# jianhengLiu/VINS-RGBD-FAST

Hardware: AMD Instinct MI355X
Metric: VIO frames/sec (640x480, 150 feats, 10-KF window) (higher is better)
Workload: dtype f64; 1 GPU; BASELINE configs[2]: 128 independent synthetic 640x480 RGB-D + 200 Hz IMU sequences per MI355X, 150 features, 10-keyframe window; sequences_per_gpu=128, tracker_lag=1, parallelism=sequences sharded per GPU, no data-path collective

## Files before the change

### vins-rgbd-fast_amd/csrc/be_kernels.hip

```cpp
#include <hip/hip_runtime.h>
#include "kernels.h"
#include "be_factors.h"

using namespace dm;

#if VIO_TIMERS
#define PH_INIT long long ph_t0 = (s == 0 && threadIdx.x == 0) ? VIO_CLOCK() : 0
#define PH(k) do { if (s == 0 && threadIdx.x == 0) { long long n_ = VIO_CLOCK(); B.timings[k] += (float)(n_ - ph_t0); ph_t0 = n_; } } while (0)
#else
#define PH_INIT do {} while (0)
#define PH(k) do {} while (0)
#endif

namespace {

struct Ctx {
    float *timings;
    const DevCfg *C;
    int s, W, P, LW, NL, NLs, NPR;
    BeSeq *be;
    FeSeq *fe;
    const vio_calibration *K;
    PreInt *pre;
    int *lm_id, *lm_start, *lm_nobs, *lm_est, *lm_solve, *lm_dyn, *lm_order, *lm_free, *lm_tmp, *lm_pidx, *lm_aidx, *lm_relo;
// ... 1486 lines not shown
                bool hit = false;
                int r = 0;
                if (k < F) { int st_, no_, rl_, r0_; lm_fields(k, st_, no_, rl_, r0_); r = r0_ + (j - i - 1); hit = st_ == i && no_ > j - i && r < nres; }
                unsigned long long m = __ballot(hit);
                if (hit) c.pair_list[o + __popcll(m & ((1ULL << lane) - 1ULL))] = r;
                o += __popcll(m);
            }
            if (relo_on && j == i + 1)
                for (int k0 = 0; k0 < F; k0 += 64) {
                    int k = k0 + lane;
                    bool hit = false;
                    int r = 0;
                    if (k < F) { int st_, no_, rl_, r0_; lm_fields(k, st_, no_, rl_, r0_); r = r0_ + no_ - 1; hit = st_ == i && rl_ && r < nres; }
                    unsigned long long m = __ballot(hit);
                    if (hit) c.pair_list[o + __popcll(m & ((1ULL << lane) - 1ULL))] = r;
                    o += __popcll(m);
                }
        }
        __syncthreads();
    }
    PH(104);
    if (t == 0) {
        be.n_in_problem = F; be.n_var_landmarks = Fa; be.n_residuals = nres - sh_i[3];
        be.relo_factors = sh_i[3];
        be.iterations = 0; be.successful = 0;
    }
    __syncthreads();
}

__device__ __forceinline__ void solve_epilogue(Ctx &c, const Params &X, double cost, int iters_done, int succ, long long ts0, double *sdx, double *sh_d, int *sh_i) {
    const int t = threadIdx.x, nt = blockDim.x;
    const vio_config &cfg = c.C->c;
    BeSeq &be = *c.be;
    const int W = c.W, nlm = be.n_lm;
    if (!cfg.use_imu) {
        if (t == 0) {
            be.final_cost = cost; be.iterations = iters_done; be.successful = succ;
            be.iter_total += iters_done; be.solve_total++;
            be.dbg[4] = (int)(VIO_CLOCK() - ts0);
        }
        if (t <= W) {
            const int i = t;
            for (int k = 0; k < 7; k++) be.para_Pose[i][k] = X.pose[i * 7 + k];
            stm(be.Rs[i], q2R(qnormalized(mkq(X.pose[i * 7 + 6], X.pose[i * 7 + 3], X.pose[i * 7 + 4], X.pose[i * 7 + 5]))));
            be.Ps[i][0] = X.pose[i * 7]; be.Ps[i][1] = X.pose[i * 7 + 1]; be.Ps[i][2] = X.pose[i * 7 + 2];
        }
    } else {
    if (t == 0) {
        be.final_cost = cost; be.iterations = iters_done; be.successful = succ;
        be.iter_total += iters_done; be.solve_total++;
        be.dbg[4] = (int)(VIO_CLOCK() - ts0);
        v3 origin_R0 = R2ypr(ldm(be.Rs[0]));
        v3 origin_P0 = ld3(be.Ps[0]);
        quat q0 = mkq(X.pose[6], X.pose[3], X.pose[4], X.pose[5]);
        v3 origin_R00 = R2ypr(q2R(q0));
        double y_diff = origin_R0.x - origin_R00.x;
        m3 rot_diff = ypr2R(mk(y_diff, 0, 0));
        if (fabs(fabs(origin_R0.y) - 90) < 1.0 || fabs(fabs(origin_R00.y) - 90) < 1.0) rot_diff = mul(ldm(be.Rs[0]), tr(q2R(q0)));
        sh_d[0] = 0;
        for (int q = 0; q < 9; q++) sdx[q] = rot_diff.a[q];
        sdx[9] = origin_P0.x; sdx[10] = origin_P0.y; sdx[11] = origin_P0.z;
    }
    __syncthreads();
    if (t <= W) for (int k = 0; k < 7; k++) be.para_Pose[t][k] = X.pose[t * 7 + k];
    if (t <= W) {
        int i = t;
        m3 rot_diff = ldm(sdx);
        v3 origin_P0 = mk(sdx[9], sdx[10], sdx[11]);
        quat qi = qnormalized(mkq(X.pose[i * 7 + 6], X.pose[i * 7 + 3], X.pose[i * 7 + 4], X.pose[i * 7 + 5]));
        stm(be.Rs[i], mul(rot_diff, q2R(qi)));
        st3(be.Ps[i], add(mul(rot_diff, mk(X.pose[i * 7] - X.pose[0], X.pose[i * 7 + 1] - X.pose[1], X.pose[i * 7 + 2] - X.pose[2])), origin_P0));
        st3(be.Vs[i], mul(rot_diff, mk(X.sb[i * 9], X.sb[i * 9 + 1], X.sb[i * 9 + 2])));
        for (int k = 0; k < 3; k++) { be.Bas[i][k] = X.sb[i * 9 + 3 + k]; be.Bgs[i][k] = X.sb[i * 9 + 6 + k]; }
        if (i == W && !be.init_frame) for (int k = 0; k < 3; k++) be.latest_Bg[k] = X.sb[i * 9 + 6 + k];
    }
    if (t == W + 1) {
        be.tic[0] = X.ex[0]; be.tic[1] = X.ex[1]; be.tic[2] = X.ex[2];
        stm(be.ric, q2R(qnormalized(mkq(X.ex[6], X.ex[3], X.ex[4], X.ex[5]))));
        if (cfg.estimate_td) be.td = X.td;
    }
    __syncthreads();
    if (t == 0 && be.relo_info) {
        const m3 rot_diff = ldm(sdx);
        const v3 origin_P0 = mk(sdx[9], sdx[10], sdx[11]);
        const m3 relo_r = mul(rot_diff, q2R(qnormalized(mkq(X.relo[6], X.relo[3], X.relo[4], X.relo[5]))));
        const v3 relo_t = add(mul(rot_diff, mk(X.relo[0] - X.pose[0], X.relo[1] - X.pose[1], X.relo[2] - X.pose[2])), origin_P0);
        const m3 prev_r = ldm(be.prev_relo_r);
        const double drift_yaw = R2ypr(prev_r).x - R2ypr(relo_r).x;
        const m3 dr = ypr2R(mk(drift_yaw, 0, 0));
        stm(be.drift_correct_r, dr);
        st3(be.drift_correct_t, sub(ld3(be.prev_relo_t), mul(dr, relo_t)));
        const int li = be.relo_local;
        const m3 Rl = ldm(be.Rs[li]);
        st3(be.relo_relative_t, mul(tr(relo_r), sub(ld3(be.Ps[li]), relo_t)));
        const quat qrel = R2q(mul(tr(relo_r), Rl));
        be.relo_relative_q[0] = qrel.w; be.relo_relative_q[1] = qrel.x; be.relo_relative_q[2] = qrel.y; be.relo_relative_q[3] = qrel.z;
        const double a = R2ypr(Rl).x - R2ypr(relo_r).x;
        be.relo_relative_yaw = a > 0 ? a - 360.0 * floor((a + 180.0) / 360.0) : a + 360.0 * floor((-a + 180.0) / 360.0);
        for (int k = 0; k < 7; k++) be.relo_Pose[k] = X.relo[k];
        be.relo_info = 0;
    }
    }
    for (int k = t; k < nlm; k += nt) {
        int slot = c.lm_order[k];
        int pi = c.lm_pidx[slot];
        if (pi < 0) continue;
        double d = 1.0 / c.feat[pi];
        c.lm_depth[slot] = d;
        c.lm_solve[slot] = d < 0 ? 2 : 1;
    }
    __syncthreads();
    if (be.solver_flag == 1 && !be.init_frame) {
        if (t == 0) {
            int fail = 0;
            if (nrm(ld3(be.Bas[W])) > 2.5) fail = 1;
            if (nrm(ld3(be.Bgs[W])) > 1.0) fail = 1;
            v3 tmpP = ld3(be.Ps[W]);
            if (nrm(sub(tmpP, ld3(be.last_P))) > 5) fail = 1;
            if (fabs(tmpP.z - be.last_P[2]) > 1) fail = 1;
            sh_i[0] = fail;
        }
        __syncthreads();
        if (sh_i[0]) {
            for (int k = t; k < c.NL; k += nt) c.lm_free[k] = c.NL - 1 - k;
            if (t == 0) {
                for (int i = 0; i <= W + 1; i++) c.pre[i].valid = 0;
                for (int i = 0; i <= W; i++) {
                    for (int k = 0; k < 3; k++) { be.Ps[i][k] = 0; be.Vs[i][k] = 0; be.Bas[i][k] = 0; be.Bgs[i][k] = 0; }
                    stm(be.Rs[i], eye());
                    be.Headers[i] = 0;
                    be.pre_idx[i] = i;
                }
                const vio_calibration &K = *c.K;
                for (int k = 0; k < 9; k++) be.ric[k] = cfg.estimate_extrinsic == 2 ? be.ex_ric[k] : K.ric[k];
                for (int k = 0; k < 3; k++) { be.tic[k] = K.tic[k]; be.latest_Bg[k] = 0; }
                be.td = K.td;
                be.g[0] = 0; be.g[1] = 0; be.g[2] = K.g_norm;
                be.first_imu = 0; be.frame_count = 0; be.solver_flag = 0; be.openExEstimation = 0; be.has_prior = 0;
                be.initFirstPoseFlag = 0; be.prevTime = -1; be.n_lm = 0; be.n_free = c.NL; be.ring_base = 0;
                be.imu_head = be.imu_count_ingest;
                be.relo_info = 0;
                be.reboot_count++;
                be.status_code = VIO_REBOOTED;
                be.rebooted = 1;
                be.do_marg = 0;
                be.overflow = 0;
            }
        }
    }
}

}

template <bool EXACT> __device__ void marg_body(const Batch &B, int s, int *scratch, double *sred, unsigned char *smem_marg);
__device__ void finish_body(const Batch &B, int s, int *scratch, PreWork &pw, unsigned char *smem_marg);

__device__ __forceinline__ void solve_body(const Batch &B, int s, int *scratch, double *sred, unsigned char *smem, PreWork &pw);

__global__ __launch_bounds__(1024) void be_solve_kernel(Batch B) {
    const int s = blockIdx.x + B.s0;
    __shared__ int scratch[2 * 1024 + 8];
    __shared__ double sred[64];
    extern __shared__ __attribute__((aligned(16))) unsigned char smem[];
    PreWork &pw = *(PreWork *)(smem + 16 * ((B.cfg->LW * 8 + 15) / 16));
    solve_body(B, s, scratch, sred, smem, pw);
}
__global__ __launch_bounds__(512) void be_solve_kernel_512(Batch B) {
    const int s = blockIdx.x + B.s0;
    __shared__ int scratch[2 * 1024 + 8];
    __shared__ double sred[64];
    extern __shared__ __attribute__((aligned(16))) unsigned char smem[];
    PreWork &pw = *(PreWork *)(smem + 16 * ((B.cfg->LW * 8 + 15) / 16));
    solve_body(B, s, scratch, sred, smem, pw);
}
__global__ __launch_bounds__(512) void be_marg_kernel(Batch B) {
    const int s = blockIdx.x + B.s0;
    __shared__ int scratch[2 * 512 + 8];
    __shared__ double sred[64];
    __shared__ PreWork pw;
    extern __shared__ __attribute__((aligned(16))) unsigned char smem[];
    marg_body<false>(B, s, scratch, sred, smem);
    __syncthreads();
    finish_body(B, s, scratch, pw, smem);
}
__global__ __launch_bounds__(512) void be_marg_exact_kernel(Batch B) {
    const int s = blockIdx.x + B.s0;
    __shared__ int scratch[2 * 512 + 8];
    __shared__ double sred[64];
    __shared__ PreWork pw;
    extern __shared__ __attribute__((aligned(16))) unsigned char smem[];
    marg_body<true>(B, s, scratch, sred, smem);
    __syncthreads();
    finish_body(B, s, scratch, pw, smem);
}

__device__ __forceinline__ void solve_body(const Batch &B, int s, int *scratch, double *sred, unsigned char *smem, PreWork &pw) {
    const int t = threadIdx.x, nt = blockDim.x;
    Ctx c = make_ctx(B, s);
    const DevCfg &C = *B.cfg;
    const vio_config &cfg = C.c;
    BeSeq &be = *c.be;
    if (!be.do_solve) return;
    const int W = c.W, P = c.P, LW = c.LW, W1 = W + 1;
    __shared__ Params X, Xc;
    __shared__ double sdx[6 * VIO_MAXW + 16], srp[6 * VIO_MAXW + 16];
    __shared__ int sh_i[8];
    __shared__ double sh_d[8];
    double *xs = (double *)smem;
    double *work = xs + LW;
    const int npairs = (W + 1) * W / 2;
    double *pb = (npairs * 210 <= 12288) ? work : c.pairblk;
    __shared__ double chol_dinv[VIO_LWMAX];
    const bool tiles_in_lds = ((LW >> 4) * ((LW >> 4) + 1) / 2) * 256 <= 16896 && !(B.flags & 1);
    const bool schur_staged = tiles_in_lds && schur_staged_ok(LW, nt);
    const bool hpl_sparse = schur_staged && 6 * W1 + 7 <= 128;

    PH_INIT;
    const long long ts0 = VIO_CLOCK();
    int F, Fa, nres;
    solve_prologue(B, c, X, scratch, pw, sh_i, F, Fa, nres);
    {
        const int *al = c.pair_list + c.nres_cap - c.NL;
        int nb = 0;
        for (int k = t; k < Fa; k += nt) nb += c.lm_est[al[k]] == 2 ? 1 : 0;
        if (nb) { atomicOr(&c.be->overflow, 512); atomicAdd(&c.be->bounded_solves, nb); }
    }
    const int nlm = be.n_lm;
    int *alist = c.pair_list + c.nres_cap - c.NL;
    const int n = c.NPR;
    PH(2);
    const int ex_active = sh_i[0], td_active = sh_i[1];
    const bool vext = ex_active || td_active;
    const int ne_ext = vext ? 7 : 0;
    const int oE = 15 * W1, oT = 15 * W1 + 6;

    double *g = c.vec, *sp = c.vec + 1 * LW, *dgp = c.vec + 2 * LW, *gradp = c.vec + 3 * LW, *gnp = c.vec + 4 * LW, *stp = c.vec + 5 * LW,
           *gs = c.vec + 6 * LW, *tmpv = c.vec + 7 * LW, *delta = c.vec + 8 * LW, *sgp = c.vec + 9 * LW, *hsgp = c.vec + 10 * LW,
           *yp = c.vec + 11 * LW, *up = c.vec + 12 * LW, *tmpv2 = c.vec + 13 * LW;
    double *sl = c.lvec, *dgl = c.lvec + c.NLs, *gradl = c.lvec + 2 * c.NLs, *gnl = c.lvec + 3 * c.NLs, *stl = c.lvec + 4 * c.NLs,
           *inv = c.lvec + 5 * c.NLs, *gls = c.lvec + 6 * c.NLs, *Hlls = c.lvec + 7 * c.NLs;
    const int Kpad = (Fa + 3) & ~3;
    double *hsgl = c.res + (size_t)c.nres_cap * 42 - 4 * (size_t)c.NLs;
    double *yl = hsgl + c.NLs, *ul = yl + c.NLs, *tmpl = ul + c.NLs;

    double cost = evaluate(c, X, c.feat, true, nres, sred, sdx, srp, work, vext);
    PH(4);
    assemble(B, c, X, nres, Fa, alist, srp, work, pb, hpl_sparse, vext);
    PH(5);
    if (t == 0) be.initial_cost = cost;
    for (int a = t; a < LW; a += nt) {
        bool act = a < P && (a < oE ? true : (a < oT ? ex_active != 0 : td_active != 0));
        if (!cfg.use_imu && (a < 6 || (a >= 6 * W1 && a < oE))) act = false;
        sp[a] = act ? 1.0 / (1.0 + sqrt(c.H[a * LW + a])) : 0.0;
    }
    for (int k = t; k < Kpad; k += nt) sl[k] = k < Fa ? 1.0 / (1.0 + sqrt(c.Hll[k])) : 0.0;
    __syncthreads();
    auto prepare_point = [&]() -> double {
        double m = 0;
        for (int a = t; a < P; a += nt) m = fmax(m, sp[a] != 0.0 ? fabs(g[a]) : 0.0);
        for (int k = t; k < Fa; k += nt) m = fmax(m, fabs(c.gl[k]));
        double r = block_max(m, sred);
        for (int a = t; a < LW; a += nt) {
            double hs = a < P ? sp[a] * sp[a] * c.H[a * LW + a] : 0.0;
            gs[a] = a < P ? sp[a] * g[a] : 0.0;
            dgp[a] = sqrt(fmin(fmax(hs, 1e-6), 1e32));
            gradp[a] = gs[a] / dgp[a];
            sgp[a] = gradp[a] / dgp[a];
            up[a] = sp[a] * sgp[a];
        }
        for (int k = t; k < Kpad; k += nt) {
            double hl = k < Fa ? sl[k] * sl[k] * c.Hll[k] : 0.0;
            Hlls[k] = hl;
            gls[k] = k < Fa ? sl[k] * c.gl[k] : 0.0;
            dgl[k] = sqrt(fmin(fmax(hl, 1e-6), 1e32));
            gradl[k] = gls[k] / dgl[k];
            ul[k] = sl[k] * (gradl[k] / dgl[k]);
        }
        __syncthreads();
        return r;
    };

    double radius = 1e4, mu = 1e-8, alpha = 0, dogleg_norm = 0;
    bool cauchy_valid = false;
    auto compute_cauchy = [&]() {
        matvec_pass(c.H, LW, P, P, nullptr, up, nullptr, tmpv, work);
        matvec_pass_2range(c.Hpl, LW, Fa, P, 6 * W1, 15 * W1, ne_ext, ul, up, tmpv2, tmpl, work);
        double g2 = 0, jg2 = 0;
        for (int a = t; a < LW; a += nt) {
            double v = a < P ? sp[a] * (tmpv[a] + tmpv2[a]) : 0.0;
            hsgp[a] = v;
            if (a < P) { g2 += gradp[a] * gradp[a]; jg2 += sgp[a] * v; }
        }
        for (int k = t; k < Kpad; k += nt) {
            double sgl = k < Fa ? gradl[k] / dgl[k] : 0.0;
            double v = k < Fa ? sl[k] * tmpl[k] + Hlls[k] * sgl : 0.0;
            hsgl[k] = v;
            if (k < Fa) { g2 += gradl[k] * gradl[k]; jg2 += sgl * v; }
        }
        block_sum2(g2, jg2, sred);
        alpha = g2 / jg2;
        cauchy_valid = true;
    };

    bool reuse = false, need_eval = false, have_J = false;
    int invalid = 0;
    int iters_done = 0, succ = 0;
    if (prepare_point() > 1e-10)
    for (int iter = 1; iter <= cfg.max_iterations; iter++) {
        iters_done = iter;
        if (!reuse) {
            if (need_eval) {
                PH(13);
                if (!have_J) cost = evaluate(c, X, c.feat, true, nres, sred, sdx, srp, work, vext);
                have_J = false;
                PH(4);
                assemble(B, c, X, nres, Fa, alist, srp, work, pb, hpl_sparse, vext);
                PH(5);
                need_eval = false;
                if (prepare_point() <= 1e-10) { iters_done = iter - 1; break; }
                PH(6);
            }
            cauchy_valid = false;
            bool ok = false;
            while (mu < 1.0) {
                for (int k = t; k < Kpad; k += nt) {
                    double iv = k < Fa ? 1.0 / (Hlls[k] + mu * dgl[k] * dgl[k]) : 0.0;
                    inv[k] = iv;
                    tmpl[k] = sl[k] * iv * gls[k];
                }
                __syncthreads();
                matvec_pass_2range(c.Hpl, LW, Fa, P, 6 * W1, 15 * W1, ne_ext, tmpl, nullptr, tmpv, nullptr, work);
                for (int a = t; a < LW; a += nt) xs[a] = a < P ? gs[a] - sp[a] * tmpv[a] : 0.0;
                for (int k = t; k < Kpad; k += nt) tmpl[k] = sl[k] * sl[k] * inv[k];
                __syncthreads();
                bool chol_ok;
                if (tiles_in_lds) {
                    {
                        unsigned colmask = 0;
                        for (int cb = 0; cb < (LW >> 4); cb++) {
                            const int c0 = 16 * cb, c1 = c0 + 15;
                            if (c0 < 6 * W1 || (vext && c1 >= 15 * W1 && c0 < 15 * W1 + 7)) colmask |= 1u << cb;
                        }
                        if (schur_staged)
                            schur_mfma_staged<9>(c.H, c.Hpl, tmpl, dgp, sp, mu, Kpad, LW, LW, work, colmask);
// ... 193 lines not shown
        double *cs = (double *)smem, *sn = cs + 256;
        int *pp = (int *)(sn + 256), *qq = pp + 256;
        double *As = scrA, *V2 = scrV;
        for (int w = t; w < n * n; w += nt) { const int i = w / n, j = w - i * n; As[w] = 0.5 * (Ar[i * n + j] + Ar[j * n + i]); }
        __syncthreads();
        const bool hbm_ql = !c.C->eig_jacobi;
        if (hbm_ql) { sym_eig_hbm(As, n, n, (double *)marg_dyn_lds, sred); V2 = As; }
        else sw2 = jacobi_block(As, V2, n, n, cs, sn, pp, qq, sred);
        for (int k = t; k < n; k += nt) {
            ev2[k] = hbm_ql ? ((const double *)marg_dyn_lds)[k] : As[k * n + k];
            double vb = 0;
            for (int i = 0; i < n; i++) vb += V2[i * n + k] * br[i];
            vb2[k] = vb;
        }
        __syncthreads();
        for (int w = t; w < n * n; w += nt) {
            const int k = w / n, i = w - k * n;
            const double S = ev2[k] > eps ? ev2[k] : 0.0;
            c.prior_J[w] = sqrt(S) * V2[i * n + k];
        }
        for (int k = t; k < n; k += nt) {
            const double Sinv = ev2[k] > eps ? 1.0 / ev2[k] : 0.0;
            c.prior_rf[k] = sqrt(Sinv) * vb2[k];
        }
        __syncthreads();
        for (int w = t; w < n * n; w += nt) {
            const int a = w / n, bb = w - a * n;
            double sacc = 0;
            for (int k = 0; k < n; k++) sacc += c.prior_J[k * n + a] * c.prior_J[k * n + bb];
            c.prior_H[w] = sacc;
        }
        for (int a = t; a < n; a += nt) {
            double sacc = 0;
            for (int k = 0; k < n; k++) sacc += c.prior_J[k * n + a] * c.prior_rf[k];
            c.prior_r[a] = sacc;
        }
    }
    __syncthreads();
    double acc = 0;
    for (int k = t; k < n; k += nt) acc += c.prior_rf[k] * c.prior_rf[k];
    const double c0 = block_sum(acc, sred);
    __syncthreads();
    if (t == 0) be.prior_c0 = c0;
    return sw2;
}

__device__ void marg_exact_finish(const Ctx &c, BeSeq &be, double *A, const double *b, int md, int mq, int n, const double *Cl, int ldc, int F0,
                                  bool second_new, double *sred, unsigned char *smem) {
    const int t = threadIdx.x, nt = blockDim.x;
    const double eps = 1e-8;
    const int MX = c.C->MX, m = md + F0;
    double *Emm = c.margE, *EV = Emm + (size_t)MX * MX, *Einv = EV + (size_t)MX * MX, *ET1 = Einv + (size_t)MX * MX;
    extern __shared__ __attribute__((aligned(16))) unsigned char marg_dyn_lds[];
    double *cs = (double *)smem, *sn = cs + 256;
    int *pp = (int *)(sn + 256), *qq = pp + 256;
    auto amm = [&](int i, int j) -> double {
        if (i < md && j < md) return 0.5 * (A[i * mq + j] + A[j * mq + i]);
        if (i >= md && j >= md) return i == j ? c.Hll[i - md] : 0.0;
        return Cl[(size_t)((i >= md ? i : j) - md) * ldc + (i >= md ? j : i)];
    };
    int sw1 = 0;
    double *Ar = c.margV, *br = c.vec;
    const long long tx0 = VIO_CLOCK();
    if (m <= c.C->MXL) {
        const int ld = m | 1;
        double *Al = (double *)marg_dyn_lds, *aux = Al + (size_t)m * ld;
        for (int w = t; w < m * m; w += nt) { const int i = w / m, j = w - i * m; Al[i * ld + j] = amm(i, j); }
        __syncthreads();
        sym_eig_lds(Al, m, ld, aux, c.C->eig_one_wave != 0);
        if (VIO_TIMERS && t == 0) be.dbg[7] = (int)(VIO_CLOCK() - tx0);
        for (int k = t; k < m; k += nt) { const double ev = aux[k]; aux[EIG_LD + k] = ev > eps ? 1.0 / ev : 0.0; }
        __syncthreads();
        for (int w = t; w < m * m; w += nt) {
            const int i = w / m, j = w - i * m;
            double sacc = 0;
            for (int k = 0; k < m; k++) sacc += Al[i * ld + k] * Al[j * ld + k] * aux[EIG_LD + k];
            Einv[w] = sacc;
        }
    } else {
        for (int w = t; w < m * m; w += nt) { const int i = w / m, j = w - i * m; Emm[w] = amm(i, j); }
        __syncthreads();
        if (!c.C->eig_jacobi) {
            double *ewk = (double *)marg_dyn_lds;
            sym_eig_hbm(Emm, m, m, ewk, sred);
            if (VIO_TIMERS && t == 0) be.dbg[7] = (int)(VIO_CLOCK() - tx0);
            for (int k = t; k < m; k += nt) { const double ev = ewk[k]; ewk[SYM_EIG_HBM_MAX + k] = ev > eps ? 1.0 / ev : 0.0; }
            __syncthreads();
            for (int w = t; w < m * m; w += nt) {
                const int i = w / m, j = w - i * m;
                const double *vi = Emm + (size_t)i * m, *vj = Emm + (size_t)j * m;
                double sacc = 0;
                for (int k0 = 0; k0 < m; k0 += 16) {
                    double a[16], b[16];
#pragma unroll
                    for (int u = 0; u < 16; u++) { const int k = min(k0 + u, m - 1); a[u] = vi[k]; b[u] = vj[k]; }
#pragma unroll
                    for (int u = 0; u < 16; u++) if (k0 + u < m) sacc += a[u] * b[u] * ewk[SYM_EIG_HBM_MAX + k0 + u];
                }
                Einv[w] = sacc;
            }
        } else {
        sw1 = jacobi_block(Emm, EV, m, m, cs, sn, pp, qq, sred);
        if (VIO_TIMERS && t == 0) be.dbg[7] = (int)(VIO_CLOCK() - tx0);
        for (int w = t; w < m * m; w += nt) {
            const int i = w / m, j = w - i * m;
            double sacc = 0;
            for (int k = 0; k < m; k++) { const double ev = Emm[(size_t)k * m + k]; if (ev > eps) sacc += EV[(size_t)i * m + k] * EV[(size_t)j * m + k] / ev; }
            Einv[w] = sacc;
        }
        }
    }
    __syncthreads();
    for (int w = t; w < n * m; w += nt) {
        const int i = w / m, j = w - i * m;
        double sacc = 0;
        for (int k = 0; k < md; k++) sacc += A[(md + i) * mq + k] * Einv[(size_t)k * m + j];
        for (int k0 = md; k0 < m; k0 += 16) {
            double a[16], b[16];
#pragma unroll
            for (int u = 0; u < 16; u++) { const int k = min(k0 + u, m - 1); a[u] = Cl[(size_t)(k - md) * ldc + md + i]; b[u] = Einv[(size_t)k * m + j]; }
#pragma unroll
            for (int u = 0; u < 16; u++) if (k0 + u < m) sacc += a[u] * b[u];
        }
        ET1[w] = sacc;
    }
    __syncthreads();
    for (int w = t; w < n * n; w += nt) {
        const int i = w / n, j = w - i * n;
        double tt = A[(md + i) * mq + md + j];
        for (int k = 0; k < md; k++) tt -= ET1[(size_t)i * m + k] * A[k * mq + md + j];
        for (int k0 = md; k0 < m; k0 += 16) {
            double a[16], b[16];
#pragma unroll
            for (int u = 0; u < 16; u++) { const int k = min(k0 + u, m - 1); a[u] = ET1[(size_t)i * m + k]; b[u] = Cl[(size_t)(k - md) * ldc + md + j]; }
#pragma unroll
            for (int u = 0; u < 16; u++) if (k0 + u < m) tt -= a[u] * b[u];
        }
        Ar[w] = tt;
    }
    for (int i = t; i < n; i += nt) {
        double sacc = b[md + i];
        for (int k = 0; k < md; k++) sacc -= ET1[(size_t)i * m + k] * b[k];
        for (int k = md; k < m; k++) sacc -= ET1[(size_t)i * m + k] * c.gl[k - md];
        br[i] = sacc;
    }
    __syncthreads();
    if (VIO_TIMERS && t == 0) be.dbg[8] = (int)(VIO_CLOCK() - tx0);
    const int sw2 = marg_literal_prior(c, be, Ar, br, n, c.margW, A, sred, smem);
    if (VIO_TIMERS && t == 0) be.dbg[9] = (int)(VIO_CLOCK() - tx0);
    if (t == 0) { be.dbg[0] = sw1 * 100 + sw2; be.dbg[2] = second_new ? 1 : 0; be.dbg[4] = m; }
    if (VIO_TIMERS && t == 0) be.dbg[10] = (int)(VIO_CLOCK() - tx0);
}

template <bool EXACT> __device__ void marg_body(const Batch &B, int s, int *scratch, double *sred, unsigned char *smem_marg) {
    const int t = threadIdx.x, nt = blockDim.x;
    Ctx c = make_ctx(B, s);
    const DevCfg &C = *B.cfg;
    const vio_config &cfg = C.c;
    BeSeq &be = *c.be;
    if (!be.do_marg || be.rebooted || be.frame_count < c.W) return;
    const int W = c.W, W1 = W + 1, n = c.NPR;
    const double eps = 1e-8;
    __shared__ Params X;
    __shared__ double sdx[6 * VIO_MAXW + 16], srp[6 * VIO_MAXW + 16];
    __shared__ double cs[VIO_MAXW * 3 + 10], sn[VIO_MAXW * 3 + 10];
    __shared__ int pp[VIO_MAXW * 3 + 10], qq[VIO_MAXW * 3 + 10];
    __shared__ double A15[225], V15[225], Pinv[225];
    __shared__ int newpresent[VIO_MAXW + 3];
    const bool second_new = be.marginalization_flag != 0;
    if (second_new && !(be.has_prior && be.prior_present[W - 1])) return;
    const bool exact = EXACT && cfg.marg_exact == 1 && c.margE != nullptr;
    const bool lit2 = EXACT && cfg.marg_exact == 2;
    int F0x = 0;
    int F0k = 0;
    PH_INIT;
    const long long tk0 = VIO_CLOCK();
    if (t <= W) {
        int i = t;
        X.pose[i * 7 + 0] = be.Ps[i][0]; X.pose[i * 7 + 1] = be.Ps[i][1]; X.pose[i * 7 + 2] = be.Ps[i][2];
        quat q = R2q(ldm(be.Rs[i]));
        X.pose[i * 7 + 3] = q.x; X.pose[i * 7 + 4] = q.y; X.pose[i * 7 + 5] = q.z; X.pose[i * 7 + 6] = q.w;
        for (int k = 0; k < 3; k++) { X.sb[i * 9 + k] = be.Vs[i][k]; X.sb[i * 9 + 3 + k] = be.Bas[i][k]; X.sb[i * 9 + 6 + k] = be.Bgs[i][k]; }
    }
    if (t == W + 1) {
        X.ex[0] = be.tic[0]; X.ex[1] = be.tic[1]; X.ex[2] = be.tic[2];
        quat q = R2q(ldm(be.ric));
        X.ex[3] = q.x; X.ex[4] = q.y; X.ex[5] = q.z; X.ex[6] = q.w;
        X.td = be.td;
    }
    if (t < W + 3) newpresent[t] = 0;
    __syncthreads();
    if (t <= W) for (int k = 0; k < 7; k++) be.para_Pose[t][k] = X.pose[t * 7 + k];
    const int md = second_new ? 6 : 15;
    const int mq = md + n;
    double *A = c.margA, *b = c.margB;
    for (int i = t; i < mq * mq; i += nt) A[i] = 0;
    for (int i = t; i < mq; i += nt) b[i] = 0;
    __syncthreads();
    const int rS = md + 6 * W, rE = md + 6 * W + 9, rT = md + 6 * W + 15;
    if (be.has_prior) {
        prior_dx(c, X, sdx);
        for (int i = t; i < n; i += nt) {
            double sacc = c.prior_r[i];
            for (int j0 = 0; j0 < n; j0 += 32) {
                double hv[32];
#pragma unroll
                for (int u = 0; u < 32; u++) hv[u] = c.prior_H[(size_t)min(j0 + u, n - 1) * n + i];
#pragma unroll
                for (int u = 0; u < 32; u++) if (j0 + u < n) sacc += hv[u] * sdx[j0 + u];
            }
            srp[i] = sacc;
        }
        __syncthreads();
        auto pmap = [&](int a) -> int {
            if (a < 6 * W) {
                int k = a / 6, d = a - 6 * k;
                if (second_new) return k == W - 1 ? d : md + 6 * k + d;
                return k == 0 ? d : md + 6 * (k - 1) + d;
            }
            if (a < 6 * W + 9) return second_new ? rS + (a - 6 * W) : 6 + (a - 6 * W);
            if (a < 6 * W + 15) return rE + (a - 6 * W - 9);
            return rT;
        };
        for (int w0 = t; w0 < n * n; w0 += 8 * nt) {
            double pv[8];
#pragma unroll
            for (int u = 0; u < 8; u++) pv[u] = c.prior_H[min(w0 + u * nt, n * n - 1)];
#pragma unroll
            for (int u = 0; u < 8; u++) {
                const int w = w0 + u * nt;
                if (w < n * n) { const int a = w / n, bb = w - a * n; A[pmap(a) * mq + pmap(bb)] = 0.0 + pv[u]; }
            }
        }
        for (int a = t; a < n; a += nt) b[pmap(a)] += srp[a];
        if (t < W + 3) {
            const int pres = be.prior_present[t];
            if (t > W) { if (pres) newpresent[t] = 1; }
            else if (second_new) { if (t < W - 1 || t == W) newpresent[t] = pres; }
            else if (t >= 1 && t < W && pres) newpresent[t - 1] = 1;
        }
        __syncthreads();
    }
    PH(16);
    if (!second_new) {
        PreInt &p1 = c.pre[be.pre_idx[1]];
        if (cfg.use_imu && p1.sum_dt < 10.0) {
            double *Jw = c.pairblk;
            double *raw = c.imu_raw;
            if ((t & 63) == 0) for (int part = t >> 6; part < 5; part += nt >> 6) {
                v3 G = ld3(be.g);
                if (part == 0) {
                    double r15[15];
                    bf::imu_raw_residual(p1, G, &X.pose[0], &X.sb[0], &X.pose[7], &X.sb[9], r15);
                    for (int r = 0; r < 15; r++) {
                        double sacc = 0;
                        for (int k = 0; k <= r; k++) sacc += p1.sqrt_info[r * 15 + k] * r15[k];
                        raw[r * 31 + 30] = sacc;
                    }
                } else
                    bf::imu_raw_jacobian_part(p1, G, &X.pose[0], &X.sb[0], &X.pose[7], &X.sb[9], part - 1, raw, 31);
            }
            __syncthreads();
            for (int w = t; w < 450; w += nt) {
                int r = w / 30, col = w - r * 30;
                double sacc = 0;
                for (int k = 0; k <= r; k++) sacc += p1.sqrt_info[r * 15 + k] * raw[k * 31 + col];
                Jw[w] = sacc;
            }
            __syncthreads();
            for (int w = t; w < 930; w += nt) {
                int a = w / 31, bb = w - a * 31;
                int ia = a < 15 ? a : (a < 21 ? md + (a - 15) : rS + (a - 21));
                double sacc = 0;
                if (bb < 30) {
                    int ib = bb < 15 ? bb : (bb < 21 ? md + (bb - 15) : rS + (bb - 21));
                    for (int k = 0; k < 15; k++) sacc += Jw[k * 30 + a] * Jw[k * 30 + bb];
                    A[ia * mq + ib] += sacc;
                } else {
                    for (int k = 0; k < 15; k++) sacc += Jw[k * 30 + a] * raw[k * 31 + 30];
                    b[ia] += sacc;
                }
            }
            if (t == 0) { newpresent[0] = 1; newpresent[W] = 1; }
            __syncthreads();
        }
        PH(17);
        int nlm = be.n_lm;
        int *flag = c.lm_tmp, *offs = c.res_k;
        for (int k = t; k < nlm; k += nt) { int slot = c.lm_order[k]; flag[k] = (in_problem(c, slot) && c.lm_start[slot] == 0) ? 1 : 0; }
        __syncthreads();
        int F0 = block_scan_flags(flag, nlm, offs, scratch);
        int *list0 = c.pair_list;
        for (int k = t; k < nlm; k += nt) if (flag[k]) list0[offs[k]] = c.lm_order[k];
        __syncthreads();
        const int per = W;
        int F0c = min(F0, c.nres_cap / per);
        if (exact) { F0c = min(F0c, min(C.MX - 15, 480)); F0x = F0c; }
        F0k = F0c;
        __shared__ double mgeo[(VIO_MAXW + 1) * 32 + 16];
        if (t >= 1 && t <= W) {
            bf::PairGeo g;
            bf::pair_geo(&X.pose[0], &X.pose[t * 7], X.ex, g);
            double *o = mgeo + (size_t)(t - 1) * 32;
            for (int q = 0; q < 9; q++) { o[q] = g.A1[q]; o[9 + q] = g.A2[q]; o[18 + q] = g.M[q]; }
            o[27] = g.t[0]; o[28] = g.t[1]; o[29] = g.t[2];
        }
        if (t == 0) stm(mgeo + (size_t)W * 32, q2R(mkq(X.ex[6], X.ex[3], X.ex[4], X.ex[5])));
        __syncthreads();
        for (int w = t; w < F0c * per; w += nt) {
            int li = w / per, k = w - li * per + 1;
            int slot = list0[li];
            double *out = c.res + (size_t)w * 42;
            if (k >= c.lm_nobs[slot]) { out[40] = 0; out[41] = 0; for (int q = 0; q < 40; q++) out[q] = 0; continue; }
            double rr[2], wgt = 1.0;
            const double inv_dep = 1.0 / c.lm_depth[slot];
            const bf::PairGeo &g = *(const bf::PairGeo *)(mgeo + (size_t)(k - 1) * 32);
            bf::eval_projection_pair(cfg, g, mgeo + (size_t)W * 32, X.ex, inv_dep, X.td, c.K->tr, obs_ptr(c, slot, 0), obs_ptr(c, slot, k), cfg.estimate_td != 0, rr, out,
                                     true, &wgt);
            out[40] = wgt * rr[0];
            out[41] = wgt * rr[1];
        }
        __syncthreads();
        PH(18);
        double *Cl = c.Hpl;
        const int ldc = c.LW;
        for (int w = t; w < F0c * ldc; w += nt) Cl[w] = 0;
        __syncthreads();
        {
            const int grp = t >> 4, gln = t & 15, ngrp = nt >> 4;
            for (int li0 = 0; li0 < F0c; li0 += ngrp) {
                const int li = li0 + grp;
                const bool act = li < F0c;
                const int no = act ? c.lm_nobs[list0[li]] : 0;
                double cm[13], dsum = 0, bsum = 0;
#pragma unroll
                for (int q = 0; q < 13; q++) cm[q] = 0;
                for (int k = gln + 1; k < no; k += 16) {
                    const double *Jg = c.res + (size_t)(li * per + k - 1) * 42;
                    double Jr[42];
#pragma unroll
                    for (int q = 0; q < 42; q++) Jr[q] = Jg[q];
                    const double jl0 = Jr[19], jl1 = Jr[39];
#pragma unroll
                    for (int q = 0; q < 6; q++) {
                        cm[q] += Jr[q] * jl0 + Jr[20 + q] * jl1;
                        cm[6 + q] += Jr[12 + q] * jl0 + Jr[32 + q] * jl1;
                        Cl[(size_t)li * ldc + md + 6 * (k - 1) + q] = Jr[6 + q] * jl0 + Jr[26 + q] * jl1;
                    }
                    if (cfg.estimate_td) cm[12] += Jr[18] * jl0 + Jr[38] * jl1;
                    dsum += jl0 * jl0 + jl1 * jl1;
                    bsum += jl0 * Jr[40] + jl1 * Jr[41];
                }
#pragma unroll
                for (int off = 8; off >= 1; off >>= 1) {
#pragma unroll
                    for (int q = 0; q < 13; q++) cm[q] += __shfl_xor(cm[q], off, 16);
                    dsum += __shfl_xor(dsum, off, 16);
                    bsum += __shfl_xor(bsum, off, 16);
                }
                if (act && gln == 0) {
#pragma unroll
                    for (int q = 0; q < 6; q++) { Cl[(size_t)li * ldc + q] = cm[q]; Cl[(size_t)li * ldc + rE + q] = cm[6 + q]; }
                    if (cfg.estimate_td) Cl[(size_t)li * ldc + rT] = cm[12];
                    c.Hll[li] = dsum;
                    c.gl[li] = bsum;
                }
            }
        }
        __syncthreads();
        PH(19);
        {
            const int lane = t & 63, wave = t >> 6, nw = nt >> 6, li = lane & 15, lk = lane >> 4;
            for (int j = 1 + wave; j <= W; j += nw) {
                v4f64 a00 = {0, 0, 0, 0}, a10 = {0, 0, 0, 0}, a11 = {0, 0, 0, 0};
                const int K = 2 * F0c;
                for (int k0 = 0; k0 < K; k0 += 64) {
                    double x0[16], x1[16];
#pragma unroll
                    for (int u = 0; u < 16; u++) {
                        int kk = k0 + 4 * u + lk;
                        bool valid = kk < K;
                        int lm = min(kk, K - 1) >> 1, sub = kk & 1;
                        const double *Jr = c.res + (size_t)(lm * per + j - 1) * 42;
                        double v0 = Jr[sub * 20 + li];
                        double v1 = Jr[li < 3 ? sub * 20 + 16 + li : 40 + sub];
                        x0[u] = valid ? v0 : 0.0;
                        x1[u] = (valid && li < 4) ? v1 : 0.0;
                    }
#pragma unroll
                    for (int u = 0; u < 16; u++) {
                        if (k0 + 16 * (u >> 2) >= K) break;
                        a00 = __builtin_amdgcn_mfma_f64_16x16x4f64(x0[u], x0[u], a00, 0, 0, 0);
                        a10 = __builtin_amdgcn_mfma_f64_16x16x4f64(x1[u], x0[u], a10, 0, 0, 0);
                        a11 = __builtin_amdgcn_mfma_f64_16x16x4f64(x1[u], x1[u], a11, 0, 0, 0);
                    }
                }
                double *out = c.pairblk + (size_t)(j - 1) * 210;
#pragma unroll
                for (int r = 0; r < 4; r++) {
                    int row = lk + 4 * r, col = li;
                    if (col <= row) out[sym_idx(col, row)] = a00[r];
                    if (row < 4) out[sym_idx(col, 16 + row)] = a10[r];
                    if (row < 4 && col < 4 && col <= row) out[sym_idx(16 + col, 16 + row)] = a11[r];
                }
            }
        }
        if (!exact) for (int li = t; li < F0c; li += nt) { double d = c.Hll[li]; c.Hll[li] = d > eps ? 1.0 / d : 0.0; }
        __syncthreads();
        PH(24);
        __shared__ signed char qfr[6 * VIO_MAXW + 40], qlc[6 * VIO_MAXW + 40];
        __shared__ double sub_part[4][6 * VIO_MAXW + 40];
        for (int a = t; a <= mq; a += nt) {
            int fr = -1, lc = 0;
            if (a == mq) { fr = 0; lc = 19; }
            else if (a < 6) { fr = 0; lc = a; }
            else if (a >= md && a < md + 6 * W) { fr = (a - md) / 6 + 1; lc = 6 + (a - md) % 6; }
            else if (a >= rE && a < rE + 6) { fr = 0; lc = 12 + (a - rE); }
            else if (a == rT && cfg.estimate_td) { fr = 0; lc = 18; }
            qfr[a] = (signed char)fr; qlc[a] = (signed char)lc;
        }
        for (int w = t; w < 4 * mq; w += nt) {
            const int ch = w / mq, a = w - ch * mq;
            double acc = 0;
            if (!exact) for (int li = ch; li < F0c; li += 4) acc += Cl[(size_t)li * ldc + a] * (c.gl[li] * c.Hll[li]);
            sub_part[ch][a] = acc;
        }
        __syncthreads();
        for (int w0 = t; w0 < mq * (mq + 1); w0 += 4 * nt) {
            bool use[4], multi[4], rhs[4];
            int dst[4], row[4], sidx[4];
            double pv[4], av[4];
#pragma unroll
            for (int u = 0; u < 4; u++) {
                const int w = min(w0 + u * nt, mq * (mq + 1) - 1);
                const int a = w / (mq + 1), bb = w - a * (mq + 1);
                const int fa = qfr[a], fb = qfr[bb];
                const int la = qlc[a], lb = qlc[bb];
                use[u] = w0 + u * nt < mq * (mq + 1) && fa >= 0 && fb >= 0 && !(fa > 0 && fb > 0 && fa != fb);
                multi[u] = use[u] && fa == 0 && fb == 0;
                rhs[u] = bb == mq; row[u] = a; dst[u] = a * mq + bb;
                sidx[u] = sym_idx(la, lb);
                const int f1 = fa > 0 ? fa : (fb > 0 ? fb : 1);
                pv[u] = use[u] ? c.pairblk[(size_t)(f1 - 1) * 210 + sidx[u]] : 0.0;
                av[u] = use[u] ? (rhs[u] ? b[a] : A[dst[u]]) : 0.0;
            }
#pragma unroll
            for (int u = 0; u < 4; u++) {
                if (!use[u]) continue;
                double sacc = pv[u];
                if (multi[u]) {
                    double fv[VIO_MAXW];
#pragma unroll
                    for (int j = 0; j < VIO_MAXW; j++) fv[j] = c.pairblk[(size_t)min(j, W - 1) * 210 + sidx[u]];
                    sacc = 0;
#pragma unroll
                    for (int j = 0; j < VIO_MAXW; j++) if (j < W) sacc += fv[j];
                }
                if (!rhs[u]) A[dst[u]] = av[u] + sacc;
                else b[row[u]] = av[u] + (sacc - ((sub_part[0][row[u]] + sub_part[1][row[u]]) + (sub_part[2][row[u]] + sub_part[3][row[u]])));
            }
        }
        __syncthreads();
        PH(25);
        if (!exact) {
            const int lane = t & 63, wave = t >> 6, nw = nt >> 6, li = lane & 15, lk = lane >> 4;
            const int nbq = (mq + 15) >> 4, ntile = nbq * (nbq + 1) / 2;
            for (int tile = wave; tile < ntile; tile += nw) {
                int ti, tj;
                tri_decode(tile, ti, tj);
                v4f64 acc = {0, 0, 0, 0};
                const int ca = min(16 * ti + li, ldc - 1), cb = min(16 * tj + li, ldc - 1);
                for (int k0 = 0; k0 < F0c; k0 += 64) {
                    double xa[16], xb[16];
#pragma unroll
                    for (int u = 0; u < 16; u++) {
                        int kk = k0 + 4 * u + lk;
                        bool valid = kk < F0c;
                        int kc = min(kk, F0c - 1);
                        double va = Cl[(size_t)kc * ldc + ca], vb = Cl[(size_t)kc * ldc + cb], dinv = c.Hll[kc];
                        xa[u] = valid ? -(va * dinv) : 0.0;
                        xb[u] = valid ? vb : 0.0;
                    }
#pragma unroll
                    for (int u = 0; u < 16; u++) {
                        if (k0 + 16 * (u >> 2) >= F0c) break;
                        acc = __builtin_amdgcn_mfma_f64_16x16x4f64(xa[u], xb[u], acc, 0, 0, 0);
                    }
                }
#pragma unroll
                for (int r = 0; r < 4; r++) {
                    int row = 16 * ti + lk + 4 * r, col = 16 * tj + li;
                    if (row < mq && col < mq && (ti != tj || col <= row)) {
                        A[row * mq + col] += acc[r];
                        if (row != col) A[col * mq + row] += acc[r];
                    }
                }
            }
        }
        for (int li = t; li < F0c; li += nt) {
            int no = c.lm_nobs[list0[li]];
            for (int k = 1; k < no; k++) newpresent[k - 1] = 1;
            if (no > 1) { newpresent[W + 1] = 1; if (cfg.estimate_td) newpresent[W + 2] = 1; }
        }
        __syncthreads();
    }
    if (VIO_TIMERS && s == 0 && t == 0 && !second_new) B.timings[31] += 1.0f;
    PH(20);
    if (exact) marg_exact_finish(c, be, A, b, md, mq, n, c.Hpl, c.LW, F0x, second_new, sred, smem_marg);
    else {
    for (int w = t; w < md * md; w += nt) { int i = w / md, j = w - i * md; A15[w] = 0.5 * (A[i * mq + j] + A[j * mq + i]); }
    __syncthreads();
    __shared__ int pinv_direct;
    __shared__ double L15[225];
    if (t < 64) {
        const bool okc = spd_inverse_wave16(A15, md, 1e-6, L15, V15, Pinv);
        if (t == 0) pinv_direct = okc ? 1 : 0;
    }
    __syncthreads();
    if (!pinv_direct) {
        if (t < 64) jacobi_wave16(A15, V15, md, md, cs, sn, pp, qq);
        __syncthreads();
        for (int w = t; w < md * md; w += nt) {
            int i = w / md, j = w - i * md;
            double sacc = 0;
            for (int k = 0; k < md; k++) { double ev = A15[k * md + k]; if (ev > eps) sacc += V15[i * md + k] * V15[j * md + k] / ev; }
            Pinv[w] = sacc;
        }
        __syncthreads();
    }
    if (VIO_TIMERS && s == 0 && t == 0 && pinv_direct) B.timings[26] += 1.0f;
    PH(36);
    double *T1 = (double *)smem_marg, *Amr = T1 + (size_t)n * md;
    for (int w = t; w < n * md; w += nt) {
        int i = w / md, j = w - i * md;
        double sacc = 0;
        for (int k = 0; k < md; k++) sacc += A[(md + i) * mq + k] * Pinv[k * md + j];
        T1[w] = sacc;
        const int k2 = w / n, j2 = w - k2 * n;
        Amr[w] = A[k2 * mq + md + j2];
    }
    __syncthreads();
    PH(37);
    double *Ar = c.margV;
    double *br = c.vec;
    for (int w0 = t; w0 < n * n; w0 += 8 * nt) {
        double av[8];
#pragma unroll
        for (int u = 0; u < 8; u++) { const int w = min(w0 + u * nt, n * n - 1), i = w / n, j = w - i * n; av[u] = A[(md + i) * mq + md + j]; }
#pragma unroll
        for (int u = 0; u < 8; u++) {
            const int w = w0 + u * nt;
            if (w >= n * n) break;
            const int i = w / n, j = w - i * n;
            double tt = av[u];
            for (int k = 0; k < md; k++) tt -= T1[i * md + k] * Amr[k * n + j];
            Ar[w] = tt;
        }
    }
    for (int i = t; i < n; i += nt) {
        double sacc = b[md + i];
        for (int k = 0; k < md; k++) sacc -= T1[i * md + k] * b[k];
        br[i] = sacc;
    }
    __syncthreads();
    PH(21);
    if (lit2) {
        __shared__ int cert_bad;
        if (t == 0) cert_bad = pinv_direct ? 0 : 1;
        __syncthreads();
        double n_t = 0, n_d = 0, n_db = 0;
        if (!second_new) {
            const double *Cl = c.Hpl;
            const int ldc = c.LW;
            for (int li = t; li < F0k; li += nt) {
                const double dinv = c.Hll[li];
                if (!(dinv > 0.0)) cert_bad = 1;
                n_d += dinv * dinv;
                for (int a = 0; a < md; a++) {
                    double tt = 0;
                    for (int bq = 0; bq < md; bq++) tt += Pinv[a * md + bq] * Cl[(size_t)li * ldc + bq];
                    tt *= dinv;
                    n_t += tt * tt;
                    const double db = dinv * Cl[(size_t)li * ldc + a];
                    n_db += db * db;
                }
            }
        }
        block_sum3(n_t, n_d, n_db, sred);
        double n_s = 0;
        for (int w = t; w < md * md; w += nt) n_s += Pinv[w] * Pinv[w];
        n_s = block_sum(n_s, sred);
        __syncthreads();
        if (t == 0) {
            const double bound = sqrt(n_s) + 2.0 * sqrt(n_t) + sqrt(n_d) + sqrt(n_db) * sqrt(n_t);
            const bool certified = !cert_bad && isfinite(bound) && bound > 0.0 && 1.0 / bound > 1e-7;
            be.dbg[11] = certified ? 1 : 0;
            if (!certified) be.dbg[12] += 1;
        }
        __syncthreads();
        const int sw2 = marg_literal_prior(c, be, Ar, br, n, c.margW, A, sred, smem_marg);
        if (t == 0) { be.dbg[0] = sw2; be.dbg[2] = second_new ? 1 : 0; be.dbg[4] = md; }
    } else {
    for (int w0 = t; w0 < n * n; w0 += 8 * nt) {
        double x[8], y[8];
#pragma unroll
        for (int u = 0; u < 8; u++) { const int w = min(w0 + u * nt, n * n - 1), i = w / n, j = w - i * n; x[u] = Ar[i * n + j]; y[u] = Ar[j * n + i]; }
#pragma unroll
        for (int u = 0; u < 8; u++) if (w0 + u * nt < n * n) c.prior_H[w0 + u * nt] = 0.5 * (x[u] + y[u]);
    }
    for (int i = t; i < n; i += nt) c.prior_r[i] = br[i];
    PH(38);
    {
        __shared__ __attribute__((aligned(16))) double cq_x[EIG_LD + 16];
        __shared__ double cq_dinv[EIG_LD + 16];
        __shared__ int cq_flag;
        const int nbq = (n + 15) >> 4;
        double *T = (double *)smem_marg;
        double dmax = 0;
        for (int i = t; i < n; i += nt) dmax = fmax(dmax, fabs(Ar[i * n + i]));
        dmax = block_max(dmax, sred);
        const double delta = 64.0 * 2.220446049250313e-16 * (double)n * dmax;
        const int ntl = nbq * (nbq + 1) / 2 * 256;
        for (int w0 = t; w0 < ntl; w0 += 4 * nt) {
            double x[4], y[4];
            int ii[4], jj[4], dd[4];
#pragma unroll
            for (int u = 0; u < 4; u++) {
                const int w = min(w0 + u * nt, ntl - 1);
                int tile = w >> 8, e = w & 255, r = e >> 4, cc = e & 15, ti, tj;
                tri_decode(tile, ti, tj);
                const int i = 16 * ti + r, j = 16 * tj + cc, ic = min(i, n - 1), jc = min(j, n - 1);
                ii[u] = i; jj[u] = j; dd[u] = tl_idx(ti, tj, r, cc);
                x[u] = Ar[ic * n + jc]; y[u] = Ar[jc * n + ic];
            }
#pragma unroll
            for (int u = 0; u < 4; u++) {
                if (w0 + u * nt >= ntl) break;
                const int i = ii[u], j = jj[u];
                T[dd[u]] = (i < n && j < n) ? 0.5 * (x[u] + y[u]) + (i == j ? delta : 0.0) : (i == j ? 1.0 : 0.0);
            }
        }
        for (int i = t; i < 16 * nbq; i += nt) cq_x[i] = i < n ? br[i] : 0.0;
        __syncthreads();
        PH(39);
        double c0 = 0;
        if (dmax > 0 && chol_tiles(T, nbq, &cq_flag, cq_dinv, nullptr, cq_x)) {
            double acc = 0;
            for (int i = t; i < n; i += nt) acc += cq_x[i] * cq_x[i];
            c0 = block_sum(acc, sred);
            if (!isfinite(c0)) c0 = 0;
        }
        __syncthreads();
        if (t == 0) { be.prior_c0 = c0; be.dbg[0] = 0; be.dbg[2] = second_new ? 1 : 0; }
    }
    }
    }
    PH(22);
    if (t < W) {
        int src = second_new ? (t == W - 1 ? W : t) : t + 1;
        for (int d = 0; d < 7; d++) c.prior_x0[t * 7 + d] = X.pose[src * 7 + d];
    }
    if (t == W) for (int d = 0; d < 9; d++) c.prior_x0[W * 7 + d] = X.sb[(second_new ? 0 : 1) * 9 + d];
    if (t == W + 1) { for (int d = 0; d < 7; d++) c.prior_x0[W * 7 + 9 + d] = X.ex[d]; c.prior_x0[W * 7 + 16] = X.td; }
    __syncthreads();
    if (t < W + 3) be.prior_present[t] = newpresent[t];
    if (t == 0) { be.has_prior = 1; be.dbg[3] = (int)(VIO_CLOCK() - tk0); }
    PH(23);
}

__global__ void be_set_relo_kernel(Batch B, int seq, const double *par) {
    if (threadIdx.x != 0 || blockIdx.x != 0) return;
    BeSeq &be = B.be[seq];
    const int W = B.cfg->W;
    be.relo_stamp = par[0];
    be.relo_index = (int)par[1];
    be.relo_nmatch = (int)par[2];
    for (int k = 0; k < 3; k++) be.prev_relo_t[k] = par[3 + k];
    for (int k = 0; k < 9; k++) be.prev_relo_r[k] = par[6 + k];
    for (int i = 0; i < W; i++)
        if (be.relo_stamp == be.Headers[i]) {
            be.relo_local = i;
            be.relo_info = 1;
            for (int j = 0; j < 7; j++) be.relo_Pose[j] = be.para_Pose[i][j];
        }
}

__global__ __launch_bounds__(512) void be_prior_factor_kernel(Batch B, int seq) {
    const int s = seq, t = threadIdx.x, nt = blockDim.x;
    __shared__ double sred[64];
    extern __shared__ __attribute__((aligned(16))) unsigned char smem_marg[];
    Ctx c = make_ctx(B, s);
    BeSeq &be = *c.be;
    if (!be.has_prior) return;
    const int n = c.NPR;
    const double eps = 1e-8;
    const double *br = c.prior_r;
    const long long tj0 = VIO_CLOCK();
    const bool in_lds = n <= 96;
    const int ldj = in_lds ? (n | 1) : n;
    double *As = in_lds ? (double *)smem_marg : c.margA;
    double *Vv = in_lds ? (double *)smem_marg + n * ldj : c.margW + (size_t)n * 16;
    for (int w = t; w < n * n; w += nt) { int i = w / n, j = w - i * n; As[i * ldj + j] = c.prior_H[w]; }
    __syncthreads();
    __shared__ double ev_d[6 * VIO_MAXW + 16], ev_e[6 * VIO_MAXW + 16], ev_g[6 * VIO_MAXW + 16];
    __shared__ double ev_part[8 * EIG_LD];
    if (in_lds) {
        double *Al = (double *)smem_marg;
        if ((nt >> 6) <= 8) sym_eig_tridiag_mt(Al, n, ldj, ev_d, ev_e, ev_g, ev_part);
        else sym_eig_tridiag(Al, n, ldj, ev_d, ev_e, ev_g, sred);
        if (t == 0) be.dbg[5] = (int)(VIO_CLOCK() - tj0);
        tridiag_ql_wave(Al, n, ldj, ev_d, ev_e);
    } else {
        double *Ag = c.margA;
        if ((nt >> 6) <= 8) sym_eig_tridiag_mt(Ag, n, ldj, ev_d, ev_e, ev_g, ev_part);
        else sym_eig_tridiag(Ag, n, ldj, ev_d, ev_e, ev_g, sred);
        if (t == 0) be.dbg[5] = (int)(VIO_CLOCK() - tj0);
        tridiag_ql_wave(Ag, n, ldj, ev_d, ev_e);
    }
    if (t == 0) be.dbg[6] = (int)(VIO_CLOCK() - tj0);
    Vv = As;
    if (t == 0) be.dbg[1] = (int)(VIO_CLOCK() - tj0);
    for (int w = t; w < n * n; w += nt) {
        int k = w / n, i = w - k * n;
        double wv = ev_d[k];
        double S = wv > eps ? wv : 0.0;
        c.prior_J[w] = sqrt(S) * Vv[i * ldj + k];
    }
    for (int k = t; k < n; k += nt) {
        double wv = ev_d[k];
        double Sinv = wv > eps ? 1.0 / wv : 0.0;
        double vb = 0;
        for (int i = 0; i < n; i++) vb += Vv[i * ldj + k] * br[i];
        c.prior_rf[k] = sqrt(Sinv) * vb;
    }
}

__device__ void finish_body(const Batch &B, int s, int *scratch, PreWork &pw, unsigned char *smem_marg) {
    const int t = threadIdx.x, nt = blockDim.x;
    Ctx c = make_ctx(B, s);
    const DevCfg &C = *B.cfg;
    const vio_config &cfg = C.c;
    BeSeq &be = *c.be;
    const int W = c.W, W1 = W + 1;
    __shared__ int sh_i[4];
    double *od = B.odom + (size_t)s * 11;
    if (!be.processed || be.rebooted) return;
    PH_INIT;
    int nlm = be.n_lm;
    int *flag = c.lm_pidx, *offs = c.lm_aidx;
    const int fc = be.frame_count;
    const int sflag0 = be.solver_flag;
    __syncthreads();
    const bool dyn_initial = sflag0 == 0 && (cfg.dynamic_init || (fc == W && !be.do_solve && be.ex_pending));
    if (dyn_initial) {
        if (fc < W) {
            if (t == 0) be.frame_count = fc + 1;
            return;
        }
    } else if (sflag0 == 0) {
        if (fc == W && be.do_solve) {
            if (t == 0) be.solver_flag = 1;
            __syncthreads();
        } else {
            if (t == 0 && fc < W) {
                int n = fc + 1;
                for (int k = 0; k < 3; k++) { be.Ps[n][k] = be.Ps[fc][k]; be.Vs[n][k] = be.Vs[fc][k]; be.Bas[n][k] = be.Bas[fc][k]; be.Bgs[n][k] = be.Bgs[fc][k]; }
                for (int k = 0; k < 9; k++) be.Rs[n][k] = be.Rs[fc][k];
                be.frame_count = n;
            }
            return;
        }
    } else if (!be.init_frame) {
        m3 ric = ldm(be.ric);
        v3 tic = ld3(be.tic);
        for (int k = t; k < nlm; k += nt) {
            int slot = c.lm_order[k];
            if (!(c.lm_nobs[slot] >= 2 && c.lm_start[slot] < W - 2)) continue;
            double depth = c.lm_depth[slot];
            if (depth < 0) continue;
            int imu_i = c.lm_start[slot], no = c.lm_nobs[slot];
            const double *oi = obs_ptr(c, slot, imu_i);
            v3 pts_i = mk(oi[0], oi[1], oi[2]);
            double err = 0, err3 = 0;
            int cnt = 0;
            for (int q = 1; q < no; q++) {
                int imu_j = imu_i + q;
                const double *oj = obs_ptr(c, slot, imu_j);
                v3 pts_j = mk(oj[0], oj[1], oj[2]);
                v3 pts_w = add(mul(ldm(be.Rs[imu_i]), add(mul(ric, scl(depth, pts_i)), tic)), ld3(be.Ps[imu_i]));
                v3 pts_cj = mul(tr(ric), sub(mul(tr(ldm(be.Rs[imu_j])), sub(pts_w, ld3(be.Ps[imu_j]))), tic));
                double rx = pts_cj.x / pts_cj.z - pts_j.x, ry = pts_cj.y / pts_cj.z - pts_j.y;
                err += sqrt(rx * rx + ry * ry);
                err3 += nrm(sub(pts_cj, pts_j)) / depth;
                cnt++;
            }
            if (cnt > 0) c.lm_dyn[slot] = (cfg.focal_length * err / cnt > 10 || err3 / cnt > 2.0) ? 1 : 0;
        }
        __syncthreads();
    }
    PH(27);
    if (be.marginalization_flag == 0) {
        if (t == 0) {
            for (int k = 0; k < 9; k++) be.back_R0[k] = be.Rs[0][k];
            for (int k = 0; k < 3; k++) be.back_P0[k] = be.Ps[0][k];
            int first = be.pre_idx[0];
            for (int i = 0; i < W; i++) {
                be.Headers[i] = be.Headers[i + 1];
                for (int k = 0; k < 3; k++) { be.Ps[i][k] = be.Ps[i + 1][k]; be.Vs[i][k] = be.Vs[i + 1][k]; be.Bas[i][k] = be.Bas[i + 1][k]; be.Bgs[i][k] = be.Bgs[i + 1][k]; }
                for (int k = 0; k < 9; k++) be.Rs[i][k] = be.Rs[i + 1][k];
                be.pre_idx[i] = be.pre_idx[i + 1];
            }
            be.pre_idx[W] = first;
            bf::preint_init(c.pre[first], ld3(be.acc_0), ld3(be.gyr_0), ld3(be.Bas[W]), ld3(be.Bgs[W]));
        }
        __syncthreads();
        PH(28);
        m3 R0 = mul(ldm(be.back_R0), ldm(be.ric)), R1 = mul(ldm(be.Rs[0]), ldm(be.ric));
        v3 P0 = add(ld3(be.back_P0), mul(ldm(be.back_R0), ld3(be.tic))), P1 = add(ld3(be.Ps[0]), mul(ldm(be.Rs[0]), ld3(be.tic)));
        for (int k = t; k < nlm; k += nt) {
            int slot = c.lm_order[k];
// ... 228 lines not shown
```

### vins-rgbd-fast_amd/csrc/kernels.h

```cpp
#pragma once
#include <hip/hip_runtime.h>
#include "vio_state.h"
#include "../../include/vio_synth.h"

#define PI_CH 8
#define PREINT_MANY_LDS_DOUBLES (PI_CH * (225 + 270))
static inline size_t fast_lds_bytes(int rw, int rh) {
    return (size_t)(((rw + 6) * rh + 15) & ~15) + (size_t)((rw * rh + 15) & ~15) + (size_t)(((rw - 6) * (rh - 6) + 63) / 64 + 2) * 8 + 16;
}
__host__ __device__ static inline size_t ps_eval_lds_bytes(int W) {
    const size_t W1 = (size_t)W + 1, a = (W1 * W1 + 1) * 32 * 8, b = (size_t)W * (VIO_PREINT_HDR + 1) * 8;
    return (a > b ? a : b) + 64;
}
static inline size_t ps_ls_lds_bytes(int W) { (void)W; return ((((sizeof(Params) / sizeof(double)) + 1) & ~(size_t)1) + 176) * 8 + 16; }
struct LkImages {
    const uint8_t *prev[4];
    const uint8_t *next[4];
    int w[4], h[4];
};

__global__ void fe_begin_kernel(Batch B, const double *stamps, int gate, int publish, const uint8_t *modes, const double *R_rel);
__global__ void be_latest_odometry_kernel(Batch B, int seq, double *out11);
__global__ void fe_predict_motion_kernel(Batch B, int seq, double t0, double t1, double *out9);
__global__ void fe_pyrdown_kernel(Batch B, const uint8_t *src_base, size_t src_stride, int sw, int sh, int dst_level, int write_level0);
__global__ void fe_pyrdown_stage_kernel(const uint8_t *src, int sw, int sh, uint8_t *dst);
__global__ void fe_clahe_lut_kernel(Batch B, const uint8_t *src_base, size_t stride);
__global__ void fe_clahe_apply_kernel(Batch B, const uint8_t *src_base, size_t stride);
__global__ void fe_clahe_lut_stage_kernel(const uint8_t *src, int W, int H, uint8_t *lut);
__global__ void fe_clahe_apply_stage_kernel(const uint8_t *src, int W, int H, const uint8_t *lut, uint8_t *dst);
__global__ void fe_predict_kernel(Batch B);
__global__ void fe_lk_kernel(Batch B);
__global__ void fe_lk_stage_kernel(LkImages im, int maxLevel, int n, const float2 *prevPts, float2 *nextPts, uint8_t *status);
__global__ void fe_ransac_stage_kernel(vio_config c, int n, const float2 *p1, const float2 *p2, uint8_t *status);
__global__ void fe_camera_stage_kernel(vio_camera cam, int n, const double *uv, const double *R9, double *ray, double *un, double *uv_out);
__global__ void fe_select_kernel(Batch B);
__global__ void fe_fast_kernel(Batch B);
__global__ void fe_fast_stage_kernel(const uint8_t *img, int W, GridRect r, uint32_t *out, int cap, int *count);
__global__ void fe_add_kernel(Batch B, int gate);
struct IngestSrc {
    const int *n_obs;
    const int *ids;
    const double *obs;
    const double *stamps;
    int cap;
};
template <bool EXCALIB> __global__ void be_ingest_kernel(Batch B, const uint16_t *depth_base, size_t depth_stride, IngestSrc src);
__global__ void be_stage_relative_r_kernel(int n, const double *corres6, double *R9);
__global__ void be_solve_kernel(Batch B);
__global__ void be_solve_kernel_512(Batch B);
__global__ void be_marg_kernel(Batch B);
__global__ void be_marg_exact_kernel(Batch B);
__global__ void ps_setup_kernel(Batch B);
__global__ void ps_eval_kernel(Batch B);
__global__ void ps_eval_kernel_occ3(Batch B);
__global__ void ps_eval_kernel_occ4(Batch B);
__global__ void ps_asm_a_kernel(Batch B);
__global__ void ps_asm_a_kernel_occ4(Batch B);
__global__ void ps_asm_b_schur_kernel(Batch B, int nb_b, int by_blocks);
__global__ void ps_serial_big_kernel(Batch B);
__global__ void ps_serial_kernel_512(Batch B);
__global__ void ps_final_kernel(Batch B);
__global__ void ps_ls_kernel(Batch B);
__global__ void ps_evalf_kernel(Batch B);
static inline size_t ps_evalf_lds_bytes(int W) {
    const size_t W1 = (size_t)W + 1, a = ((size_t)PS_FUSE_CAP * 28 + (W1 * W / 2 + 1) * 32) * 8 + (size_t)PS_FUSE_CAP * 12, b = ((size_t)W * (VIO_PREINT_HDR + 1) + (size_t)W * 465) * 8;
    return (a > b ? a : b) + 16;
}
__global__ void be_prior_factor_kernel(Batch B, int seq);
__global__ void be_set_relo_kernel(Batch B, int seq, const double *par);
__global__ void be_stage_pnp_kernel(const double *pts, int n, double *par6);
__global__ void be_dyn_finalize_kernel(Batch B, int seq, const double *samples, const int *offs);
__global__ void be_stage_imu_kernel(vio_config cfg, PreInt *P, int n, const double *dt, const double *acc, const double *gyr,
                                    const double *par, double g_norm, double *preint_out, double *r15, double *J480);
__global__ void be_stage_projection_kernel(vio_config cfg, const double *in, int use_td, int form, double *r2, double *J46);
__global__ void be_stage_imu_block_kernel(const PreInt *P, const double *par, double g_norm, double *G961);
__global__ void imu_scatter_kernel(Batch B, int total, const int *seq_of, const double *t, const double *acc, const double *gyr);
__global__ void imu_commit_kernel(Batch B, int total, const int *seq_of);
__global__ void synth_render_kernel(vio_synth_config c, int S, uint64_t seq0, const float *rays, const float *poses, uint8_t *gray, uint16_t *depth);
```

### vins-rgbd-fast_amd/csrc/vio_abi.hip

```cpp
#include <hip/hip_runtime.h>
#include <math.h>
#include <algorithm>
#include <cmath>
#include <stdlib.h>
#include <mutex>
#include <chrono>
#include <string>
#include <string.h>
#include <vector>
#include "kernels.h"
#include "dyninit_host.h"
#include "camera_model.h"
#include "snapshot.h"

thread_local std::string g_err;

namespace {

#define HIPCHK(x)                                                                                        \
    do {                                                                                                 \
        hipError_t e_ = (x);                                                                             \
        if (e_ != hipSuccess) { g_err = std::string(#x) + ": " + hipGetErrorString(e_); return VIO_EDEVICE; } \
    } while (0)

void circle_halfwidths(int radius, int *hw) {
    for (int i = 0; i <= radius; i++) hw[i] = -1;
    int err = 0, dx = radius, dy = 0, plus = 1, minus = (radius << 1) - 1;
    while (dx >= dy) {
        if (dx > hw[dy]) hw[dy] = dx;
        if (dy > hw[dx]) hw[dx] = dy;
        dy++;
        err += plus;
        plus += 2;
        int mask = (err <= 0) - 1;
        err -= minus & mask;
        dx += mask;
        minus -= mask & 2;
    }
}

}

struct vio_batch {
    DevCfg hc;
    Batch B;
    int S;
    int device = -1;
    struct Group {
        int s0 = 0, n = 0;
        hipStream_t stream = nullptr;
        hipStream_t fe_stream = nullptr;
        hipEvent_t ev_solve = nullptr, ev_fe = nullptr, ev_be = nullptr, ev_ingest = nullptr;
        hipStream_t copy_stream = nullptr;
        hipStream_t copy_stream2 = nullptr;
        hipGraphExec_t solve_graph = nullptr;
        uint64_t solve_graph_key = 0;
        hipEvent_t ev_up_gray[2] = {nullptr, nullptr}, ev_up_depth[2] = {nullptr, nullptr};
        bool up_used[2] = {false, false};
        int flip = 0;
        hipEvent_t ev_rd_gray[2] = {nullptr, nullptr}, ev_rd_depth[2] = {nullptr, nullptr};
        bool have_rd_gray[2] = {false, false}, have_rd_depth[2] = {false, false};
        hipEvent_t ev_host_fe = nullptr, ev_host_be = nullptr;
        bool host_fe_pending = false, host_be_pending = false;
        bool have_solve_ev = false, have_ingest_ev = false;
        static constexpr int kSideRing = 16;
        unsigned char *side_ring = nullptr;
        hipEvent_t side_ev[kSideRing] = {};
        bool side_used[kSideRing] = {};
        int side_pos = 0;
    };
    std::vector<Group> groups;
    int tracker_lag = 0;
    int extra_slots = 2;
    int xcd_n = 0;
    bool use_graph = false;
    int xcd_map = 1;
    int fe_xcd_map = 1;
    bool fe_partitioned = false;
    int ps_asm_b_blocks = 24;
    int asm_b_by_blocks = 2;
    int serial_threads = 512;
    hipStream_t stream = nullptr;
    hipStream_t fe_stream = nullptr;
    hipEvent_t ev[4];
    std::vector<void *> allocs;
    uint8_t *d_fisheye = nullptr;
    uint8_t *d_gray_stage = nullptr, *d_gray_stage1 = nullptr;
    uint16_t *d_depth_stage = nullptr, *d_depth_stage1 = nullptr;
    double *d_stamps = nullptr;
    uint8_t *d_modes = nullptr;
    double *d_rrel = nullptr;
    int *d_in_n = nullptr, *d_in_ids = nullptr;
    double *d_in_obs = nullptr, *d_in_stamps = nullptr;
    double *d_r9 = nullptr;
    std::vector<vio_calibration> cal;
    vio_calibration *d_cal = nullptr;
    std::vector<vio_camera> cam;
    vio_camera *d_cam = nullptr;
    struct DynSeq {
        std::vector<vinit::ImageFrame> frames;
        double initial_timestamp = 0;
        bool nonlinear = false;
        int attempts = 0, failures = 0, last_stage = 0;
    };
    std::vector<DynSeq> dyn;
    bool dyn_active = false;
    int *h_state = nullptr;
    int *d_state = nullptr;
    hipEvent_t ev_state = nullptr;
    bool state_pending = false;
    double *d_dyn_samples = nullptr;
    int *d_dyn_offs = nullptr;
    size_t dyn_samples_cap = 0;
    std::mutex imu_mu;
    std::vector<int> p_seq;
    std::vector<double> p_t, p_acc, p_gyr;
    struct ImuStage {
        int *h_seq = nullptr, *d_seq = nullptr;
        double *h_t = nullptr, *h_acc = nullptr, *h_gyr = nullptr, *d_t = nullptr, *d_acc = nullptr, *d_gyr = nullptr;
        size_t cap = 0;
        hipEvent_t done = nullptr;
        bool busy = false;
    } imu_stage[2];
    int imu_stage_cur = 0;
    hipEvent_t ev_imu = nullptr;
    std::vector<double> last_imu_t;
    size_t lds_select = 0, lds_add = 0, lds_fast = 0, lds_solve = 0, lds_serial = 0, lds_marg = 0, lds_factor = 0, lds_ps_ls = 0, lds_ps_evalf = 0;
    int ps_evalf_blocks = 0;
    bool feed_throttle = true;
    int uploads_in_flight = 2;
    int relo_frames = 0;
    bool line_search = true;
    int be_threads = 512, marg_threads = 384;
    int solve_mode = 1;
    bool asm_a_occ4 = false;
    int eval_occ = 0;
    bool serial_big = false;
    size_t lds_ps_eval = 0;
    int ps_eval_blocks = 0, ps_asm_a_blocks = 0, ps_schur_tiles = 0;
    bool timing_valid = false;
    std::vector<hipEvent_t> pev;
    int prof_steps = 0, prof_cur = -1;
    bool prof_fe_only = false;
    struct SnapRow { const char *name; int kind; unsigned char *base; int64_t bytes, blob_off; };
    std::vector<SnapRow> snap_rows;
    int64_t snap_dev_bytes = 0, snap_chunks = 0;
    int snap_entries = 0;
    SnapEntry *d_snap_tab = nullptr;
    SnapSeq *d_snap_seqs = nullptr;
    size_t snap_seqs_cap = 0;
    unsigned char *d_snap_stage = nullptr;
    size_t snap_stage_cap = 0;
};
#define VIO_NK 10
#define VIO_NEV 12
#define PEV(h, k) do { if (g.s0 == 0 && (h)->prof_cur >= 0 && (h)->prof_cur < (h)->prof_steps) (void)hipEventRecord((h)->pev[(size_t)(h)->prof_cur * VIO_NEV + (k)], (k) <= 7 ? g.fe_stream : g.stream); } while (0)

static size_t ingest_lds_bytes(const DevCfg &C, bool excalib) {
    const size_t ht = (size_t)C.lm_hash_size * 8;
    return excalib ? std::max(ht, (size_t)4 * C.NP * sizeof(double) + 16) : ht;
}
static int raise_lds_limit(const void *fn, size_t bytes) {
    struct Seen { const void *fn; int dev; size_t bytes; };
    static std::mutex mu;
    static std::vector<Seen> seen;
    int dev = 0;
    (void)hipGetDevice(&dev);
    std::lock_guard<std::mutex> lk(mu);
    for (auto &e : seen)
        if (e.fn == fn && e.dev == dev) {
            if (bytes <= e.bytes) return 0;
            e.bytes = bytes;
            return hipFuncSetAttribute(fn, hipFuncAttributeMaxDynamicSharedMemorySize, (int)bytes) == hipSuccess ? 0 : -1;
        }
    seen.push_back({fn, dev, bytes});
    return hipFuncSetAttribute(fn, hipFuncAttributeMaxDynamicSharedMemorySize, (int)bytes) == hipSuccess ? 0 : -1;
}

static bool lds_fits(const void *fn, size_t dynamic_bytes, const char *name) {
    hipFuncAttributes a;
    int dev = 0, cap = 0;
    if (hipFuncGetAttributes(&a, fn) != hipSuccess) return true;
    if (hipGetDevice(&dev) != hipSuccess || hipDeviceGetAttribute(&cap, hipDeviceAttributeMaxSharedMemoryPerBlock, dev) != hipSuccess || cap <= 0) cap = 160 * 1024;
    if (a.sharedSizeBytes + dynamic_bytes <= (size_t)cap) return true;
    g_err = std::string("configuration needs more LDS than a workgroup may own: ") + name;
    return false;
}

static size_t marg_exact_lds_bytes(int m) { return ((size_t)m * (m | 1) + 11 * (size_t)(6 * VIO_MAXW + 16)) * 8 + 64; }

struct DevGuard {
    int prev = -1;
    bool switched = false;
    bool failed = false;
    explicit DevGuard(const vio_batch *h) {
        if (!h || h->device < 0) return;
        if (hipGetDevice(&prev) != hipSuccess) { failed = true; return; }
        if (prev != h->device) { switched = hipSetDevice(h->device) == hipSuccess; failed = !switched; }
    }
    ~DevGuard() { if (switched) (void)hipSetDevice(prev); }
    DevGuard(const DevGuard &) = delete;
    DevGuard &operator=(const DevGuard &) = delete;
};
static int sync_all(vio_batch *h) {
    for (auto &g : h->groups) {
        if (g.copy_stream) HIPCHK(hipStreamSynchronize(g.copy_stream));
        if (g.copy_stream2) HIPCHK(hipStreamSynchronize(g.copy_stream2));
        HIPCHK(hipStreamSynchronize(g.fe_stream));
        HIPCHK(hipStreamSynchronize(g.stream));
        g.host_fe_pending = g.host_be_pending = false;
    }
    return VIO_OK;
}

__global__ void imu_scatter_kernel(Batch B, int total, const int *seq_of, const double *t, const double *acc, const double *gyr) {
    const int i = blockIdx.x * blockDim.x + threadIdx.x;
    if (i >= total) return;
    const DevCfg &C = *B.cfg;
    const int *off = seq_of + total;
    const int s = seq_of[i];
    const int slot = (B.be[s].imu_count + (i - off[s])) % C.NIMU;
    B.imu_t[(size_t)s * C.NIMU + slot] = t[i];
    for (int k = 0; k < 3; k++) {
        B.imu_acc[((size_t)s * C.NIMU + slot) * 3 + k] = acc[3 * i + k];
        B.imu_gyr[((size_t)s * C.NIMU + slot) * 3 + k] = gyr[3 * i + k];
    }
}
__global__ void imu_commit_kernel(Batch B, int total, const int *seq_of) {
    const int s = blockIdx.x * blockDim.x + threadIdx.x;
    if (s >= B.S) return;
    const int *off = seq_of + total;
    B.be[s].imu_count += off[s + 1] - off[s];
}

namespace {

void cal_from_config(const vio_config &c, vio_calibration &k) {
    k.fx = c.fx; k.fy = c.fy; k.cx = c.cx; k.cy = c.cy; k.k1 = c.k1; k.k2 = c.k2; k.p1 = c.p1; k.p2 = c.p2;
    for (int i = 0; i < 9; i++) k.ric[i] = c.ric[i];
    for (int i = 0; i < 3; i++) k.tic[i] = c.tic[i];
    k.td = c.td; k.tr = c.tr;
    k.acc_n = c.acc_n; k.acc_w = c.acc_w; k.gyr_n = c.gyr_n; k.gyr_w = c.gyr_w; k.g_norm = c.g_norm;
}
void cal_into_config(const vio_calibration &k, vio_config &c) {
    c.fx = k.fx; c.fy = k.fy; c.cx = k.cx; c.cy = k.cy; c.k1 = k.k1; c.k2 = k.k2; c.p1 = k.p1; c.p2 = k.p2;
    for (int i = 0; i < 9; i++) c.ric[i] = k.ric[i];
    for (int i = 0; i < 3; i++) c.tic[i] = k.tic[i];
    c.td = k.td; c.tr = k.tr;
    c.acc_n = k.acc_n; c.acc_w = k.acc_w; c.gyr_n = k.gyr_n; c.gyr_w = k.gyr_w; c.g_norm = k.g_norm;
}

vio_camera pinhole_camera(const vio_calibration &k) {
    vio_camera m;
    memset(&m, 0, sizeof(m));
    m.model = VIO_CAMERA_PINHOLE;
    const double p[8] = {k.fx, k.fy, k.cx, k.cy, k.k1, k.k2, k.p1, k.p2};
    for (int i = 0; i < 8; i++) m.p[i] = p[i];
    return m;
}

template <class T> int dalloc(vio_batch *h, T **p, size_t n) {
    void *q = nullptr;
    size_t bytes = n * sizeof(T);
    if (bytes == 0) bytes = sizeof(T);
    HIPCHK(hipMalloc(&q, bytes));
    HIPCHK(hipMemset(q, 0, bytes));
    h->allocs.push_back(q);
    *p = (T *)q;
    return VIO_OK;
}

enum { VIO_RESET_ESTIMATOR = 1, VIO_RESET_TRACKER = 2 };
int init_state(vio_batch *h, int s_lo, int s_hi, int what = VIO_RESET_ESTIMATOR | VIO_RESET_TRACKER) {
    const DevCfg &C = h->hc;
    int n = s_hi - s_lo, W = C.W;
    std::vector<FeSeq> fe(n);
    if (what & VIO_RESET_TRACKER) {
        memset(fe.data(), 0, sizeof(FeSeq) * n);
        for (int s = 0; s < n; s++) {
            FeSeq &f = fe[s];
            f.first_image_flag = 1;
            for (int k = 0; k < C.ncells; k++) f.grids_texture_status[k] = 1;
            f.R_rel[0] = f.R_rel[4] = f.R_rel[8] = 1;
        }
    } else {
        HIPCHK(hipMemcpy(fe.data(), h->B.fe + s_lo, sizeof(FeSeq) * n, hipMemcpyDeviceToHost));
// ... 283 lines not shown
        if (!res.ok) D.failures++;
        D.initial_timestamp = be.cur_stamp;
        if (res.ok || res.stage == 4) {
            for (int i = 0; i <= W; i++) for (int k = 0; k < 3; k++) be.Bgs[i][k] += res.delta_bg[k];
            changed = true;
        }
        if (res.force_margin_old) { be.marginalization_flag = 0; changed = true; }
    }
    if (res.ok) {
        for (int i = 0; i <= W; i++) {
            for (int k = 0; k < 3; k++) { be.Ps[i][k] = res.Ps[i][k]; be.Vs[i][k] = res.Vs[i][k]; if (res.set_ba) be.Bas[i][k] = res.Ba[k]; }
            for (int k = 0; k < 9; k++) be.Rs[i][k] = res.Rs[i][k];
        }
        for (int k = 0; k < 3; k++) be.g[k] = res.g[k];
        be.solver_flag = 1; be.init_frame = 1; be.do_solve = 1; be.do_marg = 1;
        {
            std::vector<double> samp;
            std::vector<int> offs(VIO_MAXW + 3, 0);
            for (int j = 1; j <= W; j++) {
                for (const auto &f : D.frames)
                    if (f.stamp > be.Headers[j - 1] && f.stamp <= be.Headers[j])
                        for (size_t k = 0; k < f.dt.size(); k++) {
                            samp.push_back(f.dt[k]);
                            for (int q = 0; q < 3; q++) samp.push_back(f.acc[3 * k + q]);
                            for (int q = 0; q < 3; q++) samp.push_back(f.gyr[3 * k + q]);
                        }
                offs[j + 1] = (int)(samp.size() / 7);
            }
            offs[1] = 0;
            if (samp.size() > h->dyn_samples_cap) {
                if (h->d_dyn_samples) (void)hipFree(h->d_dyn_samples);
                h->dyn_samples_cap = samp.size() * 2 + 7 * 1024;
                HIPCHK(hipMalloc((void **)&h->d_dyn_samples, h->dyn_samples_cap * sizeof(double)));
            }
            if (!h->d_dyn_offs) HIPCHK(hipMalloc((void **)&h->d_dyn_offs, (VIO_MAXW + 3) * sizeof(int)));
            if (!samp.empty()) HIPCHK(hipMemcpy(h->d_dyn_samples, samp.data(), samp.size() * sizeof(double), hipMemcpyHostToDevice));
            HIPCHK(hipMemcpy(h->d_dyn_offs, offs.data(), (VIO_MAXW + 3) * sizeof(int), hipMemcpyHostToDevice));
        }
        D.frames.clear();
        D.nonlinear = true;
        *finalize = true;
        changed = true;
    } else {
        be.dyn_failed = 1;
        changed = true;
        if (be.marginalization_flag == 0) {
            const double t0 = be.Headers[0];
            size_t k = 0;
            while (k < D.frames.size() && D.frames[k].stamp <= t0) k++;
            bool found = false;
            for (const auto &f : D.frames) if (f.stamp == t0) found = true;
            if (found) D.frames.erase(D.frames.begin(), D.frames.begin() + k);
        }
    }
    if (changed) HIPCHK(hipMemcpy(h->B.be + s, &be, sizeof(BeSeq), hipMemcpyHostToDevice));
    return VIO_OK;
}

int launch_backend(vio_batch *h, vio_batch::Group &g, const uint16_t *d_depth, const IngestSrc &src, int one_seq = -1) {
    const DevCfg &C = h->hc;
    const int S = one_seq >= 0 ? 1 : g.n;
    hipStream_t st = g.stream;
    Batch Bg = h->B;
    Bg.s0 = one_seq >= 0 ? one_seq : g.s0;
    const bool prof = one_seq < 0;
    if (prof) PEV(h, 8);
    if (C.exc) be_ingest_kernel<true><<<S, 256, ingest_lds_bytes(C, true), st>>>(Bg, d_depth, (size_t)C.c.width * C.c.height, src);
    else be_ingest_kernel<false><<<S, 256, ingest_lds_bytes(C, false), st>>>(Bg, d_depth, (size_t)C.c.width * C.c.height, src);
    if (prof) PEV(h, 9);
    if (one_seq < 0) { (void)hipEventRecord(g.ev_ingest, st); g.have_ingest_ev = true; }
    if (h->dyn_active || (C.c.dynamic_init && one_seq >= 0)) {
        HIPCHK(hipStreamSynchronize(st));
        for (int s = Bg.s0; s < Bg.s0 + S; s++) {
            if (h->dyn[s].nonlinear && one_seq < 0) continue;
            bool fin = false;
            int rc = dynamic_init_step(h, s, src, &fin);
            if (rc != VIO_OK) return rc;
            if (fin) { be_dyn_finalize_kernel<<<1, 256, 0, st>>>(h->B, s, h->d_dyn_samples, h->d_dyn_offs); HIPCHK(hipStreamSynchronize(st)); }
        }
        bool any = false;
        for (int s = 0; s < h->S; s++) any = any || !h->dyn[s].nonlinear;
        h->dyn_active = any;
    }
    const int be_threads = h->be_threads;
    if (h->solve_mode == 1) {
        const bool fuse_only = Bg.fuse > 0 && !C.c.estimate_extrinsic && !C.c.estimate_td && h->relo_frames <= 0 &&
                               (size_t)(C.W + 1) * C.c.max_cnt * 12 / 10 <= (size_t)PS_FUSE_MAXBLK * (PS_FUSE_CAP - C.W);
        Bg.fuse_only = fuse_only ? 1 : 0;
        auto launch_phased = [&]() {
            ps_setup_kernel<<<S, 512, 0, st>>>(Bg);
            const int slots = C.c.max_iterations + h->extra_slots;
            const bool xm = h->xcd_map && S >= 8;
            const int XN = h->xcd_n > 0 ? h->xcd_n : 8;
            const int nb_e = h->ps_eval_blocks, nb_a = h->ps_asm_a_blocks, nb_bs = h->ps_asm_b_blocks + h->ps_schur_tiles + (Bg.gn_ext ? 1 : 0), S8 = XN * ((S + XN - 1) / XN);
            Batch Be = Bg, Ba = Bg, Bb = Bg;
            Be.ns = Ba.ns = Bb.ns = S;
            Be.xcd_n = Ba.xcd_n = Bb.xcd_n = XN;
            Be.xcd_nb = xm ? nb_e : 0; Ba.xcd_nb = xm ? nb_a : 0; Bb.xcd_nb = xm ? nb_bs : 0;
            const dim3 g_e = xm ? dim3(S8 * nb_e) : dim3(nb_e, S), g_a = xm ? dim3(S8 * nb_a) : dim3(nb_a, S), g_b = xm ? dim3(S8 * nb_bs) : dim3(nb_bs, S);
            Batch Bf = Bg;
            Bf.ns = S; Bf.xcd_n = XN; Bf.xcd_nb = xm ? h->ps_evalf_blocks : 0;
            const dim3 g_f = xm ? dim3(S8 * h->ps_evalf_blocks) : dim3(h->ps_evalf_blocks, S);
            for (int k = 0; k < slots; k++) {
                if (Bg.fuse) ps_evalf_kernel<<<g_f, 256, h->lds_ps_evalf, st>>>(Bf);
                if (!fuse_only) {
                    if (h->eval_occ == 4) ps_eval_kernel_occ4<<<g_e, 256, h->lds_ps_eval, st>>>(Be);
                    else if (h->eval_occ == 3) ps_eval_kernel_occ3<<<g_e, 256, h->lds_ps_eval, st>>>(Be);
                    else ps_eval_kernel<<<g_e, 256, h->lds_ps_eval, st>>>(Be);
                    if (h->asm_a_occ4) ps_asm_a_kernel_occ4<<<g_a, 512, 0, st>>>(Ba);
                    else ps_asm_a_kernel<<<g_a, 512, 0, st>>>(Ba);
                }
                ps_asm_b_schur_kernel<<<g_b, 256, (size_t)(C.NL + 16 + (6 * (C.W + 1) + 7 <= 128 ? 8 * 128 : 8 * 192) ) * sizeof(double), st>>>(Bb, h->ps_asm_b_blocks, h->asm_b_by_blocks);
                if (h->serial_big) ps_serial_big_kernel<<<S, 512, h->lds_serial, st>>>(Bg);
                else ps_serial_kernel_512<<<S, 512, h->lds_serial, st>>>(Bg);
                if (h->line_search && k + 1 < slots) ps_ls_kernel<<<S, 256, h->lds_ps_ls, st>>>(Bg);
            }
            ps_final_kernel<<<S, 256, 0, st>>>(Bg);
        };
        if (h->use_graph && one_seq < 0) {
            uint64_t key = 1469598103934665603ULL;
            auto mixin = [&](const void *p, size_t nbytes) { const unsigned char *q = (const unsigned char *)p; for (size_t i = 0; i < nbytes; i++) { key ^= q[i]; key *= 1099511628211ULL; } };
            mixin(&Bg, sizeof(Bg));
            mixin(&h->line_search, sizeof(h->line_search));
            mixin(&fuse_only, sizeof(fuse_only));
            const int knobs[12] = {C.c.max_iterations + h->extra_slots, h->eval_occ, h->asm_a_occ4 ? 1 : 0, h->serial_big ? 1 : 0, h->serial_threads, h->ps_eval_blocks, h->ps_asm_a_blocks,
                                   h->ps_asm_b_blocks + 1000 * h->asm_b_by_blocks, h->ps_schur_tiles, h->xcd_map, h->xcd_n, (int)h->lds_serial};
            mixin(knobs, sizeof(knobs));
            mixin(&h->lds_ps_eval, sizeof(h->lds_ps_eval));
            if (g.solve_graph && g.solve_graph_key != key) { (void)hipGraphExecDestroy(g.solve_graph); g.solve_graph = nullptr; }
            g.solve_graph_key = key;
            if (!g.solve_graph) {
                hipGraph_t gr = nullptr;
                HIPCHK(hipStreamBeginCapture(st, hipStreamCaptureModeThreadLocal));
                launch_phased();
                HIPCHK(hipStreamEndCapture(st, &gr));
                HIPCHK(hipGraphInstantiate(&g.solve_graph, gr, nullptr, nullptr, 0));
                (void)hipGraphDestroy(gr);
            }
            HIPCHK(hipGraphLaunch(g.solve_graph, st));
        } else
            launch_phased();
    } else if (be_threads <= 512) be_solve_kernel_512<<<S, be_threads, h->lds_solve, st>>>(Bg);
    else be_solve_kernel<<<S, be_threads, h->lds_solve, st>>>(Bg);
    if (prof) PEV(h, 10);
    (void)hipEventRecord(g.ev_solve, st);
    g.have_solve_ev = true;
    if (C.c.dynamic_init && one_seq < 0 && &g == &h->groups.back()) {
        state_gather_kernel<<<(h->S + 255) / 256, 256, 0, st>>>(h->B, h->d_state);
        HIPCHK(hipMemcpyAsync(h->h_state, h->d_state, sizeof(int) * h->S, hipMemcpyDeviceToHost, st));
        HIPCHK(hipEventRecord(h->ev_state, st));
        h->state_pending = true;
    }
    if (C.MX > 0) be_marg_exact_kernel<<<S, h->marg_threads, h->lds_marg, st>>>(Bg);
    else be_marg_kernel<<<S, h->marg_threads, h->lds_marg, st>>>(Bg);
    if (prof) PEV(h, 11);
    HIPCHK(hipGetLastError());
    return VIO_OK;
}

int refresh_dynamic_state(vio_batch *h) {
    if (!h->hc.c.dynamic_init) return VIO_OK;
    if (h->state_pending) {
        HIPCHK(hipEventSynchronize(h->ev_state));
        h->state_pending = false;
        bool any = false;
        for (int s = 0; s < h->S; s++) {
            if (h->h_state[s] == 0 && h->dyn[s].nonlinear) h->dyn[s] = vio_batch::DynSeq();
            if (h->h_state[s] != 0) h->dyn[s].nonlinear = true;
            any = any || !h->dyn[s].nonlinear;
        }
        h->dyn_active = any;
    }
    return VIO_OK;
}

}

extern "C" {

const char *vio_last_error(void) { return g_err.c_str(); }

void vio_config_default(vio_config *c) {
    memset(c, 0, sizeof(*c));
    c->width = 640; c->height = 480;
    c->max_cnt = 150; c->min_dist = 15;
    c->grid_rows = 5; c->grid_cols = 6;
    c->window_size = 10;
    c->max_landmarks = 1000;
    c->fix_depth = 1;
    c->estimate_extrinsic = 0;
    c->estimate_td = 0;
    c->max_iterations = 8;
    c->ransac_max_iters = 1000;
    c->lk_max_level = 1;
    c->use_imu = 1;
    c->fx = 604.5821781259577; c->fy = 604.2544712985845; c->cx = 321.2638233484251; c->cy = 239.70969315130674;
    c->k1 = 0.13387871564774004; c->k2 = -0.2731913133377051; c->p1 = 0.0020296263577681264; c->p2 = -0.00044384544608203714;
    c->focal_length = 460.0;
    c->f_threshold = 1.0;
    c->depth_min = 0.3; c->depth_max = 6.0;
    c->acc_n = 0.1; c->acc_w = 0.001; c->gyr_n = 0.01; c->gyr_w = 0.0001; c->g_norm = 9.805;
    const double ric[9] = {0.02629567, -0.00713751, 0.99962873, -0.99934346, 0.02474397, 0.02646484, -0.02492368, -0.99966834, -0.00648216};
    const double tic[3] = {0.17336835, 0.049596, -0.10574841};
    memcpy(c->ric, ric, sizeof(ric));
    memcpy(c->tic, tic, sizeof(tic));
    c->td = 0.0; c->tr = 0.0;
    c->min_parallax_px = 10.0;
    c->init_depth = 5.0;
}

static void ortho_ric(const double *in, double *out) {
    dm::m3 Rc = dm::q2R(dm::qnormalized(dm::R2q(dm::ldm(in))));
    dm::stm(out, Rc);
}

static int build_devcfg(const vio_config *cfg, int imu_capacity, DevCfg &C) {
    memset(&C, 0, sizeof(C));
    C.c = *cfg;
    const vio_config &c = C.c;
    if (c.width < 64 || c.height < 64 || c.width > 4095 || c.height > 4095) { g_err = "image size out of range"; return VIO_EINVAL; }
    if (c.window_size < 4 || c.window_size > VIO_MAXW) { g_err = "window_size must be 4..20"; return VIO_EINVAL; }
    if (c.dynamic_init < 0 || c.dynamic_init > 1) { g_err = "dynamic_init must be 0 or 1"; return VIO_EINVAL; }
    if (c.use_imu < 0 || c.use_imu > 1) { g_err = "use_imu must be 0 or 1"; return VIO_EINVAL; }
    if (!c.use_imu && c.dynamic_init) { g_err = "the dynamic initialisation needs the IMU (estimator.cpp:231)"; return VIO_EINVAL; }
    if (c.grid_rows < 1 || c.grid_cols < 1 || c.grid_rows * c.grid_cols > VIO_MAX_CELLS) { g_err = "too many grid cells"; return VIO_EINVAL; }
    if (c.min_dist < 1 || c.min_dist > 63) { g_err = "min_dist must be 1..63"; return VIO_EINVAL; }
    if (c.lk_max_level < 0 || c.lk_max_level > 3) { g_err = "lk_max_level must be 0..3"; return VIO_EINVAL; }
    if (c.estimate_extrinsic < 0 || c.estimate_extrinsic > 2) { g_err = "estimate_extrinsic must be 0, 1 or 2"; return VIO_EINVAL; }
    if (c.estimate_extrinsic == 2 && !c.use_imu) {
        g_err = "estimate_extrinsic = 2 needs the IMU: the rotation is calibrated against the gyroscope's delta_q (identity without IMU)";
        return VIO_EINVAL;
    }
    if (c.estimate_extrinsic == 2) {
        dm::stm(C.c.ric, dm::eye());
        for (int k = 0; k < 3; k++) C.c.tic[k] = 0;
    } else {
        ortho_ric(c.ric, C.c.ric);
    }
    C.W = c.window_size;
    C.ncells = c.grid_rows * c.grid_cols;
    C.grids_threshold = c.max_cnt / C.ncells;
    if (C.grids_threshold <= 0) { g_err = "max_cnt must exceed the number of grid cells (feature_tracker.cpp:88-93)"; return VIO_EINVAL; }
    C.grid_h = c.height / c.grid_rows;
    C.grid_w = c.width / c.grid_cols;
    int res_h = c.height - (c.grid_rows - 1) * C.grid_h, res_w = c.width - (c.grid_cols - 1) * C.grid_w;
    for (int i = 0; i < c.grid_rows; i++)
        for (int j = 0; j < c.grid_cols; j++) {
            GridRect r;
            r.x = j == 0 ? 0 : j * C.grid_w - 3;
            r.y = i == 0 ? 0 : i * C.grid_h - 3;
            int gw = (j == c.grid_cols - 1) ? res_w : C.grid_w, gh = (i == c.grid_rows - 1) ? res_h : C.grid_h;
            r.w = gw + ((j > 0 && j < c.grid_cols - 1) ? 6 : 3);
            r.h = gh + ((i > 0 && i < c.grid_rows - 1) ? 6 : 3);
            if (c.grid_cols == 1) r.w = gw;
            if (c.grid_rows == 1) r.h = gh;
            C.rect[i * c.grid_cols + j] = r;
        }
    circle_halfwidths(c.min_dist, C.circle_hw);
    C.NP = (c.max_cnt + C.ncells * (C.grids_threshold + 2) + 8 + 7) & ~7;
    if (C.NP > VIO_FAST_CAP) { g_err = "max_cnt too large for this build"; return VIO_EINVAL; }
    C.NL = c.max_landmarks < C.NP ? C.NP : c.max_landmarks;
    C.NL = (C.NL + 7) & ~7;
    C.lm_hash_size = 256;
    while (C.lm_hash_size < 2 * C.NL) C.lm_hash_size <<= 1;
    C.NRES = std::max(4 * C.NL, C.W * C.NP + 2 * C.NL);
    C.NRES = (C.NRES + 63) & ~63;
    C.NIMU = imu_capacity < 256 ? 256 : imu_capacity;
    C.P = 15 * (C.W + 1) + 7;
    C.NPRIOR = 6 * C.W + 16;
    C.LW = (C.P + 15) & ~15;
    int off = 0, sw = c.width, sh = c.height;
    C.lvl_w[0] = sw; C.lvl_h[0] = sh; C.lvl_off[0] = 0;
    for (int l = 1; l <= 3; l++) {
        sw = (sw + 1) / 2; sh = (sh + 1) / 2;
        C.lvl_w[l] = sw; C.lvl_h[l] = sh; C.lvl_off[l] = off;
        off += (sw * sh + 63) & ~63;
    }
    C.pyr_bytes = off;
    if (c.marg_exact < 0 || c.marg_exact > 2) { g_err = "marg_exact must be 0, 1 or 2"; return VIO_EINVAL; }
    if (c.equalize < 0 || c.equalize > 1) { g_err = "equalize must be 0 or 1"; return VIO_EINVAL; }
    C.MX = c.marg_exact == 1 ? std::min(15 + C.NP, 495) : (c.marg_exact == 2 ? 16 : 0);
    return VIO_OK;
}

static int create_group_streams(vio_batch *h, vio_batch::Group &g, bool partitioned) {
    if (g.solve_graph) { (void)hipGraphExecDestroy(g.solve_graph); g.solve_graph = nullptr; }
    if (g.stream) { (void)hipStreamDestroy(g.stream); g.stream = nullptr; }
    if (g.fe_stream) { (void)hipStreamDestroy(g.fe_stream); g.fe_stream = nullptr; }
    int n_cu = 0, dev = 0;
    if (hipGetDevice(&dev) != hipSuccess || hipDeviceGetAttribute(&n_cu, hipDeviceAttributeMultiprocessorCount, dev) != hipSuccess) n_cu = 0;
    const char *fe_cus_env = getenv("VIO_FE_CUS");
    const int fe_cus = fe_cus_env ? atoi(fe_cus_env) : (h->S <= 128 ? n_cu / 4 : 0);
    hipError_t e_fe, e_be;
    h->fe_partitioned = false;
    if (partitioned && n_cu >= 8 && n_cu <= 1024 && fe_cus > 0 && fe_cus < n_cu) {
        h->fe_partitioned = true;
        const int nw = (n_cu + 31) / 32;
        std::vector<uint32_t> mfe(nw, 0u), mbe(nw, 0u);
        const int ng = (int)h->groups.size(), gi = (int)(&g - &h->groups[0]);
        const bool split = getenv("VIO_BE_CU_SPLIT") && atoi(getenv("VIO_BE_CU_SPLIT")) != 0 && ng > 1 && (n_cu - fe_cus) / ng >= 1;
        const int per = (n_cu - fe_cus) / ng;
        const int b0 = split ? fe_cus + gi * per : fe_cus, b1 = split ? (gi == ng - 1 ? n_cu : b0 + per) : n_cu;
        for (int q = 0; q < n_cu; q++) {
            if (q < fe_cus) mfe[q >> 5] |= 1u << (q & 31);
            if (q >= b0 && q < b1) mbe[q >> 5] |= 1u << (q & 31);
        }
        e_fe = hipExtStreamCreateWithCUMask(&g.fe_stream, (uint32_t)nw, mfe.data());
        e_be = getenv("VIO_BE_CU_ALL") ? hipStreamCreate(&g.stream) : hipExtStreamCreateWithCUMask(&g.stream, (uint32_t)nw, mbe.data());
    } else {
        e_fe = hipStreamCreate(&g.fe_stream);
        e_be = hipStreamCreate(&g.stream);
    }
    if (e_be != hipSuccess || e_fe != hipSuccess) { g_err = "stream create failed"; return VIO_EDEVICE; }
    return VIO_OK;
}

vio_batch *vio_create(const vio_config *cfg, int n_seq, int imu_capacity) { return vio_create_on_device(cfg, n_seq, imu_capacity, -1); }
int vio_get_device(vio_batch *h) { return h ? h->device : VIO_EINVAL; }

vio_batch *vio_create_on_device(const vio_config *cfg, int n_seq, int imu_capacity, int device) {
    if (!cfg || n_seq < 1) { g_err = "bad arguments"; return nullptr; }
    int ndev = 0;
    if (hipGetDeviceCount(&ndev) != hipSuccess || ndev < 1) { g_err = "no HIP device (the product path has no CPU fallback)"; return nullptr; }
    if (device >= ndev) { g_err = "vio_create_on_device: no such HIP device"; return nullptr; }
    int caller_dev = 0;
    if (hipGetDevice(&caller_dev) != hipSuccess) { g_err = "hipGetDevice failed"; return nullptr; }
    vio_batch *h = new vio_batch();
    h->device = device < 0 ? caller_dev : device;
    DevGuard dev_guard(h);
    if (dev_guard.failed) { g_err = "vio_create_on_device: hipSetDevice failed"; delete h; return nullptr; }
    if (build_devcfg(cfg, imu_capacity, h->hc) != VIO_OK) { delete h; return nullptr; }
    h->hc.MXL = 0;
    h->hc.eig_one_wave = getenv("VIO_EIG_ONE_WAVE") ? (atoi(getenv("VIO_EIG_ONE_WAVE")) != 0) : 0;
    h->hc.eig_jacobi = getenv("VIO_MARG_EIG_JACOBI") ? (atoi(getenv("VIO_MARG_EIG_JACOBI")) != 0) : 0;
    if (h->hc.MX > 0) {
        hipFuncAttributes fa;
        int cap = 0;
        if (hipDeviceGetAttribute(&cap, hipDeviceAttributeMaxSharedMemoryPerBlock, h->device) != hipSuccess || cap <= 0) cap = 160 * 1024;
        if (hipFuncGetAttributes(&fa, (const void *)be_marg_exact_kernel) == hipSuccess) {
            const long avail = (long)cap - (long)fa.sharedSizeBytes - 256;
            int m = 0;
            while (m < 128 && (long)marg_exact_lds_bytes(m + 1) <= avail) m++;
            if (getenv("VIO_MARG_EIG_LDS")) m = std::min(m, std::max(0, atoi(getenv("VIO_MARG_EIG_LDS"))));
            h->hc.MXL = m;
        }
    }
    h->S = n_seq;
    const DevCfg &C = h->hc;
    const size_t S = (size_t)n_seq, NP = C.NP, NL = C.NL, W1 = C.W + 1, HW = (size_t)C.c.width * C.c.height;
    Batch &B = h->B;
    memset(&B, 0, sizeof(B));
    B.S = n_seq;
    int rc = VIO_OK;
#define DA(ptr, n) if (rc == VIO_OK) rc = dalloc(h, &ptr, (size_t)(n))
    DA(B.cfg, 1); DA(B.fe, S); DA(B.be, S); DA(B.pre, S * (C.W + 2));
    static_assert(sizeof(vio_calibration) % alignof(vio_camera) == 0, "camera table alignment");
    DA(h->d_cal, S * (sizeof(vio_calibration) + sizeof(vio_camera)) / sizeof(vio_calibration) + 1); B.cal = h->d_cal;
    h->d_cam = (vio_camera *)(h->d_cal + S);
    DA(B.img, S * 2 * HW); DA(B.pyr, S * 2 * (size_t)C.pyr_bytes);
    if (C.c.equalize) { DA(B.clahe_lut, S * 64 * 256); DA(B.clahe_img, S * HW); }
    DA(B.cur_pts, S * NP); DA(B.forw_pts, S * NP); DA(B.cur_un_pts, S * NP); DA(B.pts_velocity, S * NP); DA(B.prev_un_pt, S * NP);
    DA(B.unstable_pts, S * NP); DA(B.tmp_pts, S * NP);
    DA(B.ids, S * NP); DA(B.track_cnt, S * NP); DA(B.prev_un_id, S * NP); DA(B.tmp_i0, S * NP); DA(B.tmp_i1, S * NP);
    DA(B.lk_status, S * NP); DA(B.accept_xy, S * 2 * NP); DA(B.cand, S * C.ncells * VIO_FAST_CAP);
    DA(B.obs_id, S * NP); DA(B.obs, S * NP * 7);
    DA(B.imu_t, S * C.NIMU); DA(B.imu_acc, S * C.NIMU * 3); DA(B.imu_gyr, S * C.NIMU * 3);
    DA(B.lm_id, S * NL); DA(B.lm_start, S * NL); DA(B.lm_nobs, S * NL); DA(B.lm_est_flag, S * NL); DA(B.lm_solve_flag, S * NL);
    DA(B.lm_dyn, S * NL); DA(B.lm_order, S * NL); DA(B.lm_free, S * NL); DA(B.lm_tmp, S * NL); DA(B.lm_pidx, S * NL); DA(B.lm_aidx, S * NL);
    DA(B.lm_depth, S * NL); DA(B.lm_obs, S * NL * W1 * VIO_OBS_D); DA(B.para_feat, S * NL); DA(B.cand_feat, S * NL);
    DA(B.lm_relo, S * NL); DA(B.relo_xy, S * NL * 2); DA(B.relo_mp, S * NP * 3);
    const size_t n = C.NPRIOR, LW = C.LW, nres = C.NRES, npair = W1 * W1, mq = 15 + n;
    DA(B.prior_J, S * n * n); DA(B.prior_r, S * n); DA(B.prior_x0, S * (C.W * 7 + 17)); DA(B.prior_H, S * n * n); DA(B.prior_rf, S * n);
    DA(B.H, S * LW * LW); DA(B.Sc, S * LW * LW); DA(B.Hpl, 2 * S * (NL + 8) * LW); DA(B.vec, S * VEC_SLOTS * LW);
    DA(B.Hll, 2 * S * (NL + 8)); DA(B.gl, 2 * S * (NL + 8)); DA(B.lvec, S * (NL + 8) * 8);
    if (C.W <= PS_FUSE_MAXW) DA(B.pairpart, S * PS_FUSE_MAXPAIRS * PS_FUSE_MAXBLK * 210);
    DA(B.ls_scratch, S * ps_eval_lds_bytes(C.W));
    DA(B.res, S * nres * 42); DA(B.res_lm, S * nres); DA(B.res_k, S * nres); DA(B.res_pair, S);
    DA(B.pair_start, S * (npair + 1)); DA(B.pair_list, S * nres); DA(B.pairblk, S * npair * 210);
    DA(B.imu_raw, S * C.W * 15 * 31);
    DA(B.margA, S * mq * mq); DA(B.margB, S * mq); DA(B.margV, S * n * n); DA(B.margW, S * (n + 16) * (n + 16));
    if (C.MX > 0) DA(B.margE, S * ((size_t)3 * C.MX * C.MX + n * (size_t)C.MX));
    DA(B.odom, S * 11); DA(B.timings, 128); DA(B.fe_ticks, S * 4);
    if (C.c.estimate_extrinsic == 2) { DA(h->hc.exc, S); DA(h->hc.exh, S * (size_t)VIO_EXCALIB_CAP * VIO_EXCALIB_PAIR_D); }
    B.hist_cap = 2048;
    B.s0 = 0;
    B.ns = 0; B.xcd_nb = 0; B.xcd_n = 8;
    if (getenv("VIO_BE_THREADS")) h->be_threads = std::min(1024, std::max(64, atoi(getenv("VIO_BE_THREADS")) & ~63));
    if (getenv("VIO_ASM_B_MODE")) h->asm_b_by_blocks = std::max(0, std::min(2, atoi(getenv("VIO_ASM_B_MODE"))));
    h->ps_asm_b_blocks = h->hc.W <= 10 ? 12 : 24;
    if (getenv("VIO_ASM_B_BLOCKS")) h->ps_asm_b_blocks = std::max(1, std::min(256, atoi(getenv("VIO_ASM_B_BLOCKS"))));
    if (getenv("VIO_EVAL_OCC")) h->eval_occ = atoi(getenv("VIO_EVAL_OCC"));
    if (getenv("VIO_GRAPH")) h->use_graph = atoi(getenv("VIO_GRAPH")) != 0;
    if (getenv("VIO_XCD_MAP")) h->xcd_map = atoi(getenv("VIO_XCD_MAP"));
    if (getenv("VIO_FE_XCD_MAP")) h->fe_xcd_map = atoi(getenv("VIO_FE_XCD_MAP"));
    if (getenv("VIO_XCD_N")) h->xcd_n = atoi(getenv("VIO_XCD_N"));
    if (getenv("VIO_FEED_THROTTLE")) h->feed_throttle = atoi(getenv("VIO_FEED_THROTTLE")) != 0;
    if (getenv("VIO_UPLOADS_IN_FLIGHT")) h->uploads_in_flight = atoi(getenv("VIO_UPLOADS_IN_FLIGHT")) == 1 ? 1 : 2;
    if (getenv("VIO_EXTRA_SLOTS")) h->extra_slots = std::max(1, atoi(getenv("VIO_EXTRA_SLOTS")));
    if (getenv("VIO_ASM_A_OCC")) h->asm_a_occ4 = atoi(getenv("VIO_ASM_A_OCC")) >= 4;
    if (getenv("VIO_MARG_THREADS")) h->marg_threads = std::min(512, std::max(64, atoi(getenv("VIO_MARG_THREADS")) & ~63));
    B.flags = getenv("VIO_FLAGS") ? atoi(getenv("VIO_FLAGS")) : 0;
    DA(B.odom_hist, S * (size_t)B.hist_cap * 11); DA(B.odom_count, S);
    DA(B.sst, S);
    DA(h->d_stamps, S); DA(h->d_modes, S); DA(h->d_rrel, S * 9); DA(h->d_r9, 16);
    DA(h->d_in_n, S); DA(h->d_in_stamps, S); DA(h->d_in_ids, S * NP); DA(h->d_in_obs, S * NP * 7);
#undef DA
    B.gW = h->hc.W; B.gP = h->hc.P; B.gLW = h->hc.LW; B.gNL = h->hc.NL; B.gNP = h->hc.NP; B.gNRES = h->hc.NRES; B.gNPRIOR = h->hc.NPRIOR; B.gMX = h->hc.MX;
    if (rc == VIO_OK && hipMemcpy(B.cfg, &h->hc, sizeof(DevCfg), hipMemcpyHostToDevice) != hipSuccess) { g_err = "cfg upload failed"; rc = VIO_EDEVICE; }
    if (rc == VIO_OK) {
        int per = getenv("VIO_GROUP_SEQS") ? atoi(getenv("VIO_GROUP_SEQS")) : n_seq;
        if (per < 1) per = 1;
        if (C.c.dynamic_init) per = n_seq;
        int ng = (n_seq + per - 1) / per;
        if (ng > 16) { ng = 16; per = (n_seq + ng - 1) / ng; ng = (n_seq + per - 1) / per; }
        h->groups.resize(ng);
        for (int k = 0; k < ng && rc == VIO_OK; k++) {
            vio_batch::Group &g = h->groups[k];
            g.s0 = k * per;
            g.n = std::min(per, n_seq - g.s0);
            if (create_group_streams(h, g, false) != VIO_OK) { rc = VIO_EDEVICE; break; }
            if (hipEventCreateWithFlags(&g.ev_solve, hipEventDisableTiming) != hipSuccess || hipEventCreateWithFlags(&g.ev_fe, hipEventDisableTiming) != hipSuccess ||
                hipEventCreateWithFlags(&g.ev_be, hipEventDisableTiming) != hipSuccess || hipEventCreateWithFlags(&g.ev_ingest, hipEventDisableTiming) != hipSuccess) { g_err = "event create failed"; rc = VIO_EDEVICE; }
        }
        if (rc == VIO_OK) { h->stream = h->groups[0].stream; h->fe_stream = h->groups[0].fe_stream; }
        if (rc == VIO_OK && hipEventCreateWithFlags(&h->ev_imu, hipEventDisableTiming) != hipSuccess) { g_err = "event create failed"; rc = VIO_EDEVICE; }
    }
    if (rc == VIO_OK && C.c.dynamic_init) {
        h->dyn.assign(n_seq, vio_batch::DynSeq());
        h->dyn_active = true;
        if (hipHostMalloc((void **)&h->h_state, sizeof(int) * n_seq, hipHostMallocDefault) != hipSuccess || hipMalloc((void **)&h->d_state, sizeof(int) * n_seq) != hipSuccess ||
            hipEventCreateWithFlags(&h->ev_state, hipEventDisableTiming) != hipSuccess) { g_err = "dynamic-init state allocation failed"; rc = VIO_EDEVICE; }
    }
    for (int i = 0; i < 4 && rc == VIO_OK; i++)
        if (hipEventCreate(&h->ev[i]) != hipSuccess) { g_err = "event create failed"; rc = VIO_EDEVICE; }
    if (rc == VIO_OK) {
        vio_calibration k;
        cal_from_config(C.c, k);
        h->cal.assign(n_seq, k);
        if (hipMemcpy(h->d_cal, h->cal.data(), sizeof(vio_calibration) * n_seq, hipMemcpyHostToDevice) != hipSuccess) { g_err = "calibration upload failed"; rc = VIO_EDEVICE; }
        vio_camera m = pinhole_camera(k);
        h->cam.assign(n_seq, m);
        if (rc == VIO_OK && hipMemcpy(h->d_cam, h->cam.data(), sizeof(vio_camera) * n_seq, hipMemcpyHostToDevice) != hipSuccess) { g_err = "camera upload failed"; rc = VIO_EDEVICE; }
    }
    if (rc == VIO_OK) { h->last_imu_t.assign(n_seq, -1e300); rc = init_state(h, 0, n_seq); }
    if (rc == VIO_OK) for (auto &g : h->groups) (void)hipEventRecord(g.ev_be, g.stream);
    if (rc == VIO_OK) {
        h->lds_select = (size_t)C.NP * 104 + 260 * 4 + 64;
        h->lds_add = (size_t)C.NP * 16 + (size_t)4 * 192 * 8  + 3 * VIO_FAST_CAP * 4 + 260 * 4 + 64 * 4 + (size_t)C.NP * 12 + 64;
        h->lds_fast = 0;
        for (int k = 0; k < C.ncells; k++) h->lds_fast = std::max(h->lds_fast, fast_lds_bytes(C.rect[k].w, C.rect[k].h));
        {
            size_t npairs = (size_t)(C.W + 1) * C.W / 2;
            size_t workd = std::max((size_t)C.W * 450, npairs * 210 <= 12288 ? npairs * 210 : (size_t)0);
            workd = std::max(workd, (size_t)1400 );
            workd = std::max(workd, (size_t)4 * 336);
            workd = std::max(workd, ((size_t)(C.W + 1) * (C.W + 1) + 1) * 32);
            if (C.NPRIOR <= 96) workd = std::max(workd, (size_t)C.NPRIOR * (C.NPRIOR | 1) + 2);
            {
                size_t nb = (size_t)C.LW >> 4, tiles = nb * (nb + 1) / 2 * 256;
                if (tiles <= 16896) workd = std::max(workd, tiles);
            }
            h->lds_solve = ((size_t)C.LW + 2 + workd) * 8 + 16;
            (void)raise_lds_limit((const void *)be_solve_kernel, (size_t)(h->lds_solve));
            (void)raise_lds_limit((const void *)be_solve_kernel_512, (size_t)(h->lds_solve));
            {
                const size_t nb = (size_t)C.LW >> 4, tiles = nb * (nb + 1) / 2 * 256;
                const size_t wk = std::max(tiles <= 16896 ? tiles : (2 * nb + 1) * 256, (size_t)16 * 336);
                h->serial_big = tiles > 16896;
                h->B.form_s = (getenv("VIO_FORM_S") ? atoi(getenv("VIO_FORM_S")) != 0 : true) && h->asm_b_by_blocks == 2;
                h->lds_serial = ((size_t)C.LW + 2 + wk + 2 + (size_t)14  * C.LW) * 8 + 16;
                if (getenv("VIO_SERIAL_LDS") && (size_t)atol(getenv("VIO_SERIAL_LDS")) > h->lds_serial) h->lds_serial = (size_t)atol(getenv("VIO_SERIAL_LDS"));
                (void)raise_lds_limit(h->serial_big ? (const void *)ps_serial_big_kernel : (const void *)ps_serial_kernel_512, h->lds_serial);
            }
            {
                const size_t nb = (size_t)C.LW >> 4, tiles = nb * (nb + 1) / 2 * 256, W1 = (size_t)C.W + 1;
                const bool eligible = !(B.flags & 1) && (size_t)C.W * C.NP / 256 + 4 <= PS_MAX_EVAL_BLOCKS &&
                                      (size_t)C.W * 768 <= (W1 * W1 - W1 * C.W / 2) * 210 && nb <= 32;
                h->solve_mode = getenv("VIO_SOLVE_MODE") ? atoi(getenv("VIO_SOLVE_MODE")) : 1;
                if (!eligible) h->solve_mode = 0;
                h->lds_ps_eval = ps_eval_lds_bytes(C.W);
                (void)raise_lds_limit((const void *)ps_eval_kernel, h->lds_ps_eval);
                h->lds_ps_evalf = ps_evalf_lds_bytes(C.W);
                {
                    const int want = getenv("VIO_FUSE") ? atoi(getenv("VIO_FUSE")) : 0;
                    int chunks = (int)std::min<size_t>(PS_FUSE_MAXBLK, (W1 * (size_t)C.c.max_cnt * 11 / 10 + (PS_FUSE_CAP - C.W) - 1) / (PS_FUSE_CAP - C.W));
                    if (want > 1) chunks = std::min(PS_FUSE_MAXBLK, want);
                    B.fuse = (want && C.W <= PS_FUSE_MAXW && C.c.use_imu && B.pairpart) ? std::max(1, chunks) : 0;
                    if (B.fuse && raise_lds_limit((const void *)ps_evalf_kernel, h->lds_ps_evalf) != 0) B.fuse = 0;
                    h->ps_evalf_blocks = 2 + B.fuse;
                }
                h->lds_ps_ls = ps_ls_lds_bytes(C.W);
                (void)raise_lds_limit((const void *)ps_ls_kernel, h->lds_ps_ls);
                h->line_search = !(C.c.reference_quirks & VIO_QUIRK_BOUND_CLAMP_ONLY) && !(getenv("VIO_LINE_SEARCH") && atoi(getenv("VIO_LINE_SEARCH")) == 0);
                (void)raise_lds_limit((const void *)ps_eval_kernel_occ3, h->lds_ps_eval);
                (void)raise_lds_limit((const void *)ps_eval_kernel_occ4, h->lds_ps_eval);
                B.eval_rpt = getenv("VIO_EVAL_RPT") ? std::max(1, std::min(4, atoi(getenv("VIO_EVAL_RPT")))) : 2;
                h->ps_eval_blocks = (int)std::min<size_t>(PS_MAX_EVAL_BLOCKS, (size_t)C.W * C.NP / (256 * (size_t)B.eval_rpt) + 4);
                h->ps_asm_a_blocks = (int)((W1 * (W1 - 1) / 2 + C.W + 32 + 7) / 8);
                int nact = 0;
                for (size_t a = 0; a < nb; a++) for (size_t b2 = 0; b2 <= a; b2++) {
                    auto act = [&](size_t cb) { const size_t c0 = 16 * cb, c1 = c0 + 15; return c0 < 6 * W1 || (c1 >= 15 * W1 && c0 < 15 * W1 + 7); };
                    if (act(a) && act(b2)) nact++;
                }
                h->ps_schur_tiles = nact;
                h->B.n_schur = nact;
                h->B.gn_ext = getenv("VIO_GN_EXT") ? (atoi(getenv("VIO_GN_EXT")) != 0) : 1;
            }
        }
        {
            size_t nbq = ((size_t)C.NPRIOR + 15) >> 4;
            h->lds_marg = std::max(std::max((size_t)nbq * (nbq + 1) / 2 * 2048, (size_t)2 * C.NPRIOR * 15 * 8), (size_t)PREINT_MANY_LDS_DOUBLES * 8) + 64;
            if (C.MXL > 0) h->lds_marg = std::max(h->lds_marg, marg_exact_lds_bytes(C.MXL));
            if (C.MX > 0) h->lds_marg = std::max(h->lds_marg, (size_t)7 * 512 * 8 + 64);
            h->lds_factor = C.NPRIOR <= 96 ? (size_t)C.NPRIOR * (C.NPRIOR | 1) * 8 + 64 : 64;
            (void)raise_lds_limit((const void *)be_prior_factor_kernel, h->lds_factor);
        }
        (void)raise_lds_limit((const void *)be_marg_kernel, (size_t)(h->lds_marg));
        (void)raise_lds_limit((const void *)be_marg_exact_kernel, (size_t)(h->lds_marg));
        const bool excalib = C.c.estimate_extrinsic == 2;
        const void *ingest = excalib ? (const void *)be_ingest_kernel<true> : (const void *)be_ingest_kernel<false>;
        (void)raise_lds_limit(ingest, ingest_lds_bytes(C, excalib));

        (void)raise_lds_limit((const void *)fe_select_kernel, (size_t)(h->lds_select));
        (void)raise_lds_limit((const void *)fe_add_kernel, (size_t)(h->lds_add));
        (void)raise_lds_limit((const void *)fe_fast_kernel, (size_t)(h->lds_fast));
        bool fits = lds_fits(C.MX > 0 ? (const void *)be_marg_exact_kernel : (const void *)be_marg_kernel, h->lds_marg, "be_marg") &&
                    lds_fits(ingest, ingest_lds_bytes(C, excalib), "be_ingest") &&
                    lds_fits((const void *)fe_select_kernel, h->lds_select, "fe_select") && lds_fits((const void *)fe_add_kernel, h->lds_add, "fe_add") &&
                    lds_fits((const void *)fe_fast_kernel, h->lds_fast, "fe_fast");
        if (fits && h->solve_mode == 1)
            fits = lds_fits((const void *)ps_eval_kernel, h->lds_ps_eval, "ps_eval") && lds_fits((const void *)ps_ls_kernel, h->lds_ps_ls, "ps_ls") &&
                   lds_fits(h->serial_big ? (const void *)ps_serial_big_kernel : (const void *)ps_serial_kernel_512, h->lds_serial, "ps_serial");
        else if (fits)
            fits = lds_fits(h->be_threads <= 512 ? (const void *)be_solve_kernel_512 : (const void *)be_solve_kernel, h->lds_solve, "be_solve");
        if (!fits) rc = VIO_ECAPACITY;
    }
    if (rc != VIO_OK) { vio_destroy(h); return nullptr; }
    return h;
}

void vio_destroy(vio_batch *h) {
    if (!h) return;
    int caller_dev = -1;
    const bool dev_switched = h->device >= 0 && hipGetDevice(&caller_dev) == hipSuccess && caller_dev != h->device && hipSetDevice(h->device) == hipSuccess;
    (void)hipDeviceSynchronize();
    for (void *p : h->allocs) (void)hipFree(p);
    if (h->d_gray_stage) (void)hipFree(h->d_gray_stage);
    if (h->d_fisheye) (void)hipFree(h->d_fisheye);
    if (h->d_depth_stage) (void)hipFree(h->d_depth_stage);
    if (h->d_gray_stage1) (void)hipFree(h->d_gray_stage1);
    if (h->d_depth_stage1) (void)hipFree(h->d_depth_stage1);
    for (auto &sg : h->imu_stage) {
        if (sg.h_seq) {
            (void)hipHostFree(sg.h_seq); (void)hipHostFree(sg.h_t); (void)hipHostFree(sg.h_acc); (void)hipHostFree(sg.h_gyr);
            (void)hipFree(sg.d_seq); (void)hipFree(sg.d_t); (void)hipFree(sg.d_acc); (void)hipFree(sg.d_gyr);
        }
        if (sg.done) (void)hipEventDestroy(sg.done);
    }
    if (h->ev_imu) (void)hipEventDestroy(h->ev_imu);
    if (h->ev_state) (void)hipEventDestroy(h->ev_state);
    if (h->h_state) (void)hipHostFree(h->h_state);
    if (h->d_state) (void)hipFree(h->d_state);
    if (h->d_dyn_samples) (void)hipFree(h->d_dyn_samples);
    if (h->d_dyn_offs) (void)hipFree(h->d_dyn_offs);
    if (h->d_snap_tab) (void)hipFree(h->d_snap_tab);
    if (h->d_snap_seqs) (void)hipFree(h->d_snap_seqs);
    if (h->d_snap_stage) (void)hipFree(h->d_snap_stage);
    for (hipEvent_t e : h->pev) (void)hipEventDestroy(e);
    for (auto &g : h->groups) {
        if (g.stream) (void)hipStreamDestroy(g.stream);
        if (g.fe_stream) (void)hipStreamDestroy(g.fe_stream);
        if (g.ev_solve) (void)hipEventDestroy(g.ev_solve);
        if (g.ev_fe) (void)hipEventDestroy(g.ev_fe);
        if (g.ev_be) (void)hipEventDestroy(g.ev_be);
        if (g.ev_ingest) (void)hipEventDestroy(g.ev_ingest);
        if (g.solve_graph) (void)hipGraphExecDestroy(g.solve_graph);
        for (int p = 0; p < 2; p++) {
            if (g.ev_up_gray[p]) (void)hipEventDestroy(g.ev_up_gray[p]);
            if (g.ev_up_depth[p]) (void)hipEventDestroy(g.ev_up_depth[p]);
        }
        for (int p = 0; p < 2; p++) {
            if (g.ev_rd_gray[p]) (void)hipEventDestroy(g.ev_rd_gray[p]);
            if (g.ev_rd_depth[p]) (void)hipEventDestroy(g.ev_rd_depth[p]);
        }
        if (g.ev_host_fe) (void)hipEventDestroy(g.ev_host_fe);
        if (g.side_ring) { (void)hipHostFree(g.side_ring); for (auto e : g.side_ev) if (e) (void)hipEventDestroy(e); }
        if (g.ev_host_be) (void)hipEventDestroy(g.ev_host_be);
        if (g.copy_stream) (void)hipStreamDestroy(g.copy_stream);
        if (g.copy_stream2) (void)hipStreamDestroy(g.copy_stream2);
    }
    for (int i = 0; i < 4; i++) if (h->ev[i]) (void)hipEventDestroy(h->ev[i]);
    delete h;
    if (dev_switched) (void)hipSetDevice(caller_dev);
}

int vio_reset(vio_batch *h) {
    DevGuard dev_guard(h);
    if (dev_guard.failed) { g_err = "hipSetDevice failed for the handle's device"; return VIO_EDEVICE; }
    if (!h) return VIO_EINVAL;
    { int rc_ = sync_all(h); if (rc_ != VIO_OK) return rc_; }
    return init_state(h, 0, h->S);
}

int vio_reset_seq(vio_batch *h, int seq) {
    DevGuard dev_guard(h);
    if (dev_guard.failed) { g_err = "hipSetDevice failed for the handle's device"; return VIO_EDEVICE; }
    if (!h || seq < 0 || seq >= h->S) return VIO_EINVAL;
    { int rc_ = sync_all(h); if (rc_ != VIO_OK) return rc_; }
    { int rc_ = refresh_dynamic_state(h); if (rc_ != VIO_OK) return rc_; }
    return init_state(h, seq, seq + 1, VIO_RESET_ESTIMATOR);
}

int vio_reset_tracker_seq(vio_batch *h, int seq) {
    DevGuard dev_guard(h);
    if (dev_guard.failed) { g_err = "hipSetDevice failed for the handle's device"; return VIO_EDEVICE; }
    if (!h || seq < 0 || seq >= h->S) return VIO_EINVAL;
    { int rc_ = sync_all(h); if (rc_ != VIO_OK) return rc_; }
    return init_state(h, seq, seq + 1, VIO_RESET_TRACKER);
}

int vio_push_imu(vio_batch *h, int seq, int n, const double *t, const double *acc, const double *gyr) {
    DevGuard dev_guard(h);
    if (dev_guard.failed) { g_err = "hipSetDevice failed for the handle's device"; return VIO_EDEVICE; }
    if (!h || seq < 0 || seq >= h->S || n < 0) return VIO_EINVAL;
    std::lock_guard<std::mutex> lk(h->imu_mu);
    for (int i = 0; i < n; i++) {
        if (!(t[i] > h->last_imu_t[seq])) continue;
        h->last_imu_t[seq] = t[i];
        h->p_seq.push_back(seq);
        h->p_t.push_back(t[i]);
        for (int k = 0; k < 3; k++) { h->p_acc.push_back(acc[3 * i + k]); h->p_gyr.push_back(gyr[3 * i + k]); }
    }
    return VIO_OK;
}

static int note_stage_read(hipEvent_t &ev, bool &have, hipStream_t st) {
    if (!ev) HIPCHK(hipEventCreateWithFlags(&ev, hipEventDisableTiming));
    HIPCHK(hipEventRecord(ev, st));
    have = true;
    return VIO_OK;
}

static int stage_inputs(vio_batch *h, vio_batch::Group &g, const uint8_t *gray, const uint16_t *depth, const double *stamps, int on_device,
                        const uint8_t **dg, const uint16_t **dd, bool overlap = false) {
    const DevCfg &C = h->hc;
    size_t HW = (size_t)C.c.width * C.c.height, S = h->S, s0 = g.s0, n = g.n;
    if (stamps) HIPCHK(hipMemcpyAsync(h->d_stamps + s0, stamps + s0, n * sizeof(double), hipMemcpyHostToDevice, g.fe_stream));
    if (on_device) { *dg = gray; *dd = depth; return VIO_OK; }
    const int p = overlap ? g.flip : 0;
    if (overlap && !g.copy_stream) {
        HIPCHK(hipStreamCreate(&g.copy_stream));
        if (!(getenv("VIO_COPY_STREAMS") && atoi(getenv("VIO_COPY_STREAMS")) == 1)) HIPCHK(hipStreamCreate(&g.copy_stream2));
        for (int q = 0; q < 2; q++) {
            HIPCHK(hipEventCreateWithFlags(&g.ev_up_gray[q], hipEventDisableTiming));
            HIPCHK(hipEventCreateWithFlags(&g.ev_up_depth[q], hipEventDisableTiming));
        }
    }
    static const bool si_trace = getenv("VIO_FEED_TRACE") && atoi(getenv("VIO_FEED_TRACE")) != 0;
    auto si_now = []() { return std::chrono::duration<double, std::micro>(std::chrono::steady_clock::now().time_since_epoch()).count(); };
    const double si0 = si_trace ? si_now() : 0;
    if (overlap && g.up_used[p]) {
        HIPCHK(hipEventSynchronize(g.ev_up_gray[p]));
        HIPCHK(hipEventSynchronize(g.ev_up_depth[p]));
    }
    if (overlap && h->uploads_in_flight == 1 && g.up_used[p ^ 1]) {
        HIPCHK(hipEventSynchronize(g.ev_up_gray[p ^ 1]));
        HIPCHK(hipEventSynchronize(g.ev_up_depth[p ^ 1]));
    }
    if (overlap && h->feed_throttle && g.have_rd_depth[p]) {
        HIPCHK(hipEventSynchronize(g.ev_rd_depth[p]));
    }
    if (overlap) g.up_used[p] = true;
    const double si1 = si_trace ? si_now() : 0;
    if (gray) {
        uint8_t *&buf = p ? h->d_gray_stage1 : h->d_gray_stage;
        if (!buf) HIPCHK(hipMalloc((void **)&buf, S * HW));
        if (overlap) {
            if (g.have_rd_gray[p]) HIPCHK(hipStreamWaitEvent(g.copy_stream, g.ev_rd_gray[p], 0));
            HIPCHK(hipMemcpyAsync(buf + s0 * HW, gray + s0 * HW, n * HW, hipMemcpyHostToDevice, g.copy_stream));
// ... 595 lines not shown
        {"fx", &k.fx, 1}, {"fy", &k.fy, 1}, {"cx", &k.cx, 1}, {"cy", &k.cy, 1}, {"k1", &k.k1, 1}, {"k2", &k.k2, 1}, {"p1", &k.p1, 1},
        {"p2", &k.p2, 1}, {"ric", k.ric, 9}, {"tic", k.tic, 3}, {"td", &k.td, 1}, {"tr", &k.tr, 1}, {"acc_n", &k.acc_n, 1},
        {"acc_w", &k.acc_w, 1}, {"gyr_n", &k.gyr_n, 1}, {"gyr_w", &k.gyr_w, 1}, {"g_norm", &k.g_norm, 1}};
    for (const auto &f : fin)
        for (int i = 0; i < f.n; i++)
            if (!std::isfinite(f.v[i])) return std::string(f.name) + " is not finite";
    const struct { const char *name; double v; } pos[] = {
        {"fx", k.fx}, {"fy", k.fy}, {"acc_n", k.acc_n}, {"acc_w", k.acc_w}, {"gyr_n", k.gyr_n}, {"gyr_w", k.gyr_w}, {"g_norm", k.g_norm}};
    for (const auto &f : pos)
        if (!(f.v > 0)) return std::string(f.name) + " must be > 0";
    if (!(k.tr >= 0)) return "tr must be >= 0";
    {
        double err = 0;
        for (int i = 0; i < 3; i++)
            for (int j = 0; j < 3; j++) {
                double d = (i == j) ? -1.0 : 0.0;
                for (int q = 0; q < 3; q++) d += k.ric[3 * i + q] * k.ric[3 * j + q];
                err = std::max(err, std::fabs(d));
            }
        const double *R = k.ric;
        const double det = R[0] * (R[4] * R[8] - R[5] * R[7]) - R[1] * (R[3] * R[8] - R[5] * R[6]) + R[2] * (R[3] * R[7] - R[4] * R[6]);
        if (!(err <= 1e-6) || !(det > 0)) return "ric is not a rotation (orthonormal within 1e-6, determinant +1)";
    }
    return "";
}

int vio_set_calibration(vio_batch *h, int seq, const vio_calibration *cal) {
    DevGuard dev_guard(h);
    if (dev_guard.failed) { g_err = "hipSetDevice failed for the handle's device"; return VIO_EDEVICE; }
    if (!h || !cal) { g_err = "vio_set_calibration: bad arguments"; return VIO_EINVAL; }
    if (seq < 0 || seq >= h->S) { g_err = "vio_set_calibration: seq out of range"; return VIO_EINVAL; }
    const vio_calibration &k = *cal;
    const std::string why = calibration_check(k);
    if (!why.empty()) { g_err = "vio_set_calibration: " + why; return VIO_EINVAL; }
    vio_calibration e = k;
    if (h->hc.c.estimate_extrinsic == 2) {
        dm::stm(e.ric, dm::eye());
        for (int i = 0; i < 3; i++) e.tic[i] = 0;
    } else {
        ortho_ric(k.ric, e.ric);
    }
    { int rc_ = sync_all(h); if (rc_ != VIO_OK) return rc_; }
    { int rc_ = refresh_dynamic_state(h); if (rc_ != VIO_OK) return rc_; }
    HIPCHK(hipMemcpy(h->d_cal + seq, &e, sizeof(vio_calibration), hipMemcpyHostToDevice));
    h->cal[seq] = e;
    return init_state(h, seq, seq + 1);
}

int vio_get_calibration(vio_batch *h, int seq, vio_calibration *out) {
    if (!h || !out || seq < 0 || seq >= h->S) { g_err = "vio_get_calibration: bad arguments"; return VIO_EINVAL; }
    *out = h->cal[seq];
    return VIO_OK;
}

static std::string camera_check(const vio_camera &m, int width, int height) {
    static const char *const names[3][9] = {{"fx", "fy", "cx", "cy", "k1", "k2", "p1", "p2", nullptr},
                                            {"k2", "k3", "k4", "k5", "mu", "mv", "u0", "v0", nullptr},
                                            {"xi", "k1", "k2", "p1", "p2", "gamma1", "gamma2", "u0", "v0"}};
    if (m.model < VIO_CAMERA_PINHOLE || m.model > VIO_CAMERA_MEI) return "model is not VIO_CAMERA_PINHOLE, _KANNALA_BRANDT or _MEI";
    if (m.reserved != 0) return "reserved must be 0";
    const char *const *nm = names[m.model];
    for (int i = 0; i < 12; i++)
        if (!std::isfinite(m.p[i])) return std::string(i < 9 && nm[i] ? nm[i] : "p[" + std::to_string(i) + "]") + " is not finite";
    const int pos[3][2] = {{0, 1}, {4, 5}, {5, 6}};
    for (int j = 0; j < 2; j++)
        if (!(m.p[pos[m.model][j]] > 0)) return std::string(nm[pos[m.model][j]]) + " must be > 0";
    if (m.model == VIO_CAMERA_MEI && !(m.p[0] >= 0)) return "xi must be >= 0";
    const double W1 = width - 1, H1 = height - 1;
    const double pts[8][2] = {{0, 0}, {W1, 0}, {0, H1}, {W1, H1}, {W1 / 2, 0}, {W1 / 2, H1}, {0, H1 / 2}, {W1, H1 / 2}};
    for (const auto &q : pts) {
        double x, y, z;
        vcam::lift(m, q[0], q[1], x, y, z);
        if (!(std::isfinite(x) && std::isfinite(y) && std::isfinite(z) && z > 0)) {
            char b[160];
            snprintf(b, sizeof(b), "pixel (%g, %g) does not lift to a finite ray in front of the camera (z = %g): the field of view reaches 90 degrees",
                     q[0], q[1], z);
            return b;
        }
    }
    return "";
}

int vio_set_camera(vio_batch *h, int seq, const vio_camera *cam) {
    DevGuard dev_guard(h);
    if (dev_guard.failed) { g_err = "hipSetDevice failed for the handle's device"; return VIO_EDEVICE; }
    if (!h || !cam) { g_err = "vio_set_camera: bad arguments"; return VIO_EINVAL; }
    if (seq < 0 || seq >= h->S) { g_err = "vio_set_camera: seq out of range"; return VIO_EINVAL; }
    const std::string why = camera_check(*cam, h->hc.c.width, h->hc.c.height);
    if (!why.empty()) { g_err = "vio_set_camera: " + why; return VIO_EINVAL; }
    vio_camera m = *cam;
    vio_calibration k = h->cal[seq];
    if (m.model == VIO_CAMERA_PINHOLE) {
        k.fx = m.p[0]; k.fy = m.p[1]; k.cx = m.p[2]; k.cy = m.p[3]; k.k1 = m.p[4]; k.k2 = m.p[5]; k.p1 = m.p[6]; k.p2 = m.p[7];
        m = pinhole_camera(k);
    }
    { int rc_ = sync_all(h); if (rc_ != VIO_OK) return rc_; }
    { int rc_ = refresh_dynamic_state(h); if (rc_ != VIO_OK) return rc_; }
    HIPCHK(hipMemcpy(h->d_cal + seq, &k, sizeof(vio_calibration), hipMemcpyHostToDevice));
    HIPCHK(hipMemcpy(h->d_cam + seq, &m, sizeof(vio_camera), hipMemcpyHostToDevice));
    h->cal[seq] = k;
    h->cam[seq] = m;
    return init_state(h, seq, seq + 1);
}

int vio_get_camera(vio_batch *h, int seq, vio_camera *out) {
    if (!h || !out || seq < 0 || seq >= h->S) { g_err = "vio_get_camera: bad arguments"; return VIO_EINVAL; }
    *out = h->cam[seq].model == VIO_CAMERA_PINHOLE ? pinhole_camera(h->cal[seq]) : h->cam[seq];
    return VIO_OK;
}

static void snapshot_build_layout(vio_batch *h) {
    if (!h->snap_rows.empty()) return;
    const DevCfg &C = h->hc;
    const Batch &B = h->B;
    const int64_t NP = C.NP, NL = C.NL, W1 = C.W + 1, HW = (int64_t)C.c.width * C.c.height, n = C.NPRIOR, LW = C.LW, nres = C.NRES, npair = W1 * W1, mq = 15 + n;
    std::vector<vio_batch::SnapRow> &R = h->snap_rows;
#define ROW(kind, name, ptr, count) R.push_back({name, kind, (unsigned char *)(ptr), (ptr) ? (int64_t)(count) * (int64_t)sizeof(*(ptr)) : 0, -1})
#define STATE(member, count) ROW(1, #member, B.member, count)
#define SCRATCH(member, count) ROW(0, #member, B.member, count)
#define HANDLE(name) R.push_back({name, 2, nullptr, 0, -1})
    HANDLE("cfg"); HANDLE("S"); HANDLE("s0 ns xcd_nb xcd_n"); HANDLE("tracker_lag (header)"); HANDLE("eval_rpt");
    STATE(fe, 1); STATE(be, 1);
    ROW(1, "cal", h->d_cal, 1); ROW(1, "cam (cam_of)", h->d_cam, 1);
    STATE(pre, C.W + 2);
    STATE(img, 2 * HW); STATE(pyr, 2 * (int64_t)C.pyr_bytes);
    SCRATCH(clahe_lut, 64 * 256); SCRATCH(clahe_img, HW);
    HANDLE("fisheye");
    STATE(cur_pts, NP); STATE(forw_pts, NP); STATE(cur_un_pts, NP); STATE(pts_velocity, NP); STATE(prev_un_pt, NP); STATE(unstable_pts, NP);
    SCRATCH(tmp_pts, NP);
    STATE(ids, NP); STATE(track_cnt, NP); STATE(prev_un_id, NP);
    SCRATCH(tmp_i0, NP); SCRATCH(tmp_i1, NP);
    STATE(lk_status, NP); STATE(accept_xy, 2 * NP);
    SCRATCH(cand, (int64_t)C.ncells * VIO_FAST_CAP);
    STATE(obs_id, NP); STATE(obs, NP * 7);
    STATE(imu_t, C.NIMU); STATE(imu_acc, (int64_t)C.NIMU * 3); STATE(imu_gyr, (int64_t)C.NIMU * 3);
    STATE(lm_id, NL); STATE(lm_start, NL); STATE(lm_nobs, NL); STATE(lm_est_flag, NL); STATE(lm_solve_flag, NL); STATE(lm_dyn, NL);
    STATE(lm_order, NL); STATE(lm_free, NL);
    SCRATCH(lm_tmp, NL);
    STATE(lm_pidx, NL); STATE(lm_aidx, NL);
    STATE(lm_depth, NL); STATE(lm_obs, NL * W1 * VIO_OBS_D);
    STATE(lm_relo, NL); STATE(relo_xy, NL * 2); STATE(relo_mp, NP * 3);
    STATE(para_feat, NL);
    SCRATCH(cand_feat, NL);
    SCRATCH(prior_J, n * n);
    STATE(prior_r, n); STATE(prior_x0, C.W * 7 + 17); STATE(prior_H, n * n);
    SCRATCH(prior_rf, n);
    SCRATCH(H, LW * LW); SCRATCH(Sc, LW * LW); SCRATCH(Hpl, 2 * (NL + 8) * LW); SCRATCH(vec, VEC_SLOTS * LW);
    SCRATCH(Hll, 2 * (NL + 8)); SCRATCH(gl, 2 * (NL + 8)); SCRATCH(lvec, (NL + 8) * 8);
    SCRATCH(res, nres * 42); SCRATCH(res_pair, 1); SCRATCH(res_lm, nres); SCRATCH(res_k, nres);
    SCRATCH(pair_start, npair + 1); SCRATCH(pair_list, nres); SCRATCH(pairblk, npair * 210);
    SCRATCH(ls_scratch, (int64_t)ps_eval_lds_bytes(C.W)); SCRATCH(pairpart, (int64_t)PS_FUSE_MAXPAIRS * PS_FUSE_MAXBLK * 210);
    HANDLE("gW gP gLW gNL gNP gNRES gNPRIOR gMX"); HANDLE("gn_ext n_schur form_s fuse fuse_only");
    SCRATCH(imu_raw, (int64_t)C.W * 15 * 31);
    SCRATCH(margA, mq * mq); SCRATCH(margB, mq); SCRATCH(margV, n * n); SCRATCH(margW, (n + 16) * (n + 16));
    SCRATCH(margE, (int64_t)3 * C.MX * C.MX + n * (int64_t)C.MX);
    STATE(odom, 11); STATE(odom_hist, (int64_t)B.hist_cap * 11); STATE(odom_count, 1);
    HANDLE("hist_cap (shape key)"); HANDLE("flags");
    HANDLE("timings");
    SCRATCH(fe_ticks, 4);
    STATE(sst, 1);
    ROW(1, "DevCfg::exc", C.exc, 1); ROW(1, "DevCfg::exh", C.exh, (int64_t)VIO_EXCALIB_CAP * VIO_EXCALIB_PAIR_D);
    R.push_back({"host: last_imu_t", 1, nullptr, (int64_t)sizeof(double), -1});
    R.push_back({"host: dyn (DynSeq, variable)", 1, nullptr, 0, -1});
    R.push_back({"host: p_seq p_t p_acc p_gyr (flushed by save, dropped by load)", 0, nullptr, 0, -1});
#undef ROW
#undef STATE
#undef SCRATCH
#undef HANDLE
    int64_t off = 0, chunks = 0;
    int ne = 0;
    for (auto &r : R)
        if (r.kind == 1 && r.base && r.bytes > 0) { r.blob_off = off; off += (r.bytes + 15) & ~(int64_t)15; chunks += (r.bytes + 15) >> 4; ne++; }
    h->snap_dev_bytes = off; h->snap_chunks = chunks; h->snap_entries = ne;
}
static const vio_batch::SnapRow *snapshot_row(const vio_batch *h, const char *name) {
    for (const auto &r : h->snap_rows) if (!strcmp(r.name, name)) return &r;
    return nullptr;
}
static void snapshot_handle_shape(const vio_batch *h, vio_snapshot_shape *k) {
    (void)vio_shape_key(&h->hc.c, h->hc.NIMU, k);
    k->hist_cap = h->B.hist_cap;
}

struct SnapHostFixed { double last_imu_t; int32_t has_dyn, n_frames; double initial_timestamp; int32_t nonlinear, attempts, failures, last_stage; double pad; };
struct SnapFrameFixed { double stamp; int32_t n_ids, n_dt; double lin_acc[3], lin_gyr[3], bg_lin[3]; };
static_assert(sizeof(SnapHostFixed) == 48 && sizeof(SnapFrameFixed) == 88, "snapshot host records");
static int64_t snapshot_host_bytes(const vio_batch *h, int seq) {
    int64_t b = sizeof(SnapHostFixed);
    if (!h->dyn.empty())
        for (const auto &f : h->dyn[seq].frames)
            b += (int64_t)sizeof(SnapFrameFixed) + (((int64_t)f.ids.size() + 1) & ~(int64_t)1) * 4 + (int64_t)(f.xy.size() + f.dt.size() + f.acc.size() + f.gyr.size()) * 8;
    return (b + 15) & ~(int64_t)15;
}
static void snapshot_write_host(const vio_batch *h, int seq, unsigned char *p, int64_t bytes) {
    memset(p, 0, (size_t)bytes);
    SnapHostFixed hf;
    memset(&hf, 0, sizeof(hf));
    hf.last_imu_t = h->last_imu_t[seq];
    if (!h->dyn.empty()) {
        const vio_batch::DynSeq &D = h->dyn[seq];
        hf.has_dyn = 1; hf.n_frames = (int32_t)D.frames.size(); hf.initial_timestamp = D.initial_timestamp;
        hf.nonlinear = D.nonlinear ? 1 : 0; hf.attempts = D.attempts; hf.failures = D.failures; hf.last_stage = D.last_stage;
    }
    memcpy(p, &hf, sizeof(hf)); p += sizeof(hf);
    if (h->dyn.empty()) return;
    for (const auto &f : h->dyn[seq].frames) {
        SnapFrameFixed ff;
        memset(&ff, 0, sizeof(ff));
        ff.stamp = f.stamp; ff.n_ids = (int32_t)f.ids.size(); ff.n_dt = (int32_t)f.dt.size();
        for (int k = 0; k < 3; k++) { ff.lin_acc[k] = f.lin_acc[k]; ff.lin_gyr[k] = f.lin_gyr[k]; ff.bg_lin[k] = f.bg_lin[k]; }
        memcpy(p, &ff, sizeof(ff)); p += sizeof(ff);
        if (!f.ids.empty()) memcpy(p, f.ids.data(), f.ids.size() * 4);
        p += ((f.ids.size() + 1) & ~(size_t)1) * 4;
        auto put = [&](const std::vector<double> &v) { if (!v.empty()) memcpy(p, v.data(), v.size() * 8); p += v.size() * 8; };
        put(f.xy); put(f.dt); put(f.acc); put(f.gyr);
    }
}
static std::string snapshot_read_host(const unsigned char *p, int64_t bytes, bool want_dyn, int NP, double *last_imu_t, vio_batch::DynSeq *D) {
    const unsigned char *end = p + bytes;
    SnapHostFixed hf;
    if (bytes < (int64_t)sizeof(hf)) return "host_bytes: the host part is shorter than its fixed record";
    memcpy(&hf, p, sizeof(hf)); p += sizeof(hf);
    if ((hf.has_dyn != 0) != want_dyn) return "dynamic_init: the host part does not match the handle";
    if (hf.n_frames < 0 || (!hf.has_dyn && hf.n_frames != 0)) return "host part: bad image-frame count";
    if (last_imu_t) *last_imu_t = hf.last_imu_t;
    if (D) { *D = vio_batch::DynSeq(); D->initial_timestamp = hf.initial_timestamp; D->nonlinear = hf.nonlinear != 0; D->attempts = hf.attempts; D->failures = hf.failures; D->last_stage = hf.last_stage; }
    for (int i = 0; i < hf.n_frames; i++) {
        SnapFrameFixed ff;
        if (end - p < (int64_t)sizeof(ff)) return "host_bytes: an image frame runs past the end of the blob";
        memcpy(&ff, p, sizeof(ff)); p += sizeof(ff);
        if (ff.n_ids < 0 || ff.n_ids > NP || ff.n_dt < 0 || ff.n_dt > VIO_IMU_SLOT_CAP) return "host part: image frame counts out of range";
        const int64_t need = (((int64_t)ff.n_ids + 1) & ~(int64_t)1) * 4 + ((int64_t)2 * ff.n_ids + (int64_t)7 * ff.n_dt) * 8;
        if (end - p < need) return "host_bytes: an image frame runs past the end of the blob";
        if (D) {
            vinit::ImageFrame f;
            f.stamp = ff.stamp;
            for (int k = 0; k < 3; k++) { f.lin_acc[k] = ff.lin_acc[k]; f.lin_gyr[k] = ff.lin_gyr[k]; f.bg_lin[k] = ff.bg_lin[k]; }
            const unsigned char *q = p;
            f.ids.resize(ff.n_ids);
            if (ff.n_ids) memcpy(f.ids.data(), q, (size_t)ff.n_ids * 4);
            q += (((size_t)ff.n_ids + 1) & ~(size_t)1) * 4;
            auto get = [&](std::vector<double> &v, size_t cnt) { v.resize(cnt); if (cnt) memcpy(v.data(), q, cnt * 8); q += cnt * 8; };
            get(f.xy, (size_t)2 * ff.n_ids); get(f.dt, (size_t)ff.n_dt); get(f.acc, (size_t)3 * ff.n_dt); get(f.gyr, (size_t)3 * ff.n_dt);
            D->frames.push_back(std::move(f));
        }
        p += need;
    }
    return "";
}

static int snapshot_quiesce(vio_batch *h, bool flush) {
    if (flush) { int rc = flush_imu_backend(h); if (rc != VIO_OK) return rc; }
    { int rc = sync_all(h); if (rc != VIO_OK) return rc; }
    return refresh_dynamic_state(h);
}
static int snapshot_reserve(vio_batch *h, size_t count, size_t stage_bytes) {
    snapshot_build_layout(h);
    if (!h->d_snap_tab) {
        std::vector<SnapEntry> tab;
        int64_t c0 = 0;
        for (const auto &r : h->snap_rows)
            if (r.blob_off >= 0) { tab.push_back({r.base, r.bytes, r.bytes, r.blob_off, c0}); c0 += (r.bytes + 15) >> 4; }
        HIPCHK(hipMalloc((void **)&h->d_snap_tab, tab.size() * sizeof(SnapEntry)));
        HIPCHK(hipMemcpy(h->d_snap_tab, tab.data(), tab.size() * sizeof(SnapEntry), hipMemcpyHostToDevice));
    }
    if (count > h->snap_seqs_cap) {
        if (h->d_snap_seqs) { (void)hipFree(h->d_snap_seqs); h->d_snap_seqs = nullptr; h->snap_seqs_cap = 0; }
        HIPCHK(hipMalloc((void **)&h->d_snap_seqs, count * sizeof(SnapSeq)));
        h->snap_seqs_cap = count;
    }
    if (stage_bytes > h->snap_stage_cap) {
        if (h->d_snap_stage) { (void)hipFree(h->d_snap_stage); h->d_snap_stage = nullptr; h->snap_stage_cap = 0; }
        HIPCHK(hipMalloc((void **)&h->d_snap_stage, stage_bytes));
        h->snap_stage_cap = stage_bytes;
    }
    return VIO_OK;
}
static bool snapshot_place(int n, const int64_t *offsets, const std::vector<int64_t> &bytes, std::vector<int64_t> &pos, int64_t *span) {
    bool tight = true;
    for (int i = 0; i + 1 < n; i++) tight = tight && offsets[i + 1] == offsets[i] + bytes[i];
    for (int i = 0; i < n; i++) tight = tight && (bytes[i] & 15) == 0;
    pos.resize(n);
    int64_t at = 0;
    for (int i = 0; i < n; i++) { pos[i] = at; at += (bytes[i] + 15) & ~(int64_t)15; }
    *span = at;
    return tight;
}
static int snapshot_launch(vio_batch *h, int n, const int32_t *seqs, const std::vector<int64_t> &pos, bool pack) {
    std::vector<SnapSeq> list;
    std::vector<std::pair<int, int>> runs;
    for (auto &g : h->groups) {
        const int first = (int)list.size();
        for (int i = 0; i < n; i++)
            if (seqs[i] >= g.s0 && seqs[i] < g.s0 + g.n) list.push_back({pos[i] + (int64_t)sizeof(vio_snapshot_header), seqs[i], 0});
        runs.push_back({first, (int)list.size() - first});
    }
    HIPCHK(hipMemcpy(h->d_snap_seqs, list.data(), list.size() * sizeof(SnapSeq), hipMemcpyHostToDevice));
    const unsigned gx = (unsigned)((h->snap_chunks + SNAP_THREADS - 1) / SNAP_THREADS);
    for (size_t k = 0; k < h->groups.size(); k++) {
        if (runs[k].second == 0) continue;
        const dim3 grid(gx, (unsigned)runs[k].second);
        if (pack) snap_pack_kernel<<<grid, SNAP_THREADS, 0, h->groups[k].stream>>>(h->d_snap_tab, h->snap_entries, h->snap_chunks, h->d_snap_seqs + runs[k].first, h->d_snap_stage);
        else snap_unpack_kernel<<<grid, SNAP_THREADS, 0, h->groups[k].stream>>>(h->d_snap_tab, h->snap_entries, h->snap_chunks, h->d_snap_seqs + runs[k].first, h->d_snap_stage);
    }
    HIPCHK(hipGetLastError());
    for (size_t k = 0; k < h->groups.size(); k++) if (runs[k].second) HIPCHK(hipStreamSynchronize(h->groups[k].stream));
    return VIO_OK;
// ... 624 lines not shown
```

Before: 60330 frames/s.

## Split marginalization into multi-workgroup kernels with MFMA Schur accumulation

The single-block-per-sequence marginalization kernel becomes a pipeline of wide kernels: landmark record/row evaluation and prior/IMU setup spread over several workgroups, frame blocks and rank updates computed as f64 MFMA tiles parked in scratch, a multi-workgroup scatter into the dense system, then a tail kernel for the factorization and finish. The aim is to raise parallelism for the marginalization stage, which previously ran on one block per sequence. It adds three extra launches, global-memory round trips for intermediate buffers, and a larger margW allocation. The new path is enabled by default and can be turned off with an environment variable.

New measurement: 60770 frames/s, median of 6. About the same (+0.7%).

```diff
diff --git a/vins-rgbd-fast_amd/csrc/be_kernels.hip b/vins-rgbd-fast_amd/csrc/be_kernels.hip
--- a/vins-rgbd-fast_amd/csrc/be_kernels.hip
+++ b/vins-rgbd-fast_amd/csrc/be_kernels.hip
@@ -1662,7 +1662,7 @@
 
 }
 
-template <bool EXACT> __device__ void marg_body(const Batch &B, int s, int *scratch, double *sred, unsigned char *smem_marg);
+template <bool EXACT, bool WIDE> __device__ void marg_body(const Batch &B, int s, int *scratch, double *sred, unsigned char *smem_marg);
 __device__ void finish_body(const Batch &B, int s, int *scratch, PreWork &pw, unsigned char *smem_marg);
 
 __device__ __forceinline__ void solve_body(const Batch &B, int s, int *scratch, double *sred, unsigned char *smem, PreWork &pw);
@@ -1689,7 +1689,7 @@
     __shared__ double sred[64];
     __shared__ PreWork pw;
     extern __shared__ __attribute__((aligned(16))) unsigned char smem[];
-    marg_body<false>(B, s, scratch, sred, smem);
+    marg_body<false, false>(B, s, scratch, sred, smem);
     __syncthreads();
     finish_body(B, s, scratch, pw, smem);
 }
@@ -1699,7 +1699,7 @@
     __shared__ double sred[64];
     __shared__ PreWork pw;
     extern __shared__ __attribute__((aligned(16))) unsigned char smem[];
-    marg_body<true>(B, s, scratch, sred, smem);
+    marg_body<true, false>(B, s, scratch, sred, smem);
     __syncthreads();
     finish_body(B, s, scratch, pw, smem);
 }
@@ -2199,13 +2199,385 @@
     if (VIO_TIMERS && t == 0) be.dbg[10] = (int)(VIO_CLOCK() - tx0);
 }
 
-template <bool EXACT> __device__ void marg_body(const Batch &B, int s, int *scratch, double *sred, unsigned char *smem_marg) {
+
+__device__ __forceinline__ bool marg_runs(const Ctx &c, const BeSeq &be) {
+    if (!be.do_marg || be.rebooted || be.frame_count < c.W) return false;
+    if (be.marginalization_flag != 0 && !(be.has_prior && be.prior_present[c.W - 1])) return false;
+    return true;
+}
+__device__ __forceinline__ void marg_load_state(const BeSeq &be, int W, Params &X) {
+    const int t = threadIdx.x;
+    if (t <= W) {
+        int i = t;
+        X.pose[i * 7 + 0] = be.Ps[i][0]; X.pose[i * 7 + 1] = be.Ps[i][1]; X.pose[i * 7 + 2] = be.Ps[i][2];
+        quat q = R2q(ldm(be.Rs[i]));
+        X.pose[i * 7 + 3] = q.x; X.pose[i * 7 + 4] = q.y; X.pose[i * 7 + 5] = q.z; X.pose[i * 7 + 6] = q.w;
+        for (int k = 0; k < 3; k++) { X.sb[i * 9 + k] = be.Vs[i][k]; X.sb[i * 9 + 3 + k] = be.Bas[i][k]; X.sb[i * 9 + 6 + k] = be.Bgs[i][k]; }
+    }
+    if (t == W + 1) {
+        X.ex[0] = be.tic[0]; X.ex[1] = be.tic[1]; X.ex[2] = be.tic[2];
+        quat q = R2q(ldm(be.ric));
+        X.ex[3] = q.x; X.ex[4] = q.y; X.ex[5] = q.z; X.ex[6] = q.w;
+        X.td = be.td;
+    }
+}
+__device__ __forceinline__ void marg_prior_phase(const Ctx &c, const BeSeq &be, const Params &X, double *sdx, double *srp, double *A, double *b, int md, int mq,
+                                                 bool second_new) {
+    const int t = threadIdx.x, nt = blockDim.x;
+    const int W = c.W, n = c.NPR;
+    const int rS = md + 6 * W, rE = md + 6 * W + 9, rT = md + 6 * W + 15;
+    for (int i = t; i < mq * mq; i += nt) A[i] = 0;
+    for (int i = t; i < mq; i += nt) b[i] = 0;
+    __syncthreads();
+    if (!be.has_prior) return;
+    prior_dx(c, X, sdx);
+    for (int i = t; i < n; i += nt) {
+        double sacc = c.prior_r[i];
+        for (int j0 = 0; j0 < n; j0 += 32) {
+            double hv[32];
+#pragma unroll
+            for (int u = 0; u < 32; u++) hv[u] = c.prior_H[(size_t)min(j0 + u, n - 1) * n + i];
+#pragma unroll
+            for (int u = 0; u < 32; u++) if (j0 + u < n) sacc += hv[u] * sdx[j0 + u];
+        }
+        srp[i] = sacc;
+    }
+    __syncthreads();
+    auto pmap = [&](int a) -> int {
+        if (a < 6 * W) {
+            int k = a / 6, d = a - 6 * k;
+            if (second_new) return k == W - 1 ? d : md + 6 * k + d;
+            return k == 0 ? d : md + 6 * (k - 1) + d;
+        }
+        if (a < 6 * W + 9) return second_new ? rS + (a - 6 * W) : 6 + (a - 6 * W);
+        if (a < 6 * W + 15) return rE + (a - 6 * W - 9);
+        return rT;
+    };
+    for (int w0 = t; w0 < n * n; w0 += 8 * nt) {
+        double pv[8];
+#pragma unroll
+        for (int u = 0; u < 8; u++) pv[u] = c.prior_H[min(w0 + u * nt, n * n - 1)];
+#pragma unroll
+        for (int u = 0; u < 8; u++) {
+            const int w = w0 + u * nt;
+            if (w < n * n) { const int a = w / n, bb = w - a * n; A[pmap(a) * mq + pmap(bb)] = 0.0 + pv[u]; }
+        }
+    }
+    for (int a = t; a < n; a += nt) b[pmap(a)] += srp[a];
+    __syncthreads();
+}
+__device__ __forceinline__ bool marg_imu_used(const Ctx &c, const BeSeq &be) { return c.C->c.use_imu && c.pre[be.pre_idx[1]].sum_dt < 10.0; }
+__device__ __forceinline__ void marg_imu_phase(const Ctx &c, const BeSeq &be, const Params &X, double *A, double *b, int md, int mq) {
+    const int t = threadIdx.x, nt = blockDim.x;
+    const int rS = md + 6 * c.W;
+    PreInt &p1 = c.pre[be.pre_idx[1]];
+    if (!marg_imu_used(c, be)) return;
+    double *Jw = c.pairblk;
+    double *raw = c.imu_raw;
+    if ((t & 63) == 0) for (int part = t >> 6; part < 5; part += nt >> 6) {
+        v3 G = ld3(be.g);
+        if (part == 0) {
+            double r15[15];
+            bf::imu_raw_residual(p1, G, &X.pose[0], &X.sb[0], &X.pose[7], &X.sb[9], r15);
+            for (int r = 0; r < 15; r++) {
+                double sacc = 0;
+                for (int k = 0; k <= r; k++) sacc += p1.sqrt_info[r * 15 + k] * r15[k];
+                raw[r * 31 + 30] = sacc;
+            }
+        } else
+            bf::imu_raw_jacobian_part(p1, G, &X.pose[0], &X.sb[0], &X.pose[7], &X.sb[9], part - 1, raw, 31);
+    }
+    __syncthreads();
+    for (int w = t; w < 450; w += nt) {
+        int r = w / 30, col = w - r * 30;
+        double sacc = 0;
+        for (int k = 0; k <= r; k++) sacc += p1.sqrt_info[r * 15 + k] * raw[k * 31 + col];
+        Jw[w] = sacc;
+    }
+    __syncthreads();
+    for (int w = t; w < 930; w += nt) {
+        int a = w / 31, bb = w - a * 31;
+        int ia = a < 15 ? a : (a < 21 ? md + (a - 15) : rS + (a - 21));
+        double sacc = 0;
+        if (bb < 30) {
+            int ib = bb < 15 ? bb : (bb < 21 ? md + (bb - 15) : rS + (bb - 21));
+            for (int k = 0; k < 15; k++) sacc += Jw[k * 30 + a] * Jw[k * 30 + bb];
+            A[ia * mq + ib] += sacc;
+        } else {
+            for (int k = 0; k < 15; k++) sacc += Jw[k * 30 + a] * raw[k * 31 + 30];
+            b[ia] += sacc;
+        }
+    }
+    __syncthreads();
+}
+__device__ __forceinline__ int marg_lm_list(const Ctx &c, const BeSeq &be, int *scratch) {
+    const int t = threadIdx.x, nt = blockDim.x;
+    const int nlm = be.n_lm;
+    int *flag = c.lm_tmp, *offs = c.res_k;
+    for (int k = t; k < nlm; k += nt) { int slot = c.lm_order[k]; flag[k] = (in_problem(c, slot) && c.lm_start[slot] == 0) ? 1 : 0; }
+    __syncthreads();
+    int F0 = block_scan_flags(flag, nlm, offs, scratch);
+    int *list0 = c.pair_list;
+    for (int k = t; k < nlm; k += nt) if (flag[k]) list0[offs[k]] = c.lm_order[k];
+    __syncthreads();
+    return F0;
+}
+__device__ __forceinline__ int marg_lm_count(const Ctx &c, const BeSeq &be) {
+    const int nlm = be.n_lm;
+    return nlm > 0 ? c.res_k[nlm - 1] + c.lm_tmp[nlm - 1] : 0;
+}
+#define MARG_GEO_DOUBLES ((VIO_MAXW + 1) * 32 + 16)
+__device__ __forceinline__ void marg_pair_geo(const Params &X, int W, double *mgeo) {
+    const int t = threadIdx.x;
+    if (t >= 1 && t <= W) {
+        bf::PairGeo g;
+        bf::pair_geo(&X.pose[0], &X.pose[t * 7], X.ex, g);
+        double *o = mgeo + (size_t)(t - 1) * 32;
+        for (int q = 0; q < 9; q++) { o[q] = g.A1[q]; o[9 + q] = g.A2[q]; o[18 + q] = g.M[q]; }
+        o[27] = g.t[0]; o[28] = g.t[1]; o[29] = g.t[2];
+    }
+    if (t == 0) stm(mgeo + (size_t)W * 32, q2R(mkq(X.ex[6], X.ex[3], X.ex[4], X.ex[5])));
+}
+__device__ __forceinline__ void marg_lm_records(const Ctx &c, const Params &X, const double *mgeo, int lo, int hi) {
+    const int t = threadIdx.x, nt = blockDim.x;
+    const vio_config &cfg = c.C->c;
+    const int W = c.W, per = W;
+    const int *list0 = c.pair_list;
+    for (int w = lo * per + t; w < hi * per; w += nt) {
+        int li = w / per, k = w - li * per + 1;
+        int slot = list0[li];
+        double *out = c.res + (size_t)w * 42;
+        if (k >= c.lm_nobs[slot]) { out[40] = 0; out[41] = 0; for (int q = 0; q < 40; q++) out[q] = 0; continue; }
+        double rr[2], wgt = 1.0;
+        const double inv_dep = 1.0 / c.lm_depth[slot];
+        const bf::PairGeo &g = *(const bf::PairGeo *)(mgeo + (size_t)(k - 1) * 32);
+        bf::eval_projection_pair(cfg, g, mgeo + (size_t)W * 32, X.ex, inv_dep, X.td, c.K->tr, obs_ptr(c, slot, 0), obs_ptr(c, slot, k), cfg.estimate_td != 0, rr, out,
+                                 true, &wgt);
+        out[40] = wgt * rr[0];
+        out[41] = wgt * rr[1];
+    }
+}
+__device__ __forceinline__ void marg_lm_rows(const Ctx &c, int md, int lo, int hi, bool pinv) {
+    const int t = threadIdx.x, nt = blockDim.x;
+    const vio_config &cfg = c.C->c;
+    const int W = c.W, per = W, ldc = c.LW;
+    const int rE = md + 6 * W + 9, rT = md + 6 * W + 15;
+    const double eps = 1e-8;
+    const int *list0 = c.pair_list;
+    double *Cl = c.Hpl;
+    for (int w = lo * ldc + t; w < hi * ldc; w += nt) Cl[w] = 0;
+    __syncthreads();
+    const int grp = t >> 4, gln = t & 15, ngrp = nt >> 4;
+    for (int li0 = lo; li0 < hi; li0 += ngrp) {
+        const int li = li0 + grp;
+        const bool act = li < hi;
+        const int no = act ? c.lm_nobs[list0[li]] : 0;
+        double cm[13], dsum = 0, bsum = 0;
+#pragma unroll
+        for (int q = 0; q < 13; q++) cm[q] = 0;
+        for (int k = gln + 1; k < no; k += 16) {
+            const double *Jg = c.res + (size_t)(li * per + k - 1) * 42;
+            double Jr[42];
+#pragma unroll
+            for (int q = 0; q < 42; q++) Jr[q] = Jg[q];
+            const double jl0 = Jr[19], jl1 = Jr[39];
+#pragma unroll
+            for (int q = 0; q < 6; q++) {
+                cm[q] += Jr[q] * jl0 + Jr[20 + q] * jl1;
+                cm[6 + q] += Jr[12 + q] * jl0 + Jr[32 + q] * jl1;
+                Cl[(size_t)li * ldc + md + 6 * (k - 1) + q] = Jr[6 + q] * jl0 + Jr[26 + q] * jl1;
+            }
+            if (cfg.estimate_td) cm[12] += Jr[18] * jl0 + Jr[38] * jl1;
+            dsum += jl0 * jl0 + jl1 * jl1;
+            bsum += jl0 * Jr[40] + jl1 * Jr[41];
+        }
+#pragma unroll
+        for (int off = 8; off >= 1; off >>= 1) {
+#pragma unroll
+            for (int q = 0; q < 13; q++) cm[q] += __shfl_xor(cm[q], off, 16);
+            dsum += __shfl_xor(dsum, off, 16);
+            bsum += __shfl_xor(bsum, off, 16);
+        }
+        if (act && gln == 0) {
+#pragma unroll
+            for (int q = 0; q < 6; q++) { Cl[(size_t)li * ldc + q] = cm[q]; Cl[(size_t)li * ldc + rE + q] = cm[6 + q]; }
+            if (cfg.estimate_td) Cl[(size_t)li * ldc + rT] = cm[12];
+            c.Hll[li] = pinv ? (dsum > eps ? 1.0 / dsum : 0.0) : dsum;
+            c.gl[li] = bsum;
+        }
+    }
+    __syncthreads();
+}
+__device__ __forceinline__ void marg_frame_block(const Ctx &c, int j, int F0c) {
+    const int lane = threadIdx.x & 63, li = lane & 15, lk = lane >> 4;
+    const int per = c.W;
+    v4f64 a00 = {0, 0, 0, 0}, a10 = {0, 0, 0, 0}, a11 = {0, 0, 0, 0};
+    const int K = 2 * F0c;
+    for (int k0 = 0; k0 < K; k0 += 64) {
+        double x0[16], x1[16];
+#pragma unroll
+        for (int u = 0; u < 16; u++) {
+            int kk = k0 + 4 * u + lk;
+            bool valid = kk < K;
+            int lm = min(kk, K - 1) >> 1, sub = kk & 1;
+            const double *Jr = c.res + (size_t)(lm * per + j - 1) * 42;
+            double v0 = Jr[sub * 20 + li];
+            double v1 = Jr[li < 3 ? sub * 20 + 16 + li : 40 + sub];
+            x0[u] = valid ? v0 : 0.0;
+            x1[u] = (valid && li < 4) ? v1 : 0.0;
+        }
+#pragma unroll
+        for (int u = 0; u < 16; u++) {
+            if (k0 + 16 * (u >> 2) >= K) break;
+            a00 = __builtin_amdgcn_mfma_f64_16x16x4f64(x0[u], x0[u], a00, 0, 0, 0);
+            a10 = __builtin_amdgcn_mfma_f64_16x16x4f64(x1[u], x0[u], a10, 0, 0, 0);
+            a11 = __builtin_amdgcn_mfma_f64_16x16x4f64(x1[u], x1[u], a11, 0, 0, 0);
+        }
+    }
+    double *out = c.pairblk + (size_t)(j - 1) * 210;
+#pragma unroll
+    for (int r = 0; r < 4; r++) {
+        int row = lk + 4 * r, col = li;
+        if (col <= row) out[sym_idx(col, row)] = a00[r];
+        if (row < 4) out[sym_idx(col, 16 + row)] = a10[r];
+        if (row < 4 && col < 4 && col <= row) out[sym_idx(16 + col, 16 + row)] = a11[r];
+    }
+}
+#define MARG_QMAP_LEN (6 * VIO_MAXW + 40)
+__device__ __forceinline__ void marg_qmap(const Ctx &c, int md, int mq, signed char *qfr, signed char *qlc) {
+    const int W = c.W, rE = md + 6 * W + 9, rT = md + 6 * W + 15;
+    for (int a = threadIdx.x; a <= mq; a += blockDim.x) {
+        int fr = -1, lc = 0;
+        if (a == mq) { fr = 0; lc = 19; }
+        else if (a < 6) { fr = 0; lc = a; }
+        else if (a >= md && a < md + 6 * W) { fr = (a - md) / 6 + 1; lc = 6 + (a - md) % 6; }
+        else if (a >= rE && a < rE + 6) { fr = 0; lc = 12 + (a - rE); }
+        else if (a == rT && c.C->c.estimate_td) { fr = 0; lc = 18; }
+        qfr[a] = (signed char)fr; qlc[a] = (signed char)lc;
+    }
+}
+__device__ __forceinline__ void marg_sub_part(const Ctx &c, int F0c, int mq, bool with, double *sp, int sp_ld, int tid, int nthr) {
+    const double *Cl = c.Hpl;
+    const int ldc = c.LW;
+    for (int w = tid; w < 4 * mq; w += nthr) {
+        const int ch = w / mq, a = w - ch * mq;
+        double acc = 0;
+        if (with) for (int li = ch; li < F0c; li += 4) acc += Cl[(size_t)li * ldc + a] * (c.gl[li] * c.Hll[li]);
+        sp[ch * sp_ld + a] = acc;
+    }
+}
+__device__ __forceinline__ void marg_scatter(const Ctx &c, double *A, double *b, int mq, const signed char *qfr, const signed char *qlc, const double *sp, int sp_ld,
+                                             int tid, int nthr) {
+    const int W = c.W, nt = nthr;
+    for (int w0 = tid; w0 < mq * (mq + 1); w0 += 4 * nt) {
+        bool use[4], multi[4], rhs[4];
+        int dst[4], row[4], sidx[4];
+        double pv[4], av[4];
+#pragma unroll
+        for (int u = 0; u < 4; u++) {
+            const int w = min(w0 + u * nt, mq * (mq + 1) - 1);
+            const int a = w / (mq + 1), bb = w - a * (mq + 1);
+            const int fa = qfr[a], fb = qfr[bb];
+            const int la = qlc[a], lb = qlc[bb];
+            use[u] = w0 + u * nt < mq * (mq + 1) && fa >= 0 && fb >= 0 && !(fa > 0 && fb > 0 && fa != fb);
+            multi[u] = use[u] && fa == 0 && fb == 0;
+            rhs[u] = bb == mq; row[u] = a; dst[u] = a * mq + bb;
+            sidx[u] = sym_idx(la, lb);
+            const int f1 = fa > 0 ? fa : (fb > 0 ? fb : 1);
+            pv[u] = use[u] ? c.pairblk[(size_t)(f1 - 1) * 210 + sidx[u]] : 0.0;
+            av[u] = use[u] ? (rhs[u] ? b[a] : A[dst[u]]) : 0.0;
+        }
+#pragma unroll
+        for (int u = 0; u < 4; u++) {
+            if (!use[u]) continue;
+            double sacc = pv[u];
+            if (multi[u]) {
+                double fv[VIO_MAXW];
+#pragma unroll
+                for (int j = 0; j < VIO_MAXW; j++) fv[j] = c.pairblk[(size_t)min(j, W - 1) * 210 + sidx[u]];
+                sacc = 0;
+#pragma unroll
+                for (int j = 0; j < VIO_MAXW; j++) if (j < W) sacc += fv[j];
+            }
+            if (!rhs[u]) A[dst[u]] = av[u] + sacc;
+            else b[row[u]] = av[u] + (sacc - ((sp[row[u]] + sp[sp_ld + row[u]]) + (sp[2 * sp_ld + row[u]] + sp[3 * sp_ld + row[u]])));
+        }
+    }
+}
+__device__ __forceinline__ void marg_rank_tile(const Ctx &c, int tile, int F0c, int mq, double *A, double *park) {
+    const int lane = threadIdx.x & 63, li = lane & 15, lk = lane >> 4;
+    const double *Cl = c.Hpl;
+    const int ldc = c.LW;
+    int ti, tj;
+    tri_decode(tile, ti, tj);
+    v4f64 acc = {0, 0, 0, 0};
+    const int ca = min(16 * ti + li, ldc - 1), cb = min(16 * tj + li, ldc - 1);
+    for (int k0 = 0; k0 < F0c; k0 += 64) {
+        double xa[16], xb[16];
+#pragma unroll
+        for (int u = 0; u < 16; u++) {
+            int kk = k0 + 4 * u + lk;
+            bool valid = kk < F0c;
+            int kc = min(kk, F0c - 1);
+            double va = Cl[(size_t)kc * ldc + ca], vb = Cl[(size_t)kc * ldc + cb], dinv = c.Hll[kc];
+            xa[u] = valid ? -(va * dinv) : 0.0;
+            xb[u] = valid ? vb : 0.0;
+        }
+#pragma unroll
+        for (int u = 0; u < 16; u++) {
+            if (k0 + 16 * (u >> 2) >= F0c) break;
+            acc = __builtin_amdgcn_mfma_f64_16x16x4f64(xa[u], xb[u], acc, 0, 0, 0);
+        }
+    }
+#pragma unroll
+    for (int r = 0; r < 4; r++) {
+        int row = 16 * ti + lk + 4 * r, col = 16 * tj + li;
+        if (park) park[(size_t)tile * 256 + 16 * (lk + 4 * r) + li] = acc[r];
+        else if (row < mq && col < mq && (ti != tj || col <= row)) {
+            A[row * mq + col] += acc[r];
+            if (row != col) A[col * mq + row] += acc[r];
+        }
+    }
+}
+__device__ __forceinline__ void marg_add_parked(double *A, int mq, const double *park, int tid, int nthr) {
+    for (int w = tid; w < mq * (mq + 1); w += nthr) {
+        const int a = w / (mq + 1), bb = w - a * (mq + 1);
+        if (bb == mq) continue;
+        const int row = max(a, bb), col = min(a, bb), ti = row >> 4, tj = col >> 4;
+        A[a * mq + bb] += park[(size_t)(ti * (ti + 1) / 2 + tj) * 256 + 16 * (row & 15) + (col & 15)];
+    }
+}
+__device__ __forceinline__ void marg_new_present(const Ctx &c, const BeSeq &be, bool second_new, int F0c, int *newpresent) {
+    const int t = threadIdx.x, nt = blockDim.x;
+    const int W = c.W;
+    if (t < W + 3) newpresent[t] = 0;
+    __syncthreads();
+    if (be.has_prior && t < W + 3) {
+        const int pres = be.prior_present[t];
+        if (t > W) { if (pres) newpresent[t] = 1; }
+        else if (second_new) { if (t < W - 1 || t == W) newpresent[t] = pres; }
+        else if (t >= 1 && t < W && pres) newpresent[t - 1] = 1;
+    }
+    __syncthreads();
+    if (!second_new) {
+        if (t == 0 && marg_imu_used(c, be)) { newpresent[0] = 1; newpresent[W] = 1; }
+        const int *list0 = c.pair_list;
+        for (int li = t; li < F0c; li += nt) {
+            int no = c.lm_nobs[list0[li]];
+            for (int k = 1; k < no; k++) newpresent[k - 1] = 1;
+            if (no > 1) { newpresent[W + 1] = 1; if (c.C->c.estimate_td) newpresent[W + 2] = 1; }
+        }
+    }
+    __syncthreads();
+}
+
+template <bool EXACT, bool WIDE> __device__ void marg_body(const Batch &B, int s, int *scratch, double *sred, unsigned char *smem_marg) {
     const int t = threadIdx.x, nt = blockDim.x;
     Ctx c = make_ctx(B, s);
     const DevCfg &C = *B.cfg;
     const vio_config &cfg = C.c;
     BeSeq &be = *c.be;
-    if (!be.do_marg || be.rebooted || be.frame_count < c.W) return;
+    if (!marg_runs(c, be)) return;
     const int W = c.W, W1 = W + 1, n = c.NPR;
     const double eps = 1e-8;
     __shared__ Params X;
@@ -2215,341 +2587,57 @@
     __shared__ double A15[225], V15[225], Pinv[225];
     __shared__ int newpresent[VIO_MAXW + 3];
     const bool second_new = be.marginalization_flag != 0;
-    if (second_new && !(be.has_prior && be.prior_present[W - 1])) return;
     const bool exact = EXACT && cfg.marg_exact == 1 && c.margE != nullptr;
     const bool lit2 = EXACT && cfg.marg_exact == 2;
     int F0x = 0;
     int F0k = 0;
     PH_INIT;
     const long long tk0 = VIO_CLOCK();
-    if (t <= W) {
-        int i = t;
-        X.pose[i * 7 + 0] = be.Ps[i][0]; X.pose[i * 7 + 1] = be.Ps[i][1]; X.pose[i * 7 + 2] = be.Ps[i][2];
-        quat q = R2q(ldm(be.Rs[i]));
-        X.pose[i * 7 + 3] = q.x; X.pose[i * 7 + 4] = q.y; X.pose[i * 7 + 5] = q.z; X.pose[i * 7 + 6] = q.w;
-        for (int k = 0; k < 3; k++) { X.sb[i * 9 + k] = be.Vs[i][k]; X.sb[i * 9 + 3 + k] = be.Bas[i][k]; X.sb[i * 9 + 6 + k] = be.Bgs[i][k]; }
-    }
-    if (t == W + 1) {
-        X.ex[0] = be.tic[0]; X.ex[1] = be.tic[1]; X.ex[2] = be.tic[2];
-        quat q = R2q(ldm(be.ric));
-        X.ex[3] = q.x; X.ex[4] = q.y; X.ex[5] = q.z; X.ex[6] = q.w;
-        X.td = be.td;
-    }
-    if (t < W + 3) newpresent[t] = 0;
+    marg_load_state(be, W, X);
     __syncthreads();
     if (t <= W) for (int k = 0; k < 7; k++) be.para_Pose[t][k] = X.pose[t * 7 + k];
     const int md = second_new ? 6 : 15;
     const int mq = md + n;
     double *A = c.margA, *b = c.margB;
-    for (int i = t; i < mq * mq; i += nt) A[i] = 0;
-    for (int i = t; i < mq; i += nt) b[i] = 0;
-    __syncthreads();
-    const int rS = md + 6 * W, rE = md + 6 * W + 9, rT = md + 6 * W + 15;
-    if (be.has_prior) {
-        prior_dx(c, X, sdx);
-        for (int i = t; i < n; i += nt) {
-            double sacc = c.prior_r[i];
-            for (int j0 = 0; j0 < n; j0 += 32) {
-                double hv[32];
-#pragma unroll
-                for (int u = 0; u < 32; u++) hv[u] = c.prior_H[(size_t)min(j0 + u, n - 1) * n + i];
-#pragma unroll
-                for (int u = 0; u < 32; u++) if (j0 + u < n) sacc += hv[u] * sdx[j0 + u];
-            }
-            srp[i] = sacc;
-        }
-        __syncthreads();
-        auto pmap = [&](int a) -> int {
-            if (a < 6 * W) {
-                int k = a / 6, d = a - 6 * k;
-                if (second_new) return k == W - 1 ? d : md + 6 * k + d;
-                return k == 0 ? d : md + 6 * (k - 1) + d;
-            }
-            if (a < 6 * W + 9) return second_new ? rS + (a - 6 * W) : 6 + (a - 6 * W);
-            if (a < 6 * W + 15) return rE + (a - 6 * W - 9);
-            return rT;
-        };
-        for (int w0 = t; w0 < n * n; w0 += 8 * nt) {
-            double pv[8];
-#pragma unroll
-            for (int u = 0; u < 8; u++) pv[u] = c.prior_H[min(w0 + u * nt, n * n - 1)];
-#pragma unroll
-            for (int u = 0; u < 8; u++) {
-                const int w = w0 + u * nt;
-                if (w < n * n) { const int a = w / n, bb = w - a * n; A[pmap(a) * mq + pmap(bb)] = 0.0 + pv[u]; }
-            }
-        }
-        for (int a = t; a < n; a += nt) b[pmap(a)] += srp[a];
-        if (t < W + 3) {
-            const int pres = be.prior_present[t];
-            if (t > W) { if (pres) newpresent[t] = 1; }
-            else if (second_new) { if (t < W - 1 || t == W) newpresent[t] = pres; }
-            else if (t >= 1 && t < W && pres) newpresent[t - 1] = 1;
-        }
-        __syncthreads();
-    }
+    if constexpr (WIDE) {
+        if (second_new) marg_prior_phase(c, be, X, sdx, srp, A, b, md, mq, second_new);
+        else F0k = min(marg_lm_count(c, be), c.nres_cap / W);
+    } else {
+    marg_prior_phase(c, be, X, sdx, srp, A, b, md, mq, second_new);
     PH(16);
     if (!second_new) {
-        PreInt &p1 = c.pre[be.pre_idx[1]];
-        if (cfg.use_imu && p1.sum_dt < 10.0) {
-            double *Jw = c.pairblk;
-            double *raw = c.imu_raw;
-            if ((t & 63) == 0) for (int part = t >> 6; part < 5; part += nt >> 6) {
-                v3 G = ld3(be.g);
-                if (part == 0) {
-                    double r15[15];
-                    bf::imu_raw_residual(p1, G, &X.pose[0], &X.sb[0], &X.pose[7], &X.sb[9], r15);
-                    for (int r = 0; r < 15; r++) {
-                        double sacc = 0;
-                        for (int k = 0; k <= r; k++) sacc += p1.sqrt_info[r * 15 + k] * r15[k];
-                        raw[r * 31 + 30] = sacc;
-                    }
-                } else
-                    bf::imu_raw_jacobian_part(p1, G, &X.pose[0], &X.sb[0], &X.pose[7], &X.sb[9], part - 1, raw, 31);
-            }
-            __syncthreads();
-            for (int w = t; w < 450; w += nt) {
-                int r = w / 30, col = w - r * 30;
-                double sacc = 0;
-                for (int k = 0; k <= r; k++) sacc += p1.sqrt_info[r * 15 + k] * raw[k * 31 + col];
-                Jw[w] = sacc;
-            }
-            __syncthreads();
-            for (int w = t; w < 930; w += nt) {
-                int a = w / 31, bb = w - a * 31;
-                int ia = a < 15 ? a : (a < 21 ? md + (a - 15) : rS + (a - 21));
-                double sacc = 0;
-                if (bb < 30) {
-                    int ib = bb < 15 ? bb : (bb < 21 ? md + (bb - 15) : rS + (bb - 21));
-                    for (int k = 0; k < 15; k++) sacc += Jw[k * 30 + a] * Jw[k * 30 + bb];
-                    A[ia * mq + ib] += sacc;
-                } else {
-                    for (int k = 0; k < 15; k++) sacc += Jw[k * 30 + a] * raw[k * 31 + 30];
-                    b[ia] += sacc;
-                }
-            }
-            if (t == 0) { newpresent[0] = 1; newpresent[W] = 1; }
-            __syncthreads();
-        }
+        marg_imu_phase(c, be, X, A, b, md, mq);
         PH(17);
-        int nlm = be.n_lm;
-        int *flag = c.lm_tmp, *offs = c.res_k;
-        for (int k = t; k < nlm; k += nt) { int slot = c.lm_order[k]; flag[k] = (in_problem(c, slot) && c.lm_start[slot] == 0) ? 1 : 0; }
-        __syncthreads();
-        int F0 = block_scan_flags(flag, nlm, offs, scratch);
-        int *list0 = c.pair_list;
-        for (int k = t; k < nlm; k += nt) if (flag[k]) list0[offs[k]] = c.lm_order[k];
-        __syncthreads();
+        const int F0 = marg_lm_list(c, be, scratch);
         const int per = W;
         int F0c = min(F0, c.nres_cap / per);
         if (exact) { F0c = min(F0c, min(C.MX - 15, 480)); F0x = F0c; }
         F0k = F0c;
-        __shared__ double mgeo[(VIO_MAXW + 1) * 32 + 16];
-        if (t >= 1 && t <= W) {
-            bf::PairGeo g;
-            bf::pair_geo(&X.pose[0], &X.pose[t * 7], X.ex, g);
-            double *o = mgeo + (size_t)(t - 1) * 32;
-            for (int q = 0; q < 9; q++) { o[q] = g.A1[q]; o[9 + q] = g.A2[q]; o[18 + q] = g.M[q]; }
-            o[27] = g.t[0]; o[28] = g.t[1]; o[29] = g.t[2];
-        }
-        if (t == 0) stm(mgeo + (size_t)W * 32, q2R(mkq(X.ex[6], X.ex[3], X.ex[4], X.ex[5])));
-        __syncthreads();
-        for (int w = t; w < F0c * per; w += nt) {
-            int li = w / per, k = w - li * per + 1;
-            int slot = list0[li];
-            double *out = c.res + (size_t)w * 42;
-            if (k >= c.lm_nobs[slot]) { out[40] = 0; out[41] = 0; for (int q = 0; q < 40; q++) out[q] = 0; continue; }
-            double rr[2], wgt = 1.0;
-            const double inv_dep = 1.0 / c.lm_depth[slot];
-            const bf::PairGeo &g = *(const bf::PairGeo *)(mgeo + (size_t)(k - 1) * 32);
-            bf::eval_projection_pair(cfg, g, mgeo + (size_t)W * 32, X.ex, inv_dep, X.td, c.K->tr, obs_ptr(c, slot, 0), obs_ptr(c, slot, k), cfg.estimate_td != 0, rr, out,
-                                     true, &wgt);
-            out[40] = wgt * rr[0];
-            out[41] = wgt * rr[1];
-        }
+        __shared__ double mgeo[MARG_GEO_DOUBLES];
+        marg_pair_geo(X, W, mgeo);
+        __syncthreads();
+        marg_lm_records(c, X, mgeo, 0, F0c);
         __syncthreads();
         PH(18);
-        double *Cl = c.Hpl;
-        const int ldc = c.LW;
-        for (int w = t; w < F0c * ldc; w += nt) Cl[w] = 0;
-        __syncthreads();
-        {
-            const int grp = t >> 4, gln = t & 15, ngrp = nt >> 4;
-            for (int li0 = 0; li0 < F0c; li0 += ngrp) {
-                const int li = li0 + grp;
-                const bool act = li < F0c;
-                const int no = act ? c.lm_nobs[list0[li]] : 0;
-                double cm[13], dsum = 0, bsum = 0;
-#pragma unroll
-                for (int q = 0; q < 13; q++) cm[q] = 0;
-                for (int k = gln + 1; k < no; k += 16) {
-                    const double *Jg = c.res + (size_t)(li * per + k - 1) * 42;
-                    double Jr[42];
-#pragma unroll
-                    for (int q = 0; q < 42; q++) Jr[q] = Jg[q];
-                    const double jl0 = Jr[19], jl1 = Jr[39];
-#pragma unroll
-                    for (int q = 0; q < 6; q++) {
-                        cm[q] += Jr[q] * jl0 + Jr[20 + q] * jl1;
-                        cm[6 + q] += Jr[12 + q] * jl0 + Jr[32 + q] * jl1;
-                        Cl[(size_t)li * ldc + md + 6 * (k - 1) + q] = Jr[6 + q] * jl0 + Jr[26 + q] * jl1;
-                    }
-                    if (cfg.estimate_td) cm[12] += Jr[18] * jl0 + Jr[38] * jl1;
-                    dsum += jl0 * jl0 + jl1 * jl1;
-                    bsum += jl0 * Jr[40] + jl1 * Jr[41];
-                }
-#pragma unroll
-                for (int off = 8; off >= 1; off >>= 1) {
-#pragma unroll
-                    for (int q = 0; q < 13; q++) cm[q] += __shfl_xor(cm[q], off, 16);
-                    dsum += __shfl_xor(dsum, off, 16);
-                    bsum += __shfl_xor(bsum, off, 16);
-                }
-                if (act && gln == 0) {
-#pragma unroll
-                    for (int q = 0; q < 6; q++) { Cl[(size_t)li * ldc + q] = cm[q]; Cl[(size_t)li * ldc + rE + q] = cm[6 + q]; }
-                    if (cfg.estimate_td) Cl[(size_t)li * ldc + rT] = cm[12];
-                    c.Hll[li] = dsum;
-                    c.gl[li] = bsum;
-                }
-            }
-        }
-        __syncthreads();
+        marg_lm_rows(c, md, 0, F0c, !exact);
         PH(19);
-        {
-            const int lane = t & 63, wave = t >> 6, nw = nt >> 6, li = lane & 15, lk = lane >> 4;
-            for (int j = 1 + wave; j <= W; j += nw) {
-                v4f64 a00 = {0, 0, 0, 0}, a10 = {0, 0, 0, 0}, a11 = {0, 0, 0, 0};
-                const int K = 2 * F0c;
-                for (int k0 = 0; k0 < K; k0 += 64) {
-                    double x0[16], x1[16];
-#pragma unroll
-                    for (int u = 0; u < 16; u++) {
-                        int kk = k0 + 4 * u + lk;
-                        bool valid = kk < K;
-                        int lm = min(kk, K - 1) >> 1, sub = kk & 1;
-                        const double *Jr = c.res + (size_t)(lm * per + j - 1) * 42;
-                        double v0 = Jr[sub * 20 + li];
-                        double v1 = Jr[li < 3 ? sub * 20 + 16 + li : 40 + sub];
-                        x0[u] = valid ? v0 : 0.0;
-                        x1[u] = (valid && li < 4) ? v1 : 0.0;
-                    }
-#pragma unroll
-                    for (int u = 0; u < 16; u++) {
-                        if (k0 + 16 * (u >> 2) >= K) break;
-                        a00 = __builtin_amdgcn_mfma_f64_16x16x4f64(x0[u], x0[u], a00, 0, 0, 0);
-                        a10 = __builtin_amdgcn_mfma_f64_16x16x4f64(x1[u], x0[u], a10, 0, 0, 0);
-                        a11 = __builtin_amdgcn_mfma_f64_16x16x4f64(x1[u], x1[u], a11, 0, 0, 0);
-                    }
-                }
-                double *out = c.pairblk + (size_t)(j - 1) * 210;
-#pragma unroll
-                for (int r = 0; r < 4; r++) {
-                    int row = lk + 4 * r, col = li;
-                    if (col <= row) out[sym_idx(col, row)] = a00[r];
-                    if (row < 4) out[sym_idx(col, 16 + row)] = a10[r];
-                    if (row < 4 && col < 4 && col <= row) out[sym_idx(16 + col, 16 + row)] = a11[r];
-                }
-            }
-        }
-        if (!exact) for (int li = t; li < F0c; li += nt) { double d = c.Hll[li]; c.Hll[li] = d > eps ? 1.0 / d : 0.0; }
+        for (int j = 1 + (t >> 6); j <= W; j += nt >> 6) marg_frame_block(c, j, F0c);
         __syncthreads();
         PH(24);
-        __shared__ signed char qfr[6 * VIO_MAXW + 40], qlc[6 * VIO_MAXW + 40];
-        __shared__ double sub_part[4][6 * VIO_MAXW + 40];
-        for (int a = t; a <= mq; a += nt) {
-            int fr = -1, lc = 0;
-            if (a == mq) { fr = 0; lc = 19; }
-            else if (a < 6) { fr = 0; lc = a; }
-            else if (a >= md && a < md + 6 * W) { fr = (a - md) / 6 + 1; lc = 6 + (a - md) % 6; }
-            else if (a >= rE && a < rE + 6) { fr = 0; lc = 12 + (a - rE); }
-            else if (a == rT && cfg.estimate_td) { fr = 0; lc = 18; }
-            qfr[a] = (signed char)fr; qlc[a] = (signed char)lc;
-        }
-        for (int w = t; w < 4 * mq; w += nt) {
-            const int ch = w / mq, a = w - ch * mq;
-            double acc = 0;
-            if (!exact) for (int li = ch; li < F0c; li += 4) acc += Cl[(size_t)li * ldc + a] * (c.gl[li] * c.Hll[li]);
-            sub_part[ch][a] = acc;
-        }
-        __syncthreads();
-        for (int w0 = t; w0 < mq * (mq + 1); w0 += 4 * nt) {
-            bool use[4], multi[4], rhs[4];
-            int dst[4], row[4], sidx[4];
-            double pv[4], av[4];
-#pragma unroll
-            for (int u = 0; u < 4; u++) {
-                const int w = min(w0 + u * nt, mq * (mq + 1) - 1);
-                const int a = w / (mq + 1), bb = w - a * (mq + 1);
-                const int fa = qfr[a], fb = qfr[bb];
-                const int la = qlc[a], lb = qlc[bb];
-                use[u] = w0 + u * nt < mq * (mq + 1) && fa >= 0 && fb >= 0 && !(fa > 0 && fb > 0 && fa != fb);
-                multi[u] = use[u] && fa == 0 && fb == 0;
-                rhs[u] = bb == mq; row[u] = a; dst[u] = a * mq + bb;
-                sidx[u] = sym_idx(la, lb);
-                const int f1 = fa > 0 ? fa : (fb > 0 ? fb : 1);
-                pv[u] = use[u] ? c.pairblk[(size_t)(f1 - 1) * 210 + sidx[u]] : 0.0;
-                av[u] = use[u] ? (rhs[u] ? b[a] : A[dst[u]]) : 0.0;
-            }
-#pragma unroll
-            for (int u = 0; u < 4; u++) {
-                if (!use[u]) continue;
-                double sacc = pv[u];
-                if (multi[u]) {
-                    double fv[VIO_MAXW];
-#pragma unroll
-                    for (int j = 0; j < VIO_MAXW; j++) fv[j] = c.pairblk[(size_t)min(j, W - 1) * 210 + sidx[u]];
-                    sacc = 0;
-#pragma unroll
-                    for (int j = 0; j < VIO_MAXW; j++) if (j < W) sacc += fv[j];
-                }
-                if (!rhs[u]) A[dst[u]] = av[u] + sacc;
-                else b[row[u]] = av[u] + (sacc - ((sub_part[0][row[u]] + sub_part[1][row[u]]) + (sub_part[2][row[u]] + sub_part[3][row[u]])));
-            }
-        }
+        __shared__ signed char qfr[MARG_QMAP_LEN], qlc[MARG_QMAP_LEN];
+        __shared__ double sub_part[4][MARG_QMAP_LEN];
+        marg_qmap(c, md, mq, qfr, qlc);
+        marg_sub_part(c, F0c, mq, !exact, &sub_part[0][0], MARG_QMAP_LEN, t, nt);
+        __syncthreads();
+        marg_scatter(c, A, b, mq, qfr, qlc, &sub_part[0][0], MARG_QMAP_LEN, t, nt);
         __syncthreads();
         PH(25);
         if (!exact) {
-            const int lane = t & 63, wave = t >> 6, nw = nt >> 6, li = lane & 15, lk = lane >> 4;
             const int nbq = (mq + 15) >> 4, ntile = nbq * (nbq + 1) / 2;
-            for (int tile = wave; tile < ntile; tile += nw) {
-                int ti, tj;
-                tri_decode(tile, ti, tj);
-                v4f64 acc = {0, 0, 0, 0};
-                const int ca = min(16 * ti + li, ldc - 1), cb = min(16 * tj + li, ldc - 1);
-                for (int k0 = 0; k0 < F0c; k0 += 64) {
-                    double xa[16], xb[16];
-#pragma unroll
-                    for (int u = 0; u < 16; u++) {
-                        int kk = k0 + 4 * u + lk;
-                        bool valid = kk < F0c;
-                        int kc = min(kk, F0c - 1);
-                        double va = Cl[(size_t)kc * ldc + ca], vb = Cl[(size_t)kc * ldc + cb], dinv = c.Hll[kc];
-                        xa[u] = valid ? -(va * dinv) : 0.0;
-                        xb[u] = valid ? vb : 0.0;
-                    }
-#pragma unroll
-                    for (int u = 0; u < 16; u++) {
-                        if (k0 + 16 * (u >> 2) >= F0c) break;
-                        acc = __builtin_amdgcn_mfma_f64_16x16x4f64(xa[u], xb[u], acc, 0, 0, 0);
-                    }
-                }
-#pragma unroll
-                for (int r = 0; r < 4; r++) {
-                    int row = 16 * ti + lk + 4 * r, col = 16 * tj + li;
-                    if (row < mq && col < mq && (ti != tj || col <= row)) {
-                        A[row * mq + col] += acc[r];
-                        if (row != col) A[col * mq + row] += acc[r];
-                    }
-                }
-            }
-        }
-        for (int li = t; li < F0c; li += nt) {
-            int no = c.lm_nobs[list0[li]];
-            for (int k = 1; k < no; k++) newpresent[k - 1] = 1;
-            if (no > 1) { newpresent[W + 1] = 1; if (cfg.estimate_td) newpresent[W + 2] = 1; }
-        }
-        __syncthreads();
+            for (int tile = t >> 6; tile < ntile; tile += nt >> 6) marg_rank_tile(c, tile, F0c, mq, A, nullptr);
+        }
+        __syncthreads();
+    }
     }
     if (VIO_TIMERS && s == 0 && t == 0 && !second_new) B.timings[31] += 1.0f;
     PH(20);
@@ -2703,6 +2791,7 @@
     }
     }
     PH(22);
+    marg_new_present(c, be, second_new, F0k, newpresent);
     if (t < W) {
         int src = second_new ? (t == W - 1 ? W : t) : t + 1;
         for (int d = 0; d < 7; d++) c.prior_x0[t * 7 + d] = X.pose[src * 7 + d];
@@ -2713,6 +2802,78 @@
     if (t < W + 3) be.prior_present[t] = newpresent[t];
     if (t == 0) { be.has_prior = 1; be.dbg[3] = (int)(VIO_CLOCK() - tk0); }
     PH(23);
+}
+
+__device__ __forceinline__ bool ps_blk(const Batch &B, int &s, int &b);
+__device__ __forceinline__ bool marg_wide_blk(const Batch &B, int &s, int &g, int &nwg) {
+    nwg = B.xcd_nb > 0 ? B.xcd_nb : (int)gridDim.x;
+    return ps_blk(B, s, g);
+}
+__global__ __launch_bounds__(256) void be_marg_lm_kernel(Batch B) {
+    int s, g, nwg;
+    if (!marg_wide_blk(B, s, g, nwg)) return;
+    Ctx c = make_ctx(B, s);
+    BeSeq &be = *c.be;
+    if (!marg_runs(c, be) || be.marginalization_flag != 0) return;
+    __shared__ Params X;
+    __shared__ int scratch[2 * 256 + 8];
+    __shared__ double sdx[6 * VIO_MAXW + 16], srp[6 * VIO_MAXW + 16];
+    __shared__ double mgeo[MARG_GEO_DOUBLES];
+    const int W = c.W, md = 15, mq = md + c.NPR;
+    marg_load_state(be, W, X);
+    __syncthreads();
+    if (g == 0) {
+        marg_prior_phase(c, be, X, sdx, srp, c.margA, c.margB, md, mq, false);
+        marg_imu_phase(c, be, X, c.margA, c.margB, md, mq);
+    }
+    if (g > 0 || nwg == 1) {
+        const int F0c = min(marg_lm_list(c, be, scratch), c.nres_cap / W);
+        const int nch = max(nwg - 1, 1), ch = nwg == 1 ? 0 : g - 1, share = (F0c + nch - 1) / nch;
+        const int lo = min(ch * share, F0c), hi = min(lo + share, F0c);
+        marg_pair_geo(X, W, mgeo);
+        __syncthreads();
+        marg_lm_records(c, X, mgeo, lo, hi);
+        __syncthreads();
+        marg_lm_rows(c, md, lo, hi, true);
+    }
+}
+__global__ __launch_bounds__(256) void be_marg_blk_kernel(Batch B) {
+    int s, g, nwg;
+    if (!marg_wide_blk(B, s, g, nwg)) return;
+    Ctx c = make_ctx(B, s);
+    BeSeq &be = *c.be;
+    if (!marg_runs(c, be) || be.marginalization_flag != 0) return;
+    const int W = c.W, mq = 15 + c.NPR, nw = blockDim.x >> 6, lane = threadIdx.x & 63;
+    const int F0c = min(marg_lm_count(c, be), c.nres_cap / W);
+    const int nbq = (mq + 15) >> 4, ntile = nbq * (nbq + 1) / 2, nsp = (4 * mq + 63) >> 6;
+    for (int u = g * nw + (threadIdx.x >> 6); u < W + ntile + nsp; u += nwg * nw) {
+        if (u < W) marg_frame_block(c, u + 1, F0c);
+        else if (u < W + ntile) marg_rank_tile(c, u - W, F0c, mq, nullptr, c.margW);
+        else marg_sub_part(c, F0c, mq, true, c.vec + c.LW, c.LW, (u - W - ntile) * 64 + lane, nsp * 64);
+    }
+}
+__global__ __launch_bounds__(256) void be_marg_scatter_kernel(Batch B) {
+    int s, g, nwg;
+    if (!marg_wide_blk(B, s, g, nwg)) return;
+    Ctx c = make_ctx(B, s);
+    BeSeq &be = *c.be;
+    if (!marg_runs(c, be) || be.marginalization_flag != 0) return;
+    __shared__ signed char qfr[MARG_QMAP_LEN], qlc[MARG_QMAP_LEN];
+    const int md = 15, mq = md + c.NPR, tid = g * (int)blockDim.x + (int)threadIdx.x, nthr = nwg * (int)blockDim.x;
+    marg_qmap(c, md, mq, qfr, qlc);
+    __syncthreads();
+    marg_scatter(c, c.margA, c.margB, mq, qfr, qlc, c.vec + c.LW, c.LW, tid, nthr);
+    marg_add_parked(c.margA, mq, c.margW, tid, nthr);
+}
+__global__ __launch_bounds__(512) void be_marg_tail_kernel(Batch B) {
+    const int s = blockIdx.x + B.s0;
+    __shared__ int scratch[2 * 512 + 8];
+    __shared__ double sred[64];
+    __shared__ PreWork pw;
+    extern __shared__ __attribute__((aligned(16))) unsigned char smem[];
+    marg_body<false, true>(B, s, scratch, sred, smem);
+    __syncthreads();
+    finish_body(B, s, scratch, pw, smem);
 }
 
 __global__ void be_set_relo_kernel(Batch B, int seq, const double *par) {
diff --git a/vins-rgbd-fast_amd/csrc/kernels.h b/vins-rgbd-fast_amd/csrc/kernels.h
--- a/vins-rgbd-fast_amd/csrc/kernels.h
+++ b/vins-rgbd-fast_amd/csrc/kernels.h
@@ -50,6 +50,11 @@
 __global__ void be_solve_kernel_512(Batch B);
 __global__ void be_marg_kernel(Batch B);
 __global__ void be_marg_exact_kernel(Batch B);
+__global__ void be_marg_lm_kernel(Batch B);
+__global__ void be_marg_blk_kernel(Batch B);
+__global__ void be_marg_scatter_kernel(Batch B);
+__global__ void be_marg_tail_kernel(Batch B);
+static inline size_t marg_park_doubles(size_t n) { const size_t nbq = (15 + n + 15) >> 4; return nbq * (nbq + 1) / 2 * 256; }
 __global__ void ps_setup_kernel(Batch B);
 __global__ void ps_eval_kernel(Batch B);
 __global__ void ps_eval_kernel_occ3(Batch B);
diff --git a/vins-rgbd-fast_amd/csrc/vio_abi.hip b/vins-rgbd-fast_amd/csrc/vio_abi.hip
--- a/vins-rgbd-fast_amd/csrc/vio_abi.hip
+++ b/vins-rgbd-fast_amd/csrc/vio_abi.hip
@@ -132,6 +132,7 @@
     int relo_frames = 0;
     bool line_search = true;
     int be_threads = 512, marg_threads = 384;
+    int marg_wide = 1, marg_wg_lm = 9, marg_wg_blk = 8, marg_wg_scatter = 8;
     int solve_mode = 1;
     bool asm_a_occ4 = false;
     int eval_occ = 0;
@@ -721,7 +722,19 @@
         h->state_pending = true;
     }
     if (C.MX > 0) be_marg_exact_kernel<<<S, h->marg_threads, h->lds_marg, st>>>(Bg);
-    else be_marg_kernel<<<S, h->marg_threads, h->lds_marg, st>>>(Bg);
+    else if (h->marg_wide) {
+        const bool xm = h->xcd_map && S >= 8;
+        const int XN = h->xcd_n > 0 ? h->xcd_n : 8, S8 = XN * ((S + XN - 1) / XN);
+        auto wide = [&](void (*k)(Batch), int nb) {
+            Batch Bm = Bg;
+            Bm.ns = S; Bm.xcd_n = XN; Bm.xcd_nb = xm ? nb : 0;
+            k<<<xm ? dim3(S8 * nb) : dim3(nb, S), 256, 0, st>>>(Bm);
+        };
+        wide(be_marg_lm_kernel, h->marg_wg_lm);
+        wide(be_marg_blk_kernel, h->marg_wg_blk);
+        wide(be_marg_scatter_kernel, h->marg_wg_scatter);
+        be_marg_tail_kernel<<<S, h->marg_threads, h->lds_marg, st>>>(Bg);
+    } else be_marg_kernel<<<S, h->marg_threads, h->lds_marg, st>>>(Bg);
     if (prof) PEV(h, 11);
     HIPCHK(hipGetLastError());
     return VIO_OK;
@@ -947,7 +960,7 @@
     DA(B.res, S * nres * 42); DA(B.res_lm, S * nres); DA(B.res_k, S * nres); DA(B.res_pair, S);
     DA(B.pair_start, S * (npair + 1)); DA(B.pair_list, S * nres); DA(B.pairblk, S * npair * 210);
     DA(B.imu_raw, S * C.W * 15 * 31);
-    DA(B.margA, S * mq * mq); DA(B.margB, S * mq); DA(B.margV, S * n * n); DA(B.margW, S * (n + 16) * (n + 16));
+    DA(B.margA, S * mq * mq); DA(B.margB, S * mq); DA(B.margV, S * n * n); DA(B.margW, S * std::max((n + 16) * (n + 16), marg_park_doubles(n)));
     if (C.MX > 0) DA(B.margE, S * ((size_t)3 * C.MX * C.MX + n * (size_t)C.MX));
     DA(B.odom, S * 11); DA(B.timings, 128); DA(B.fe_ticks, S * 4);
     if (C.c.estimate_extrinsic == 2) { DA(h->hc.exc, S); DA(h->hc.exh, S * (size_t)VIO_EXCALIB_CAP * VIO_EXCALIB_PAIR_D); }
@@ -968,6 +981,10 @@
     if (getenv("VIO_EXTRA_SLOTS")) h->extra_slots = std::max(1, atoi(getenv("VIO_EXTRA_SLOTS")));
     if (getenv("VIO_ASM_A_OCC")) h->asm_a_occ4 = atoi(getenv("VIO_ASM_A_OCC")) >= 4;
     if (getenv("VIO_MARG_THREADS")) h->marg_threads = std::min(512, std::max(64, atoi(getenv("VIO_MARG_THREADS")) & ~63));
+    if (getenv("VIO_MARG_WIDE")) h->marg_wide = atoi(getenv("VIO_MARG_WIDE")) != 0;
+    if (getenv("VIO_MARG_WG_LM")) h->marg_wg_lm = std::max(1, std::min(64, atoi(getenv("VIO_MARG_WG_LM"))));
+    if (getenv("VIO_MARG_WG_BLK")) h->marg_wg_blk = std::max(1, std::min(64, atoi(getenv("VIO_MARG_WG_BLK"))));
+    if (getenv("VIO_MARG_WG_SCATTER")) h->marg_wg_scatter = std::max(1, std::min(64, atoi(getenv("VIO_MARG_WG_SCATTER"))));
     B.flags = getenv("VIO_FLAGS") ? atoi(getenv("VIO_FLAGS")) : 0;
     DA(B.odom_hist, S * (size_t)B.hist_cap * 11); DA(B.odom_count, S);
     DA(B.sst, S);
@@ -1086,6 +1103,7 @@
         }
         (void)raise_lds_limit((const void *)be_marg_kernel, (size_t)(h->lds_marg));
         (void)raise_lds_limit((const void *)be_marg_exact_kernel, (size_t)(h->lds_marg));
+        (void)raise_lds_limit((const void *)be_marg_tail_kernel, (size_t)(h->lds_marg));
         const bool excalib = C.c.estimate_extrinsic == 2;
         const void *ingest = excalib ? (const void *)be_ingest_kernel<true> : (const void *)be_ingest_kernel<false>;
         (void)raise_lds_limit(ingest, ingest_lds_bytes(C, excalib));
@@ -1093,7 +1111,7 @@
         (void)raise_lds_limit((const void *)fe_select_kernel, (size_t)(h->lds_select));
         (void)raise_lds_limit((const void *)fe_add_kernel, (size_t)(h->lds_add));
         (void)raise_lds_limit((const void *)fe_fast_kernel, (size_t)(h->lds_fast));
-        bool fits = lds_fits(C.MX > 0 ? (const void *)be_marg_exact_kernel : (const void *)be_marg_kernel, h->lds_marg, "be_marg") &&
+        bool fits = lds_fits(C.MX > 0 ? (const void *)be_marg_exact_kernel : h->marg_wide ? (const void *)be_marg_tail_kernel : (const void *)be_marg_kernel, h->lds_marg, "be_marg") &&
                     lds_fits(ingest, ingest_lds_bytes(C, excalib), "be_ingest") &&
                     lds_fits((const void *)fe_select_kernel, h->lds_select, "fe_select") && lds_fits((const void *)fe_add_kernel, h->lds_add, "fe_add") &&
                     lds_fits((const void *)fe_fast_kernel, h->lds_fast, "fe_fast");
@@ -1995,7 +2013,7 @@
     SCRATCH(ls_scratch, (int64_t)ps_eval_lds_bytes(C.W)); SCRATCH(pairpart, (int64_t)PS_FUSE_MAXPAIRS * PS_FUSE_MAXBLK * 210);
     HANDLE("gW gP gLW gNL gNP gNRES gNPRIOR gMX"); HANDLE("gn_ext n_schur form_s fuse fuse_only");
     SCRATCH(imu_raw, (int64_t)C.W * 15 * 31);
-    SCRATCH(margA, mq * mq); SCRATCH(margB, mq); SCRATCH(margV, n * n); SCRATCH(margW, (n + 16) * (n + 16));
+    SCRATCH(margA, mq * mq); SCRATCH(margB, mq); SCRATCH(margV, n * n); SCRATCH(margW, std::max((n + 16) * (n + 16), (int64_t)marg_park_doubles((size_t)n)));
     SCRATCH(margE, (int64_t)3 * C.MX * C.MX + n * (int64_t)C.MX);
     STATE(odom, 11); STATE(odom_hist, (int64_t)B.hist_cap * 11); STATE(odom_count, 1);
     HANDLE("hist_cap (shape key)"); HANDLE("flags");
```
